# PersiaML/PERSIA

Measured on AMD Instinct MI355X. Metric: samples/sec (whole node), DLRM-style hybrid training, higher is better.
Workload: dtype bf16; 1 GPU; preset=criteo, model=dlrm 26sparse/13dense dim128, global_batch=8192, rows=100000000, capacity_per_rank=100000000, staleness=8, parallelism=dp1+emb-a2a

## Files before the change

persia_amd/core/engine.py:

```python
import contextlib
import functools
import os
import queue
import threading
import time
from dataclasses import dataclass, field
from typing import Dict, List, Optional, Tuple

import numpy as np
import torch

from persia_amd.core import hashing
from persia_amd.core.comm import DistContext
from persia_amd.core.schema import EmbeddingSchema, GlobalConfig, SlotConfig
from persia_amd.core.store import make_store
from persia_amd.embedding import EmbeddingConfig
from persia_amd.embedding.data import PersiaBatch
from persia_amd.embedding.optim import Optimizer
from persia_amd.logger import get_default_logger
from persia_amd.ops import reference as R

_logger = get_default_logger("persia_amd.engine")

_FLIP = -(2 ** 63)
_NO_STREAM = contextlib.nullcontext()


def _roctx_range(name):

    def deco(fn):
        @functools.wraps(fn)
        def wrap(self, *a, **k):
            if not getattr(self, "_roctx", False):
                return fn(self, *a, **k)
            torch.cuda.nvtx.range_push(name)
            try:
                return fn(self, *a, **k)
            finally:
                torch.cuda.nvtx.range_pop()
        return wrap
    return deco


def _update_entry(fn):

    @functools.wraps(fn)
    def wrap(self, *a, **k):
        self._update_counter += 1
        sample = (
            self.metrics_enabled
            and self._update_counter % self._metrics_every
            == 1 % self._metrics_every
        )
        if not (sample or self._roctx):
            return fn(self, *a, **k)
        if self._roctx:
            torch.cuda.nvtx.range_push("persia:update")
        t0 = time.perf_counter()
        try:
            return fn(self, *a, **k)
        finally:
            if sample:
                self.metrics.update_gradient_time_cost_sec.set(
                    time.perf_counter() - t0
                )
            if self._roctx:
                torch.cuda.nvtx.range_pop()

    return wrap


def _sqrt_scale(sqrt_mask: torch.Tensor, seg_lens: torch.Tensor) -> torch.Tensor:
    return torch.where(
        sqrt_mask, seg_lens.clamp(min=1.0).rsqrt(), torch.ones_like(seg_lens)
    )


def _owner_of_keys(keys: torch.Tensor, world_size: int) -> torch.Tensor:
    hi = (keys >> 32) & 0xFFFFFFFF
    return (hi * world_size) >> 32


def _dedup(keys_t: torch.Tensor):
    dev = keys_t.device
    nnz = keys_t.numel()
    if nnz == 0:
        z = torch.zeros(0, dtype=torch.int64, device=dev)
        return z, z, z, torch.zeros(1, dtype=torch.int64, device=dev)
    flipped = keys_t ^ _FLIP
    svals, perm = torch.sort(flipped)
    neq = torch.ones(nnz, dtype=torch.bool, device=dev)
    neq[1:] = svals[1:] != svals[:-1]
    inv_sorted = torch.cumsum(neq, 0) - 1
    inverse = torch.empty(nnz, dtype=torch.int64, device=dev)
    inverse[perm] = inv_sorted
    uniq = svals[neq] ^ _FLIP
    ustarts = torch.cat(
        [
            torch.nonzero(neq, as_tuple=False).view(-1),
            torch.tensor([nnz], dtype=torch.int64, device=dev),
        ]
    )
    return uniq, inverse, perm, ustarts


@dataclass
class SlotPayload:

    name: str
    cfg: SlotConfig
    sum_tensor: Optional[torch.Tensor] = None
    raw_distinct: Optional[torch.Tensor] = None
    raw_index: Optional[torch.Tensor] = None
    raw_non_empty_index: Optional[torch.Tensor] = None
    raw_sample_id_num: Optional[torch.Tensor] = None

    @property
    def is_raw(self) -> bool:
        return self.raw_distinct is not None


@dataclass
class _SlotCtx:
    name: str
    cfg: SlotConfig
    pos_slice: Tuple[int, int]
    seg_offsets: torch.Tensor
    sum_seg_base: int = -1
    slot_uniq_global: Optional[torch.Tensor] = None
    slot_inverse: Optional[torch.Tensor] = None


@dataclass
class _GroupCtx:
    dim: int
    uniq_keys: torch.Tensor
    inverse: torch.Tensor
    perm: torch.Tensor
    ustarts: torch.Tensor
    u_count: Optional[torch.Tensor] = None
    slots: List[_SlotCtx] = field(default_factory=list)
    cat_offsets: Optional[torch.Tensor] = None
    seg_id: Optional[torch.Tensor] = None
    seg_lens: Optional[torch.Tensor] = None
    sqrt_mask: Optional[torch.Tensor] = None
    sum_base: Optional[torch.Tensor] = None
    n_sum_slots: int = 0
    send_counts: Optional[List[int]] = None
    recv_counts: Optional[List[int]] = None
    a2a_plan: Optional["_GroupPlan"] = None
    a2a_idx: Optional[torch.Tensor] = None
    a2a_recv_keys: Optional[torch.Tensor] = None
    a2a_owner_dedup: Optional[tuple] = None


class _GroupPlan:

    def __init__(self, dim: int, cfgs: List[SlotConfig], B: int,
                 device: torch.device):
        S = len(cfgs)
        self.dim = dim
        self.names = tuple(c.name for c in cfgs)
        self.B = B
        self.S = S
        prefixes_np = np.array([c.index_prefix for c in cfgs], dtype=np.uint64)
        self.slot_starts = torch.arange(0, (S + 1) * B, B, dtype=torch.int64,
                                        device=device)
        self.prefixes = torch.from_numpy(prefixes_np.view(np.int64)).to(device)
        self.cat_offsets = torch.arange(S * B + 1, dtype=torch.int64, device=device)
        self.seg_id = torch.arange(S * B, dtype=torch.int64, device=device)
        self.empty_scale = torch.empty(0, dtype=torch.float32, device=device)
        self.a2a_world: Optional[int] = None
        self.a2a_cap: Optional[int] = None
        self.a2a_ar: Optional[torch.Tensor] = None
        self.a2a_ones: Optional[torch.Tensor] = None
        self.owner_seg_id: Optional[torch.Tensor] = None


class _SplitSlots(torch.autograd.Function):

    @staticmethod
    def forward(ctx, base: torch.Tensor, n_slots: int, B: int):
        ctx.n_slots, ctx.B, ctx.dim = n_slots, B, base.shape[1]
        ctx.dev, ctx.dtype = base.device, base.dtype
        return tuple(base[i * B : (i + 1) * B] for i in range(n_slots))

    @staticmethod
    def backward(ctx, *grads):
        parts = [
            g
            if g is not None
            else torch.zeros(ctx.B, ctx.dim, dtype=ctx.dtype, device=ctx.dev)
            for g in grads
        ]
        return torch.cat(parts, dim=0), None, None


class PersiaTrainingBatch:

    def __init__(self):
        self._payloads: List[SlotPayload] = []
        self._lazy_sum_groups: List[Tuple["_GroupCtx", List[str], int]] = []
        self._order: Optional[Dict[str, int]] = None
        self._sorted: bool = False
        self.non_id_type_tensors: List[torch.Tensor] = []
        self.label_tensors: List[torch.Tensor] = []
        self.batch_size: int = 0
        self.requires_grad: bool = True
        self.meta: Optional[bytes] = None
        self.batch_id: Optional[int] = None
        self._groups: List[_GroupCtx] = []
        self._engine: Optional["EmbeddingEngine"] = None

    @property
    def payloads(self) -> List[SlotPayload]:
        if self._lazy_sum_groups:
            for group, _names, B in self._lazy_sum_groups:
                sums = group.sum_base
                for i, sc in enumerate(group.slots):
                    self._payloads.append(
                        SlotPayload(name=sc.name, cfg=sc.cfg,
                                    sum_tensor=sums[i * B : (i + 1) * B])
                    )
            self._lazy_sum_groups.clear()
            self._sorted = False
        if not self._sorted:
            if self._order is not None:
                self._payloads.sort(key=lambda p: self._order[p.name])
            self._sorted = True
        return self._payloads

    def enable_training_views(self) -> Dict[str, torch.Tensor]:
        views: Dict[str, torch.Tensor] = {}
        for group in self._groups:
            if group.sum_base is None:
                continue
            group.sum_base.requires_grad_(True)
            sum_names = [sc.name for sc in group.slots if sc.cfg.embedding_summation]
            parts = _SplitSlots.apply(group.sum_base, len(sum_names), self.batch_size)
            views.update(zip(sum_names, parts))
        return views

    def training_embeddings(self) -> List[torch.Tensor]:
        views = self.enable_training_views()
        return [views.get(p.name, p.sum_tensor) for p in self.payloads]

    def record_stream(self, stream: "torch.cuda.Stream") -> None:
        for t in self._device_tensors():
            t.record_stream(stream)

    def _device_tensors(self):
        for t in self.non_id_type_tensors + self.label_tensors:
            if t.is_cuda:
                yield t
        for g in self._groups:
            a2a_owner = g.a2a_owner_dedup or ()
            for t in (g.uniq_keys, g.inverse, g.perm, g.ustarts, g.u_count,
                      g.sum_base, g.cat_offsets, g.seg_id, g.seg_lens,
                      g.sqrt_mask, g.a2a_idx, g.a2a_recv_keys, *a2a_owner):
                if t is not None and t.is_cuda:
                    yield t
            for sc in g.slots:
                for t in (sc.seg_offsets, sc.slot_uniq_global, sc.slot_inverse):
                    if t is not None and t.is_cuda:
                        yield t
        for p in self._payloads:
            for t in (p.raw_distinct, p.raw_index, p.raw_non_empty_index,
                      p.raw_sample_id_num):
                if t is not None and t.is_cuda:
                    yield t


class EmbeddingEngine:
    def __init__(
        self,
        schema: EmbeddingSchema,
        hyper: EmbeddingConfig,
        optimizer: Optional[Optimizer],
        gconf: GlobalConfig,
        device: torch.device,
        dist_ctx: Optional[DistContext] = None,
        wire_dtype: torch.dtype = torch.float16,
    ):
        self.schema = schema
        self.hyper = hyper
        self.optimizer = optimizer
        self.gconf = gconf
        self.device = device
        self.dist = dist_ctx or DistContext.from_default_group()
        self.dist_grad = (
            DistContext.new_sparse_group() if self.dist.distributed else self.dist
        )
        self.wire_dtype = wire_dtype
        self.groups: Dict[int, List[SlotConfig]] = {}
        for name in schema.slot_names():
            cfg = schema.get_slot(name)
            self.groups.setdefault(cfg.dim, []).append(cfg)
        if optimizer is None:
            from persia_amd.embedding.optim import SGD

            optimizer = SGD(lr=0.0)
            self.optimizer = optimizer
        self.stores = {
            dim: make_store(
                dim, gconf.capacity, optimizer, hyper, device, gconf.spill_capacity
            )
            for dim in self.groups
        }
        self.skipped_grad_signs = 0
        self.nan_grad_batches = 0
        self._plans = {}
        self._empty_scale = torch.empty(0, dtype=torch.float32, device=device)
        spacing = schema.feature_spacing
        self._spacing_arg = spacing if spacing < (1 << 63) else -1
        self.model_manager_status = "Idle"
        self.model_manager_progress = 0.0
        self._prod_timing = os.environ.get("PA_PROD_TIMING", "0") == "1"
        self._prod_timing_live = True
        self._pt = {"prep": 0.0, "native": 0.0, "batch": 0.0, "n": 0,
                    "skip": 20}
        self._fused_dist = os.environ.get("PA_FUSED_DIST", "1") == "1"
        self._force_dist = os.environ.get("PA_FORCE_DIST", "0") == "1"
        self._roctx = os.environ.get("PA_ROCTX", "0") == "1"
        self._a2a_overflow = torch.zeros(1, dtype=torch.int64, device=device)
        from persia_amd.core.metrics import EngineMetrics

        self.metrics_enabled = bool(gconf.enable_metrics)
        self.metrics = EngineMetrics(self.metrics_enabled)
        self._metrics_every = max(1, int(os.environ.get("PA_METRICS_EVERY", "64")))
        self._batch_counter = 0
        self._update_counter = 0
        self._pending_metric = None
        self._skipped_last = (0, 0)
        self._evicted_last = 0
        self.monitor = None
        if self.metrics_enabled:
            from persia_amd.core.monitor import DistinctIdMonitor

            self.monitor = DistinctIdMonitor()
        self.incremental = None
        if gconf.enable_incremental_update:
            self.enable_incremental_update(
                gconf.incremental_dir, gconf.incremental_buffer_size
            )

    def enable_incremental_update(self, dst_dir: str,
                                  buffer_size: int = 1_000_000):
        from persia_amd.core.incremental import IncrementalUpdateDumper

        self.incremental = IncrementalUpdateDumper(self, dst_dir, buffer_size)
        return self.incremental

    @functools.cached_property
    def _C(self):
        from persia_amd.ops import native

        return native()

    def _tick(self, key: str, t0: float) -> float:
        now = time.perf_counter()
        if self._prod_timing_live:
            self._pt[key] = self._pt.get(key, 0.0) + (now - t0)
        return now

    @staticmethod
    def _materialize_group(group: "_GroupCtx") -> "_GroupCtx":
        if group.u_count is None:
            return group
        U = int(group.u_count.item())
        group.uniq_keys = group.uniq_keys.narrow(0, 0, U)
        group.ustarts = group.ustarts.narrow(0, 0, U + 1)
        group.u_count = None
        return group


    def _prepare_slot_keys(self, feat) -> Tuple[np.ndarray, np.ndarray]:
        cfg = self.schema.get_slot(feat.name)
        values, offsets = feat.values, feat.offsets
        rounds = cfg.hash_stack_rounds
        if rounds > 0:
            stacked = hashing.hash_stack(
                values, rounds, cfg.hash_stack_config.embedding_size
            )
            B = len(offsets) - 1
            lens = offsets[1:] - offsets[:-1]
            new_vals = np.empty(len(values) * rounds, dtype=np.uint64)
            new_offsets = np.zeros(B + 1, dtype=np.int64)
            np.cumsum(lens * rounds, out=new_offsets[1:])
            for r in range(rounds):
                for b in range(B):
                    s, e = offsets[b], offsets[b + 1]
                    dst = new_offsets[b] + r * (e - s)
                    new_vals[dst : dst + (e - s)] = stacked[r, s:e]
            values, offsets = new_vals, new_offsets
        signs = hashing.apply_prefix(values, cfg.index_prefix, self.schema.feature_spacing)
        keys = hashing.splitmix64(signs)
        keys[keys == np.uint64(0)] = np.uint64(0xD1B54A32D192ED03)
        return keys, offsets


    def _exchange_rows(self, group: _GroupCtx, train: bool) -> torch.Tensor:
        store = self.stores[group.dim]
        if not self.dist.distributed:
            rows = store.lookup(group.uniq_keys, train, u_count=group.u_count)
            return rows
        owner = _owner_of_keys(group.uniq_keys, self.dist.world_size)
        send_counts = torch.bincount(owner, minlength=self.dist.world_size).tolist()
        recv_counts = self.dist.all_to_all_lengths(send_counts, self.device)
        group.send_counts, group.recv_counts = send_counts, recv_counts
        recv_keys = self.dist.all_to_all(group.uniq_keys, send_counts, recv_counts)
        rows_local = store.lookup(recv_keys, train).to(self.wire_dtype)
        rows = self.dist.all_to_all(rows_local, recv_counts, send_counts)
        return rows


    def _a2a_setup(self, plan: "_GroupPlan") -> Tuple[int, int]:
        if plan.a2a_cap is not None:
            return plan.a2a_world, plan.a2a_cap
        world = self.dist.world_size
        nnz = plan.S * plan.B
        if world > 1:
            lo, hi = self.dist.allreduce_int_minmax(nnz)
            if lo != hi:
                raise RuntimeError(
                    f"padded-a2a fast path needs equal per-rank batch shapes "
                    f"(nnz min {lo} != max {hi}); set PA_FUSED_DIST=0"
                )
            per = max(1, nnz // world)
            cap = per + max(512, per // 8)
        else:
            cap = nnz
        plan.a2a_world = world
        plan.a2a_cap = cap
        plan.a2a_ar = torch.arange(nnz, dtype=torch.int64, device=self.device)
        plan.a2a_ones = torch.ones(nnz, dtype=torch.int64, device=self.device)
        plan.owner_seg_id = torch.arange(
            world * cap, dtype=torch.int64, device=self.device
        )
        return world, cap

    def _a2a_route(self, plan: "_GroupPlan", uniq: torch.Tensor,
                   u_count: Optional[torch.Tensor]):
        world, cap = plan.a2a_world, plan.a2a_cap
        if self.device.type == "cuda":
            return self._C.a2a_route(
                uniq,
                u_count if u_count is not None
                else self.stores[plan.dim].no_count,
                world, cap, self._a2a_overflow,
            )
        n = uniq.numel()
        ar = plan.a2a_ar[:n]
        owner = _owner_of_keys(uniq, world)
        if u_count is not None:
            owner = torch.where(ar < u_count, owner,
                                torch.full_like(owner, world))
        counts = torch.zeros(world + 1, dtype=torch.int64, device=uniq.device)
        counts.scatter_add_(0, owner, plan.a2a_ones[:n])
        starts = torch.cumsum(counts, 0) - counts
        pos = ar - starts.gather(0, owner)
        dummy = world * cap
        bad = (owner >= world) | (pos >= cap)
        idx = torch.where(bad, torch.full_like(pos, dummy), owner * cap + pos)
        send = torch.zeros(dummy + 1, dtype=torch.int64, device=uniq.device)
        send.scatter_(0, idx, uniq)
        self._a2a_overflow.add_((counts[:world] > cap).sum())
        return send, idx

    @_roctx_range("persia:a2a_exchange")
    def _a2a_exchange_fwd(self, plan: "_GroupPlan", group: _GroupCtx,
                          train: bool):
        world, cap = self._a2a_setup(plan)
        timing = self._prod_timing
        if timing:
            t = time.perf_counter()
        send_keys, idx = self._a2a_route(plan, group.uniq_keys, group.u_count)
        comm = self.dist
        if world > 1:
            recv_keys = comm.all_to_all_even(send_keys[: world * cap])
        else:
            recv_keys = send_keys[: world * cap].clone()
        if timing:
            t = self._tick("route", t)
        store = self.stores[group.dim]
        rows_local = store.lookup_wire(recv_keys, train, self.wire_dtype)
        if timing:
            self._tick("lkw", t)
        rows_full = torch.empty(
            world * cap + 1, group.dim, dtype=rows_local.dtype,
            device=self.device,
        )
        if world > 1:
            comm.all_to_all_even(rows_local, out=rows_full[: world * cap])
        else:
            rows_full[: world * cap].copy_(rows_local)
        rows_full[world * cap].zero_()
        group.a2a_plan = plan
        group.a2a_idx = idx
        group.a2a_recv_keys = recv_keys
        if train and self.device.type == "cuda":
            group.a2a_owner_dedup = tuple(self._C.dedup_padded(recv_keys))
        return rows_full, idx

    def check_a2a_overflow(self) -> int:
        return int(self._a2a_overflow.sum().item())


    @_roctx_range("persia:process_batch")
    def process_batch(self, batch: PersiaBatch, train: Optional[bool] = None) -> PersiaTrainingBatch:
        if self._prod_timing:
            self._prod_timing_live = self._pt["skip"] <= 0
            if not self._prod_timing_live:
                self._pt["skip"] -= 1
            _tb0 = time.perf_counter()
        self._batch_counter += 1
        sample = (
            self.metrics_enabled
            and self._batch_counter % self._metrics_every == 1 % self._metrics_every
        )
        if sample:
            _ms_t0 = time.perf_counter()
            _ms_ev0 = None
            if self.device.type == "cuda":
                _ms_ev0 = torch.cuda.Event(enable_timing=True)
                _ms_ev0.record()
        train = batch.requires_grad if train is None else train
        if self.gconf.job_type == "infer":
            train = False
        out = PersiaTrainingBatch()
        out.batch_size = batch.batch_size
        out.requires_grad = batch.requires_grad
        out.meta = batch.meta
        out.batch_id = batch.batch_id
        out._engine = self

        for i, x in enumerate(batch.non_id_type_features):
            out.non_id_type_tensors.append(
                self._upload_aux(batch, ("nid", i), x.data)
            )
        for i, x in enumerate(batch.labels):
            out.label_tensors.append(self._upload_aux(batch, ("lab", i), x.data))

        for dim, feats in self._feats_by_dim(batch).items():
            out._groups.append(self._process_group(dim, feats, out, train, batch))
        out._order = {f.name: i for i, f in enumerate(batch.id_type_features)}
        out._sorted = False
        if sample:
            self._record_lookup_metrics(batch, out, _ms_t0, _ms_ev0)
        if self._prod_timing and self._prod_timing_live:
            self._tick("batch", _tb0)
            self._pt["n"] += 1
        return out

    def _record_lookup_metrics(self, batch, out, t0: float, ev0) -> None:
        m = self.metrics
        m.lookup_preprocess_time_cost_sec.set(time.perf_counter() - t0)
        if self.monitor is not None:
            for feat in batch.id_type_features:
                vals = getattr(feat, "values", None)
                if vals is not None and len(vals):
                    self.monitor.observe(feat.name, vals)
            for name, est in self.monitor.estimates().items():
                m.distinct_id_estimate.labels(name).set(est)
        nnz = sum(
            len(getattr(f, "values", ())) for f in batch.id_type_features
        )
        pend = self._pending_metric
        self._pending_metric = None
        if pend is not None:
            ev_a, ev_b, ucnt_pin, skip_pin, p_nnz, done = pend
            if done.query():
                if ev_a is not None and ev_b is not None:
                    try:
                        m.lookup_hashmap_time_cost_sec.set(
                            ev_a.elapsed_time(ev_b) / 1e3
                        )
                    except Exception:
                        pass
                if ucnt_pin is not None and p_nnz:
                    m.batch_unique_indices_rate.set(
                        float(ucnt_pin.item()) / p_nnz
                    )
                if skip_pin is not None:
                    miss, nan = int(skip_pin[0].item()), int(skip_pin[1].item())
                    lm, ln = self._skipped_last
                    if miss > lm:
                        m.gradient_id_miss_count.inc(miss - lm)
                    if nan > ln:
                        m.nan_grad_skipped.inc(nan - ln)
                    self._skipped_last = (miss, nan)
        if self.device.type == "cuda":
            ev1 = torch.cuda.Event(enable_timing=True)
            ev1.record()
            ucnt_pin = None
            for g in out._groups:
                if g.u_count is not None:
                    ucnt_pin = torch.empty(1, dtype=torch.int64, pin_memory=True)
                    ucnt_pin.copy_(g.u_count, non_blocking=True)
                    break
                m.batch_unique_indices_rate.set(
                    g.uniq_keys.numel() / max(1, nnz)
                )
            skip_pin = None
            skipped = next(iter(self.stores.values())).skip_counters()
            if skipped is not None:
                skip_pin = torch.empty(2, dtype=torch.int32, pin_memory=True)
                skip_pin.copy_(skipped, non_blocking=True)
            done = torch.cuda.Event()
            done.record()
            self._pending_metric = (ev0, ev1, ucnt_pin, skip_pin, nnz, done)
        else:
            U = sum(g.uniq_keys.numel() for g in out._groups)
            m.batch_unique_indices_rate.set(U / max(1, nnz))
            m.nan_grad_skipped.inc(0)
        ev_tot = sum(
            getattr(s, "evicted_total", 0) for s in self.stores.values()
        )
        if ev_tot > self._evicted_last:
            m.evicted_count.inc(ev_tot - self._evicted_last)
            self._evicted_last = ev_tot

    def prepare_host_batch(self, batch: PersiaBatch) -> None:
        if self.device.type != "cuda":
            return
        pc = getattr(batch, "_pinned_cache", None)
        if pc is None:
            pc = batch._pinned_cache = {}
        for kind, items in (("nid", batch.non_id_type_features),
                            ("lab", batch.labels)):
            for i, x in enumerate(items):
                if (kind, i) not in pc:
                    pc[(kind, i)] = self._pin_array(x.data)
        for dim, feats in self._feats_by_dim(batch).items():
            if dim not in pc and self._all_single_sum(feats):
                pc[dim] = self._pin_values(feats)

    def _feats_by_dim(self, batch: PersiaBatch) -> Dict[int, List]:
        by_dim: Dict[int, List] = {}
        for feat in batch.id_type_features:
            by_dim.setdefault(self.schema.get_slot(feat.name).dim, []).append(feat)
        return by_dim

    @staticmethod
    def _pin_array(arr: np.ndarray) -> torch.Tensor:
        src = torch.from_numpy(np.ascontiguousarray(arr))
        t = torch.empty_like(src, pin_memory=True)
        t.copy_(src)
        return t

    def _upload_aux(self, batch, cache_key, arr: np.ndarray) -> torch.Tensor:
        if self.device.type != "cuda":
            return torch.from_numpy(np.ascontiguousarray(arr)).to(self.device)
        pc = getattr(batch, "_pinned_cache", None)
        if pc is None:
            pc = batch._pinned_cache = {}
        t = pc.get(cache_key)
        if t is None:
            t = pc[cache_key] = self._pin_array(arr)
        return t.to(self.device, non_blocking=True)

    def _pin_values(self, feats) -> torch.Tensor:
        values_np = np.concatenate([f.values for f in feats])
        pin = torch.empty(len(values_np), dtype=torch.int64, pin_memory=True)
        pin.numpy()[:] = values_np.view(np.int64)
        return pin

    def _upload_group(self, dim: int, feats, batch) -> torch.Tensor:
        pcache = getattr(batch, "_pinned_cache", None)
        if pcache is None:
            pcache = batch._pinned_cache = {}
        pin = pcache.get(dim)
        if pin is None:
            pin = pcache[dim] = self._pin_values(feats)
        return pin.to(self.device, non_blocking=True)

    def _all_single_sum(self, feats) -> bool:
        get_slot = self.schema.get_slot
        for f in feats:
            if not getattr(f, "is_single", False):
                return False
            cfg = get_slot(f.name)
            if not cfg.embedding_summation or cfg.hash_stack_rounds != 0:
                return False
        return True

    def _padded_a2a(self, store) -> bool:
        return (
            (self.dist.distributed or self._force_dist)
            and self._fused_dist
            and store.spill is None
        )

    def _plan(self, dim: int, names: Tuple[str, ...], B: int) -> _GroupPlan:
        plan = self._plans.get((dim, names, B))
        if plan is None:
            cfgs = [self.schema.get_slot(n) for n in names]
            plan = self._plans[(dim, names, B)] = _GroupPlan(
                dim, cfgs, B, self.device
            )
        return plan

    def _process_group_fast(self, dim: int, feats, out: PersiaTrainingBatch,
                            train: bool, batch: PersiaBatch) -> _GroupCtx:
        timing = self._prod_timing
        if timing:
            t0 = time.perf_counter()
        C = self._C
        B = len(feats[0].values)
        plan = self._plan(dim, tuple(f.name for f in feats), B)
        slot_ctxs = [
            _SlotCtx(
                name=f.name, cfg=self.schema.get_slot(f.name),
                pos_slice=(i * B, (i + 1) * B), seg_offsets=None,
                sum_seg_base=i * B,
            )
            for i, f in enumerate(feats)
        ]
        store = self.stores[dim]
        dist = self.dist.distributed
        one_call = not (dist or self._force_dist or store.spill is not None)
        padded = not one_call and self._padded_a2a(store)
        if one_call:
            if timing:
                t0 = self._tick("prep", t0)
            sums, uniq, inverse, perm, ustarts, u_count = store.lookup_local(
                self._upload_group(dim, feats, batch), plan.slot_starts,
                plan.prefixes, self._spacing_arg, plan.cat_offsets,
                plan.empty_scale, train,
            )
        else:
            ps = cur = None
            if store.spill is not None and not dist and train:
                ps, cur = store.probe_stream, torch.cuda.current_stream()
            with torch.cuda.stream(ps) if ps is not None else _NO_STREAM:
                vals_t = self._upload_group(dim, feats, batch)
                keys_t = C.sign_prep(
                    vals_t, plan.slot_starts, plan.prefixes, self._spacing_arg
                )
                if padded or not dist:
                    uniq, inverse, perm, ustarts, u_count = C.dedup_padded(keys_t)
                else:
                    uniq, inverse, perm, ustarts = _dedup(keys_t)
                    u_count = None
                if ps is not None:
                    store.spill_restore(uniq, u_count)
            if ps is not None:
                cur.wait_stream(ps)
                for x in (vals_t, uniq, inverse, perm, ustarts, u_count):
                    x.record_stream(cur)
        group = _GroupCtx(
            dim=dim, uniq_keys=uniq, inverse=inverse, perm=perm,
            ustarts=ustarts, u_count=u_count, slots=slot_ctxs,
            cat_offsets=plan.cat_offsets, seg_id=plan.seg_id,
            n_sum_slots=plan.S,
        )
        if padded:
            if timing:
                t = self._tick("dedup", t0)
            rows_full, idx = self._a2a_exchange_fwd(plan, group, train)
            if timing:
                t = self._tick("exch", t)
            sums = C.segment_sum(
                rows_full, idx.gather(0, inverse), plan.cat_offsets,
                plan.empty_scale,
            )
            if timing:
                self._tick("sum", t)
        elif not one_call:
            rows = self._exchange_rows(group, train)
            sums = C.segment_sum(
                rows.contiguous(), inverse, plan.cat_offsets, plan.empty_scale
            )
        group.sum_base = sums
        out._lazy_sum_groups.append((group, [sc.name for sc in slot_ctxs], B))
        if timing and (one_call or padded):
            self._tick("native", t0)
        return group

    def _process_group(self, dim: int, feats, out: PersiaTrainingBatch, train: bool,
                       batch: PersiaBatch) -> _GroupCtx:
        native = self.device.type == "cuda"
        fast_shape = self._all_single_sum(feats)
        if native and fast_shape:
            return self._process_group_fast(dim, feats, out, train, batch)
        feats = sorted(
            feats, key=lambda f: 0 if self.schema.get_slot(f.name).embedding_summation else 1
        )
        keys_t, slot_ctxs = self._group_keys(feats, gpu_prep=native)
        uniq_keys, inverse, perm, ustarts = _dedup(keys_t)
        group = _GroupCtx(
            dim=dim, uniq_keys=uniq_keys, inverse=inverse, perm=perm,
            ustarts=ustarts, slots=slot_ctxs,
        )
        if not native and fast_shape and self._padded_a2a(self.stores[dim]):
            plan = self._plan(
                dim, tuple(sc.name for sc in slot_ctxs), out.batch_size
            )
            rows_full, idx = self._a2a_exchange_fwd(plan, group, train)
            rows = rows_full[idx]
        else:
            rows = self._exchange_rows(group, train)
        self._sum_payloads(group, rows, out)
        self._raw_payloads(group, rows, out)
        return group

    def _group_keys(self, feats, gpu_prep: bool):
        dev = self.device
        key_arrays = []
        offset_arrays = []
        slot_ctxs: List[_SlotCtx] = []
        in_lens: List[int] = []
        rounds_list: List[int] = []
        sizes_list: List[int] = []
        pos = 0
        for feat in feats:
            cfg = self.schema.get_slot(feat.name)
            r = cfg.hash_stack_rounds
            if gpu_prep:
                keys = feat.values
                offsets = feat.offsets * r if r > 0 else feat.offsets
                out_len = len(keys) * max(r, 1)
            else:
                keys, offsets = self._prepare_slot_keys(feat)
                out_len = len(keys)
            key_arrays.append(keys)
            offset_arrays.append(offsets)
            in_lens.append(len(keys))
            rounds_list.append(r if gpu_prep else 0)
            sizes_list.append(
                cfg.hash_stack_config.embedding_size if r > 0 else 1
            )
            slot_ctxs.append(
                _SlotCtx(name=feat.name, cfg=cfg, pos_slice=(pos, pos + out_len),
                         seg_offsets=None)
            )
            pos += out_len

        all_keys = np.concatenate(key_arrays) if key_arrays else np.empty(0, np.uint64)
        keys_t = torch.from_numpy(all_keys.view(np.int64)).to(dev, non_blocking=False)
        all_offs = np.concatenate(offset_arrays or [np.zeros(1, np.int64)])
        all_offs_t = torch.from_numpy(all_offs).to(dev)
        o0 = 0
        for sc, offs in zip(slot_ctxs, offset_arrays):
            sc.seg_offsets = all_offs_t[o0 : o0 + len(offs)]
            o0 += len(offs)
        if not gpu_prep:
            return keys_t, slot_ctxs
        out_starts = torch.tensor(
            [sc.pos_slice[0] for sc in slot_ctxs] + [pos],
            dtype=torch.int64, device=dev,
        )
        prefixes = torch.from_numpy(
            np.array([sc.cfg.index_prefix for sc in slot_ctxs], dtype=np.uint64)
            .view(np.int64)
        ).to(dev)
        if not any(rounds_list):
            return self._C.sign_prep(
                keys_t, out_starts, prefixes, self._spacing_arg
            ), slot_ctxs
        in_starts = torch.from_numpy(
            np.concatenate([[0], np.cumsum(in_lens)]).astype(np.int64)
        ).to(dev)
        off_starts = torch.from_numpy(
            np.concatenate(
                [[0], np.cumsum([len(o) for o in offset_arrays])]
            ).astype(np.int64)
        ).to(dev)
        keys_t = self._C.sign_prep_stack(
            keys_t, in_starts, out_starts, prefixes,
            torch.tensor(rounds_list, dtype=torch.int32, device=dev),
            torch.tensor(sizes_list, dtype=torch.int64, device=dev),
            off_starts, all_offs_t, self._spacing_arg, pos,
        )
        return keys_t, slot_ctxs

    def _sum_payloads(self, group: _GroupCtx, rows: torch.Tensor,
                      out: PersiaTrainingBatch) -> None:
        sum_slots = [sc for sc in group.slots if sc.cfg.embedding_summation]
        if not sum_slots:
            return
        dev = self.device
        base = 0
        offs_parts, sqrt_parts = [], []
        for sc in sum_slots:
            s, _e = sc.pos_slice
            sc.sum_seg_base = base
            nseg = sc.seg_offsets.numel() - 1
            offs_parts.append(sc.seg_offsets[:-1] + s)
            sqrt_parts.append(
                torch.full((nseg,), bool(sc.cfg.sqrt_scaling), dtype=torch.bool, device=dev)
            )
            base += nseg
        sum_end = sum_slots[-1].pos_slice[1]
        cat_offsets = torch.cat(
            offs_parts + [torch.tensor([sum_end], dtype=torch.int64, device=dev)]
        )
        group.cat_offsets = cat_offsets
        group.sqrt_mask = torch.cat(sqrt_parts)
        seg_counts = cat_offsets[1:] - cat_offsets[:-1]
        group.seg_lens = seg_counts.float()
        seg_id = torch.full(
            (group.inverse.numel(),), -1, dtype=torch.int64, device=dev
        )
        seg_id[:sum_end] = torch.repeat_interleave(
            torch.arange(base, dtype=torch.int64, device=dev), seg_counts
        )
        group.seg_id = seg_id
        fwd_scale = _sqrt_scale(group.sqrt_mask, group.seg_lens)
        if dev.type == "cuda":
            sums = self._C.segment_sum(
                rows.contiguous(), group.inverse, cat_offsets, fwd_scale
            )
        else:
            sums = (
                R.segment_sum_rows(
                    rows, group.inverse[:sum_end], cat_offsets, False, torch.float32
                )
                * fwd_scale.unsqueeze(1)
            ).to(torch.float16)
        group.sum_base = sums
        group.n_sum_slots = len(sum_slots)
        b0 = 0
        for sc in sum_slots:
            nseg = sc.seg_offsets.numel() - 1
            out._payloads.append(
                SlotPayload(name=sc.name, cfg=sc.cfg, sum_tensor=sums[b0 : b0 + nseg])
            )
            b0 += nseg

    def _raw_payloads(self, group: _GroupCtx, rows: torch.Tensor,
                      out: PersiaTrainingBatch) -> None:
        for sc in group.slots:
            if sc.cfg.embedding_summation:
                continue
            s, e = sc.pos_slice
            slot_uniq, slot_inv = torch.unique(
                group.inverse[s:e], sorted=True, return_inverse=True
            )
            sc.slot_uniq_global = slot_uniq
            sc.slot_inverse = slot_inv
            scale = 1.0
            rounds = sc.cfg.hash_stack_rounds
            if sc.cfg.sqrt_scaling and rounds > 1:
                scale = 1.0 / float(np.sqrt(rounds))
            distinct, index, non_empty, num = R.raw_embedding_tensors(
                rows[slot_uniq], slot_inv, sc.seg_offsets, sc.cfg.sample_fixed_size,
                scale, torch.float16,
            )
            out._payloads.append(
                SlotPayload(
                    name=sc.name, cfg=sc.cfg, raw_distinct=distinct, raw_index=index,
                    raw_non_empty_index=non_empty, raw_sample_id_num=num,
                )
            )


    def _seg_scale(self, group: _GroupCtx, loss_scale: float,
                   skip: Optional[torch.Tensor] = None) -> torch.Tensor:
        mask = group.sqrt_mask
        has_sqrt = mask is not None and (skip is not None or bool(mask.any()))
        if skip is None and loss_scale == 1.0 and not has_sqrt:
            return self._empty_scale
        scale = torch.full(
            (group.cat_offsets.numel() - 1,), 1.0 / loss_scale,
            device=self.device,
        )
        if has_sqrt:
            scale = scale * _sqrt_scale(mask, group.seg_lens)
        if skip is not None:
            scale = torch.where(skip, torch.zeros_like(scale), scale)
        return scale

    def _nan_slot(self, sc: _SlotCtx, g: torch.Tensor) -> bool:
        if not bool(torch.isnan(g).any()):
            return False
        self.nan_grad_batches += 1
        _logger.warning(f"nan found in gradient update of {sc.name}, skipping")
        return True

    def _add_raw_grads(self, group: _GroupCtx, grads, loss_scale: float,
                       buf: torch.Tensor) -> bool:
        added = False
        for sc in group.slots:
            if sc.cfg.embedding_summation:
                continue
            g = grads.get(sc.name)
            if g is None or self._nan_slot(sc, g):
                continue
            gf = g.float()
            if loss_scale != 1.0:
                gf = gf / loss_scale
            rounds = sc.cfg.hash_stack_rounds
            if sc.cfg.sqrt_scaling and rounds > 0:
                gf = gf / float(np.sqrt(rounds))
            buf.index_add_(0, sc.slot_uniq_global, gf)
            added = True
        return added

    @_update_entry
    def apply_gradients(
        self,
        training_batch: PersiaTrainingBatch,
        grads: Dict[str, Optional[torch.Tensor]],
        loss_scale: float = 1.0,
    ) -> None:
        self._apply_slot_grads(training_batch, grads, loss_scale)

    def _apply_slot_grads(self, training_batch, grads, loss_scale) -> None:
        native = self.device.type == "cuda"
        B = training_batch.batch_size
        for group in training_batch._groups:
            self._materialize_group(group)
            U = group.uniq_keys.numel()
            buf = torch.zeros(U, group.dim, dtype=torch.float32, device=self.device)
            sum_slots = [
                sc for sc in group.slots
                if sc.cfg.embedding_summation and grads.get(sc.name) is not None
            ]
            any_grad = False
            if native and sum_slots:
                g_parts, flag_parts = [], []
                for sc in group.slots:
                    if not sc.cfg.embedding_summation:
                        continue
                    g = grads.get(sc.name)
                    if g is None:
                        g = torch.zeros(B, group.dim, dtype=torch.float16, device=self.device)
                        flag = torch.ones((), dtype=torch.bool, device=self.device)
                    else:
                        flag = torch.isnan(g).any()
                    g_parts.append(g.to(torch.float16))
                    flag_parts.append(flag.expand(B))
                scale = self._seg_scale(group, loss_scale, skip=torch.cat(flag_parts))
                self._C.grad_scatter(
                    torch.nan_to_num(torch.cat(g_parts, dim=0)).contiguous(),
                    group.perm, group.ustarts, group.seg_id, scale.contiguous(),
                    buf, 1,
                )
                any_grad = True
            elif not native:
                for sc in sum_slots:
                    g = grads[sc.name]
                    if self._nan_slot(sc, g):
                        continue
                    any_grad = True
                    s, e = sc.pos_slice
                    buf += R.segment_grad_scatter(
                        g, group.inverse[s:e], sc.seg_offsets, U,
                        scale_factor=loss_scale, sqrt_scaling=sc.cfg.sqrt_scaling,
                    )
            if self._add_raw_grads(group, grads, loss_scale, buf) or any_grad:
                self._route_and_update(group, buf)

    def _a2a_backward_native(self, group: _GroupCtx, gbase: torch.Tensor,
                             seg_scale: torch.Tensor, store) -> None:
        plan = group.a2a_plan
        world, cap = plan.a2a_world, plan.a2a_cap
        send_g = torch.empty(
            world * cap + 1, group.dim, dtype=torch.float16, device=self.device
        )
        self._C.grad_scatter_idx(
            gbase.contiguous(), group.perm, group.ustarts, group.seg_id,
            seg_scale, group.a2a_idx, send_g,
            group.u_count if group.u_count is not None else store.no_count,
        )
        if world > 1:
            recv_g = self.dist_grad.all_to_all_even(send_g[: world * cap])
        else:
            recv_g = send_g[: world * cap]
        if group.a2a_owner_dedup is None:
            group.a2a_owner_dedup = tuple(
                self._C.dedup_padded(group.a2a_recv_keys)
            )
        ou, _oinv, operm, oustarts, ou_count = group.a2a_owner_dedup
        store.scatter_update(
            ou, recv_g, operm, oustarts, plan.owner_seg_id, ou_count
        )
        if self.incremental is not None:
            self.incremental.record_keys(ou, ou_count)

    def _store_update(self, store, keys: torch.Tensor, grads: torch.Tensor) -> None:
        self.skipped_grad_signs += store.update_gradients(keys, grads)
        if self.incremental is not None:
            self.incremental.record_keys(keys)

    def _owner_merge_update(self, store, keys_recv: torch.Tensor,
                            grads_recv: torch.Tensor) -> None:
        uniq_f, inv = torch.unique(keys_recv ^ _FLIP, sorted=True, return_inverse=True)
        merged = torch.zeros(
            uniq_f.numel(), store.dim, dtype=torch.float32, device=self.device
        )
        merged.index_add_(0, inv, grads_recv.float())
        self._store_update(store, uniq_f ^ _FLIP, merged)

    def _route_and_update_padded(self, group: _GroupCtx, buf: torch.Tensor) -> None:
        plan = group.a2a_plan
        world, cap = plan.a2a_world, plan.a2a_cap
        send_g = torch.zeros(
            world * cap + 1, group.dim, dtype=self.wire_dtype,
            device=self.device,
        )
        send_g.index_copy_(
            0, group.a2a_idx[: buf.shape[0]], buf.to(self.wire_dtype)
        )
        if world > 1:
            recv_g = self.dist_grad.all_to_all_even(send_g[: world * cap])
        else:
            recv_g = send_g[: world * cap]
        rk = group.a2a_recv_keys
        m = rk != 0
        if bool(m.any()):
            self._owner_merge_update(self.stores[group.dim], rk[m], recv_g[m])

    def _route_and_update(self, group: _GroupCtx, buf: torch.Tensor) -> None:
        store = self.stores[group.dim]
        if group.a2a_idx is not None:
            return self._route_and_update_padded(group, buf)
        if not self.dist.distributed:
            return self._store_update(store, group.uniq_keys, buf)
        comm = self.dist_grad
        send_counts, recv_counts = group.send_counts, group.recv_counts
        if send_counts is None:
            owner = _owner_of_keys(group.uniq_keys, comm.world_size)
            send_counts = torch.bincount(owner, minlength=comm.world_size).tolist()
            recv_counts = comm.all_to_all_lengths(send_counts, self.device)
        keys_recv = comm.all_to_all(group.uniq_keys, send_counts, recv_counts)
        grads_recv = comm.all_to_all(
            buf.to(self.wire_dtype), send_counts, recv_counts
        )
        self._owner_merge_update(store, keys_recv, grads_recv)

    @_update_entry
    def apply_gradients_base(
        self,
        training_batch: PersiaTrainingBatch,
        raw_grads: Optional[Dict[str, Optional[torch.Tensor]]] = None,
        loss_scale: float = 1.0,
        sum_base_grads: Optional[List[torch.Tensor]] = None,
    ) -> None:
        groups = training_batch._groups
        if sum_base_grads is None:
            sum_base_grads = [
                g.sum_base.grad if g.sum_base is not None else None
                for g in groups
            ]
        if self.device.type != "cuda":
            grads: Dict[str, Optional[torch.Tensor]] = dict(raw_grads or {})
            B = training_batch.batch_size
            for group, gbase in zip(groups, sum_base_grads):
                b0 = 0
                for sc in group.slots:
                    if sc.cfg.embedding_summation:
                        grads[sc.name] = (
                            gbase[b0 : b0 + B] if gbase is not None else None
                        )
                        b0 += B
            return self._apply_slot_grads(training_batch, grads, loss_scale)

        for group, gbase in zip(groups, sum_base_grads):
            if gbase is None and not raw_grads:
                continue
            store = self.stores[group.dim]
            if gbase is not None:
                seg_scale = self._seg_scale(group, loss_scale)
                if store.fused_native and not raw_grads:
                    if (
                        group.a2a_idx is not None
                        and self.wire_dtype == torch.float16
                    ):
                        self._a2a_backward_native(group, gbase, seg_scale, store)
                        continue
                    if not self.dist.distributed:
                        store.update_local(
                            gbase, group.perm, group.ustarts, group.seg_id,
                            seg_scale, group.uniq_keys, group.u_count,
                        )
                        if self.incremental is not None:
                            self.incremental.record_keys(
                                group.uniq_keys, group.u_count
                            )
                        continue
            self._materialize_group(group)
            U = group.uniq_keys.numel()
            if gbase is not None:
                buf = torch.empty(
                    U, group.dim, dtype=torch.float32, device=self.device
                )
                self._C.grad_scatter(
                    gbase.contiguous(), group.perm, group.ustarts,
                    group.seg_id, seg_scale, buf, 0,
                )
            else:
                buf = torch.zeros(
                    U, group.dim, dtype=torch.float32, device=self.device
                )
            if raw_grads:
                self._add_raw_grads(group, raw_grads, loss_scale, buf)
            self._route_and_update(group, buf)


    def _set_status(self, status: str, progress: float = 0.0):
        self.model_manager_status = status
        self.model_manager_progress = progress

    def dump(self, dst_dir: str, blocking: bool = True) -> None:
        from persia_amd.core.checkpoint import dump_embedding

        def run():
            try:
                dump_embedding(self, dst_dir)
                self._set_status("Idle", 100.0)
            except Exception as e:
                _logger.error(f"embedding dump failed: {e}")
                self._set_status("Failed")
                if blocking:
                    raise

        self._set_status("Dumping", 0.0)
        if blocking:
            run()
        else:
            threading.Thread(target=run, daemon=True, name="persia-ckpt-dump").start()

    def load(self, src_dir: str, blocking: bool = True) -> None:
        from persia_amd.core.checkpoint import load_embedding

        def run():
            try:
                load_embedding(self, src_dir)
                self._set_status("Idle", 100.0)
            except Exception as e:
                _logger.error(f"embedding load failed: {e}")
                self._set_status("Failed")
                if blocking:
                    raise

        self._set_status("Loading", 0.0)
        if blocking:
            run()
        else:
            threading.Thread(target=run, daemon=True, name="persia-ckpt-load").start()

    def wait_for_emb_dumping(self, timeout: float = 600.0) -> None:
        import time as _time

        t0 = _time.time()
        while getattr(self, "model_manager_status", "Idle") == "Dumping":
            if _time.time() - t0 > timeout:
                raise TimeoutError("embedding dump did not finish")
            _time.sleep(0.05)
        if getattr(self, "model_manager_status", "Idle") == "Failed":
            raise RuntimeError("embedding dump failed")

    def wait_for_emb_loading(self, timeout: float = 600.0) -> None:
        import time as _time

        t0 = _time.time()
        while getattr(self, "model_manager_status", "Idle") == "Loading":
            if _time.time() - t0 > timeout:
                raise TimeoutError("embedding load did not finish")
            _time.sleep(0.05)
        if getattr(self, "model_manager_status", "Idle") == "Failed":
            raise RuntimeError("embedding load failed")

    def num_resident_rows(self) -> int:
        return sum(len(s) for s in self.stores.values())


class ForwardPipeline:

    def __init__(self, engine: EmbeddingEngine, staleness: int = 8, out_buffer: int = 8,
                 reorder: bool = False):
        self.engine = engine
        self.staleness = max(1, staleness)
        self.reorder = reorder
        self._heap: list = []
        self._next_id = 0
        self._sem = threading.Semaphore(self.staleness)
        self._in: "queue.Queue" = queue.Queue(maxsize=max(2, out_buffer))
        self._out: "queue.Queue" = queue.Queue(maxsize=max(2, out_buffer))
        self._thread: Optional[threading.Thread] = None
        self._stop = threading.Event()
        self._exc: Optional[BaseException] = None
        self.inflight = 0
        self.prod_s = 0.0
        self.prod_n = 0

    def start(self):
        if self._thread is None:
            self._thread = threading.Thread(target=self._run, daemon=True, name="persia-forward")
            self._thread.start()

    def _run(self):
        stream = None
        if self.engine.device.type == "cuda":
            torch.cuda.set_device(self.engine.device)
            prio = int(os.environ.get("PA_SPARSE_PRIORITY", "0"))
            stream = torch.cuda.Stream(device=self.engine.device, priority=prio)
        import heapq

        pending_eof = False
        while not self._stop.is_set():
            item = None
            if self.reorder and self._heap and self._heap[0][0] == self._next_id:
                item = heapq.heappop(self._heap)[1]
                self._next_id += 1
            else:
                try:
                    got = self._in.get(timeout=0.1)
                except queue.Empty:
                    if pending_eof and not self._heap:
                        self._out.put(None)
                        break
                    continue
                if got is None:
                    if self.reorder and self._heap:
                        pending_eof = True
                        continue
                    self._out.put(None)
                    break
                if self.reorder and got.batch_id is not None:
                    if got.batch_id != self._next_id:
                        heapq.heappush(self._heap, (got.batch_id, got))
                        continue
                    self._next_id += 1
                item = got
            self._sem.acquire()
            self.inflight += 1
            if self.engine.metrics_enabled:
                self.engine.metrics.staleness.set(self.inflight)
            try:
                t0 = time.perf_counter()
                if stream is not None:
                    with torch.cuda.stream(stream):
                        tb = self.engine.process_batch(item)
                    ev = torch.cuda.Event()
                    ev.record(stream)
                    tb._ready_event = ev
                else:
                    tb = self.engine.process_batch(item)
                self.prod_s += time.perf_counter() - t0
                self.prod_n += 1
                self._out.put(tb)
            except BaseException as e:
                self._exc = e
                self._out.put(None)
                break

    def put(self, batch: PersiaBatch):
        self.start()
        self._in.put(batch)
        if self.engine.metrics_enabled:
            self.engine.metrics.num_pending_batches.set(self._in.qsize())

    def finish(self):
        self.start()
        self._in.put(None)

    def get(self, timeout: Optional[float] = None) -> Optional[PersiaTrainingBatch]:
        tb = self._out.get(timeout=timeout)
        if tb is None and self._exc is not None:
            raise self._exc
        if tb is not None and getattr(tb, "_ready_event", None) is not None:
            cur = torch.cuda.current_stream()
            cur.wait_event(tb._ready_event)
            tb.record_stream(cur)
        return tb

    def release_permit(self):
        self.inflight = max(0, self.inflight - 1)
        self._sem.release()

    def stop(self):
        self._stop.set()
        self._sem.release()
        try:
            self._in.put_nowait(None)
        except queue.Full:
            pass
        if self._thread is not None:
            self._thread.join(timeout=5.0)
            self._thread = None
```

persia_amd/core/store.py:

```python
from typing import Iterator, Optional, Tuple

import numpy as np
import torch

from persia_amd.core import hashing
from persia_amd.embedding import EmbeddingConfig
from persia_amd.embedding.optim import Adagrad, Adam, Optimizer, SGD

BUCKET_SIZE = 8
PROBE_BUCKETS = 4
EMPTY_KEY = np.uint64(0)
_ZERO_REMAP = np.uint64(0xD1B54A32D192ED03)


def _floor_pow2(x: int) -> int:
    p = 1
    while (p << 1) <= x:
        p <<= 1
    return p


def _u01_from_u64(u: np.ndarray) -> np.ndarray:
    return (u >> np.uint64(40)).astype(np.float64) * (1.0 / (1 << 24))


def row_init(sign: int, dim: int, lo: float, hi: float) -> np.ndarray:
    seed = hashing.init_seed_for(np.array([sign], dtype=np.uint64))[0]
    cols = np.arange(1, dim + 1, dtype=np.uint64)
    u = hashing.splitmix64(np.uint64(seed) ^ cols)
    return (lo + (hi - lo) * _u01_from_u64(u)).astype(np.float32)


class HostTier:

    def __init__(self, capacity: int, row_width: int):
        from collections import OrderedDict

        self.capacity = capacity
        self.row_width = row_width
        self._map: "OrderedDict[int, np.ndarray]" = OrderedDict()

    def __len__(self) -> int:
        return len(self._map)

    def insert(self, keys: np.ndarray, rows: np.ndarray) -> None:
        for i, k in enumerate(keys):
            k = int(k)
            if k in self._map:
                self._map.move_to_end(k)
            self._map[k] = rows[i].copy()
        while len(self._map) > self.capacity:
            self._map.popitem(last=False)

    def fetch(self, keys: np.ndarray):
        rows = np.zeros((len(keys), self.row_width), dtype=np.float32)
        found = np.zeros(len(keys), dtype=bool)
        for i, k in enumerate(keys):
            row = self._map.pop(int(k), None)
            if row is not None:
                rows[i] = row
                found[i] = True
        return rows, found

    def __contains__(self, key) -> bool:
        return int(key) in self._map

    def export(self):
        n = len(self._map)
        keys = np.fromiter(self._map.keys(), dtype=np.uint64, count=n)
        rows = (
            np.stack(list(self._map.values()))
            if n
            else np.zeros((0, self.row_width), dtype=np.float32)
        )
        return keys, rows.astype(np.float32)


class NativeHostTier:

    def __init__(self, capacity: int, row_width: int):
        from persia_amd.ops import native

        self.capacity = capacity
        self.row_width = row_width
        self._impl = native().HostTier(capacity, row_width)

    def __len__(self) -> int:
        return int(self._impl.size())

    def insert(self, keys: np.ndarray, rows: np.ndarray) -> None:
        self._impl.insert(
            torch.from_numpy(np.ascontiguousarray(keys).view(np.int64)),
            torch.from_numpy(np.ascontiguousarray(rows, dtype=np.float32)),
        )

    def fetch(self, keys: np.ndarray):
        rows, found = self._impl.fetch(
            torch.from_numpy(np.ascontiguousarray(keys).view(np.int64))
        )
        return rows.numpy(), found.numpy()

    def __contains__(self, key) -> bool:
        return bool(self._impl.contains(int(np.int64(np.uint64(key)))))

    def export(self):
        keys, rows = self._impl.export_all()
        return keys.numpy().view(np.uint64), rows.numpy()



def _adapt_row_width(inner: np.ndarray, row_width: int,
                     state_init: float = 0.0) -> np.ndarray:
    cur = inner.shape[1]
    if cur == row_width:
        return inner
    if cur > row_width:
        return np.ascontiguousarray(inner[:, :row_width])
    out = np.full((inner.shape[0], row_width), state_init, dtype=np.float32)
    out[:, :cur] = inner
    return out


class EmbeddingStoreBase:

    fused_native = False

    def __init__(
        self,
        dim: int,
        capacity: int,
        optimizer: Optimizer,
        hyper: EmbeddingConfig,
        device: torch.device,
        spill_capacity: int = 0,
    ):
        self.dim = dim
        self.optimizer = optimizer
        self.hyper = hyper
        self.device = device
        self.opt_space = optimizer.require_space(dim)
        self.row_width = dim + self.opt_space
        self.n_buckets = _floor_pow2(max(1, capacity // BUCKET_SIZE))
        self.n_slots = self.n_buckets * BUCKET_SIZE
        self.tick = 1
        self._tick_lock = __import__("threading").Lock()
        self.spill = HostTier(spill_capacity, self.row_width) if spill_capacity > 0 else None
        if isinstance(optimizer, Adam):
            self.beta1_power = optimizer.betas[0]
            self.beta2_power = optimizer.betas[1]

    def __len__(self) -> int:
        raise NotImplementedError

    def lookup(self, keys: torch.Tensor, train: bool,
               u_count: Optional[torch.Tensor] = None) -> torch.Tensor:
        raise NotImplementedError

    def update_gradients(self, keys: torch.Tensor, grads: torch.Tensor) -> int:
        raise NotImplementedError

    def lookup_wire(self, keys: torch.Tensor, train: bool,
                    wire_dtype: torch.dtype) -> torch.Tensor:
        raise NotImplementedError

    def export_rows(self) -> Tuple[np.ndarray, np.ndarray]:
        raise NotImplementedError

    def import_rows(self, signs: np.ndarray, inner: np.ndarray) -> None:
        raise NotImplementedError

    def export_chunks(
        self, chunk_rows: int
    ) -> Iterator[Tuple[np.ndarray, np.ndarray]]:
        chunk_rows = max(1, int(chunk_rows))
        signs, inner = self.export_rows()
        for lo in range(0, len(signs), chunk_rows):
            yield signs[lo:lo + chunk_rows], inner[lo:lo + chunk_rows]

    def import_chunk(self, signs: np.ndarray, inner: np.ndarray) -> None:
        self.import_rows(np.asarray(signs), np.asarray(inner))

    def finish_import(self) -> int:
        return 0

    def clear(self) -> None:
        raise NotImplementedError

    def next_tick(self) -> int:
        with self._tick_lock:
            t = self.tick
            self.tick += 1
        return t

    def export_keys(self, signs: np.ndarray) -> Tuple[np.ndarray, np.ndarray]:
        raise NotImplementedError

    def skip_counters(self) -> Optional[torch.Tensor]:
        return None

    def _spill_export(self):
        if self.spill is None or len(self.spill) == 0:
            return None
        keys, rows = self.spill.export()
        return hashing.splitmix64_inv(keys), rows

    def _adam_step_powers(self):
        o = self.optimizer
        if isinstance(o, Adam):
            b1p, b2p = self.beta1_power, self.beta2_power
            self.beta1_power *= o.betas[0]
            self.beta2_power *= o.betas[1]
            return b1p, b2p
        return None


class CpuEmbeddingStore(EmbeddingStoreBase):

    def __init__(self, dim, capacity, optimizer, hyper, device=torch.device("cpu"),
                 spill_capacity: int = 0):
        super().__init__(dim, capacity, optimizer, hyper, device, spill_capacity)
        self.keys = np.zeros(self.n_slots, dtype=np.uint64)
        self.ticks = np.zeros(self.n_slots, dtype=np.uint32)
        self.arena = torch.zeros(self.n_slots, self.row_width, dtype=torch.float32)
        self._count = 0

    def __len__(self) -> int:
        return self._count

    def _probe(self, k: np.uint64) -> int:
        mask = np.uint64(self.n_buckets - 1)
        b0 = int(k & mask)
        for p in range(PROBE_BUCKETS):
            base = ((b0 + p) % self.n_buckets) * BUCKET_SIZE
            for s in range(BUCKET_SIZE):
                if self.keys[base + s] == k:
                    return base + s
        return -1

    def _probe_or_claim(self, k: np.uint64, tick: int) -> Tuple[int, bool]:
        mask = np.uint64(self.n_buckets - 1)
        b0 = int(k & mask)
        empty = -1
        victim, victim_tick = -1, None
        for p in range(PROBE_BUCKETS):
            base = ((b0 + p) % self.n_buckets) * BUCKET_SIZE
            for s in range(BUCKET_SIZE):
                i = base + s
                ki = self.keys[i]
                if ki == k:
                    return i, False
                if ki == EMPTY_KEY:
                    if empty < 0:
                        empty = i
                elif self.ticks[i] != tick and (
                    victim_tick is None or self.ticks[i] < victim_tick
                ):
                    victim, victim_tick = i, self.ticks[i]
        if empty >= 0:
            self.keys[empty] = k
            self.ticks[empty] = tick
            self._count += 1
            return empty, True
        if victim < 0:
            return -1, False
        if self.spill is not None:
            self.spill.insert(
                np.array([self.keys[victim]], dtype=np.uint64),
                self.arena[victim].numpy().reshape(1, -1),
            )
        self.keys[victim] = k
        self.ticks[victim] = tick
        return victim, True

    def _init_row(self, slot: int, k: np.uint64) -> None:
        sign = int(hashing.splitmix64_inv(np.array([k], dtype=np.uint64))[0])
        lo, hi = self.hyper.emb_initialization
        emb = row_init(sign, self.dim, lo, hi)
        row = torch.zeros(self.row_width, dtype=torch.float32)
        row[: self.dim] = torch.from_numpy(emb)
        if self.opt_space:
            row[self.dim :] = self.optimizer.state_init(self.dim)
        self.arena[slot] = row

    def _admitted(self, k: np.uint64, tick: int) -> bool:
        if self.hyper.admit_probability >= 1.0:
            return True
        u = hashing.splitmix64(np.array([k ^ np.uint64(tick)], dtype=np.uint64))
        return float(_u01_from_u64(u)[0]) < self.hyper.admit_probability

    def lookup(self, keys: torch.Tensor, train: bool,
               u_count: Optional[torch.Tensor] = None) -> torch.Tensor:
        assert u_count is None, "padded lookup is a HIP-path feature"
        tick = self.next_tick()
        k_np = keys.cpu().numpy().view(np.uint64).copy()
        k_np[k_np == EMPTY_KEY] = _ZERO_REMAP
        out = torch.zeros(len(k_np), self.dim, dtype=torch.float32)
        for i, k in enumerate(k_np):
            if train:
                if self._admitted(k, tick) or self._probe(k) >= 0:
                    slot, is_new = self._probe_or_claim(k, tick)
                    if slot < 0:
                        continue
                    if is_new:
                        restored = False
                        if self.spill is not None:
                            rows, found = self.spill.fetch(np.array([k], dtype=np.uint64))
                            if found[0]:
                                self.arena[slot] = torch.from_numpy(rows[0])
                                restored = True
                        if not restored:
                            self._init_row(slot, k)
                    self.ticks[slot] = tick
                    out[i] = self.arena[slot, : self.dim]
            else:
                slot = self._probe(k)
                if slot >= 0:
                    self.ticks[slot] = tick
                    out[i] = self.arena[slot, : self.dim]
        return out

    def lookup_wire(self, keys: torch.Tensor, train: bool,
                    wire_dtype: torch.dtype) -> torch.Tensor:
        out = torch.zeros(keys.numel(), self.dim, dtype=torch.float32)
        m = keys != 0
        if bool(m.any()):
            out[m] = self.lookup(keys[m], train)
        else:
            self.next_tick()
        return out.to(wire_dtype)

    def update_gradients(self, keys: torch.Tensor, grads: torch.Tensor) -> int:
        powers = self._adam_step_powers()
        k_np = keys.cpu().numpy().view(np.uint64).copy()
        k_np[k_np == EMPTY_KEY] = _ZERO_REMAP
        slots = np.array([self._probe(k) for k in k_np], dtype=np.int64)
        present = slots >= 0
        nan_rows = torch.isnan(grads.float()).any(dim=1).cpu().numpy()
        present = present & ~nan_rows
        skipped = int((slots < 0).sum())
        if present.sum() == 0:
            return skipped
        idx = torch.from_numpy(slots[present])
        g = grads.float().cpu()[torch.from_numpy(np.nonzero(present)[0])]
        rows = self.arena[idx]
        emb = rows[:, : self.dim]
        from persia_amd.ops import reference as R

        o = self.optimizer
        wb = self.hyper.weight_bound
        if isinstance(o, SGD):
            R.sgd_update(emb, g, o.lr, o.weight_decay, wb)
        elif isinstance(o, Adagrad):
            accum = rows[:, self.dim :] if not o.vectorwise_shared else rows[:, self.dim : self.dim + 1]
            R.adagrad_update(
                emb, accum, g, o.lr, o.g_square_momentum, o.eps, wb, o.vectorwise_shared
            )
        elif isinstance(o, Adam):
            m = rows[:, self.dim : 2 * self.dim]
            v = rows[:, 2 * self.dim :]
            b1p, b2p = powers
            R.adam_update(emb, m, v, g, b1p, b2p, o.lr, o.betas[0], o.betas[1], o.eps, wb)
        else:
            raise ValueError(f"unknown optimizer {o.kind}")
        self.arena[idx] = rows
        return skipped

    def export_keys(self, signs: np.ndarray) -> Tuple[np.ndarray, np.ndarray]:
        ks = hashing.splitmix64(signs.astype(np.uint64))
        ks[ks == EMPTY_KEY] = _ZERO_REMAP
        slots = np.array([self._probe(k) for k in ks], dtype=np.int64)
        found = slots >= 0
        inner = self.arena[torch.from_numpy(slots[found])].numpy().copy()
        return signs[found], inner

    def export_rows(self) -> Tuple[np.ndarray, np.ndarray]:
        occ = np.nonzero(self.keys != EMPTY_KEY)[0]
        signs = hashing.splitmix64_inv(self.keys[occ])
        inner = self.arena[torch.from_numpy(occ)].numpy()
        sp = self._spill_export()
        if sp is not None:
            signs = np.concatenate([signs, sp[0]])
            inner = np.concatenate([inner, sp[1]])
        return signs, inner

    def import_rows(self, signs: np.ndarray, inner: np.ndarray) -> None:
        inner = _adapt_row_width(
            inner, self.row_width, float(self.optimizer.state_init(self.dim))
        )
        ks = hashing.splitmix64(signs.astype(np.uint64))
        ks[ks == EMPTY_KEY] = _ZERO_REMAP
        tick = self.next_tick()
        for i, k in enumerate(ks):
            slot, _ = self._probe_or_claim(k, tick)
            if slot < 0:
                continue
            self.arena[slot] = torch.from_numpy(inner[i].astype(np.float32))
            self.ticks[slot] = tick

    def clear(self) -> None:
        self.keys[:] = EMPTY_KEY
        self.ticks[:] = 0
        self.arena.zero_()
        self._count = 0


class HipEmbeddingStore(EmbeddingStoreBase):

    fused_native = True

    def __init__(self, dim, capacity, optimizer, hyper, device, spill_capacity: int = 0):
        super().__init__(dim, capacity, optimizer, hyper, device, spill_capacity)
        from persia_amd.ops import native

        self._C = native()
        assert device.type == "cuda"
        if self.spill is not None:
            self.spill = NativeHostTier(spill_capacity, self.row_width)
        self.keys = torch.zeros(self.n_slots, dtype=torch.int64, device=device)
        self.ticks = torch.zeros(self.n_slots, dtype=torch.int32, device=device)
        self.arena = torch.zeros(
            self.n_slots, self.row_width, dtype=torch.float32, device=device
        )
        self._skipped = torch.zeros(2, dtype=torch.int32, device=device)
        self._opt_code = {"sgd": 0, "adagrad": 1, "adam": 2}[optimizer.kind]
        self._probe_stream: Optional[torch.cuda.Stream] = None
        self._restore_tick: Optional[int] = None
        self._ckpt_stream: Optional[torch.cuda.Stream] = None
        self._imported = torch.zeros(1, dtype=torch.int64, device=device)
        self._import_offered = 0
        self.evicted_total = 0
        self.no_count = torch.empty(0, dtype=torch.int64, device=device)
        self._no_scale = torch.empty(0, dtype=torch.float32, device=device)
        self._no_evict = (
            self.no_count,
            torch.empty(0, dtype=torch.int32, device=device),
            self._no_scale,
        )

    def _evict_buffers(self, n: int):
        if self.spill is None:
            return self._no_evict
        return (
            torch.zeros(n, dtype=torch.int64, device=self.device),
            torch.zeros(1, dtype=torch.int32, device=self.device),
            torch.empty(n, self.row_width, dtype=torch.float32, device=self.device),
        )

    def _drain_evictions(self, ev):
        keys_t, count_t, rows_t = ev
        if keys_t.numel() == 0:
            return
        self._drain_pending()
        cnt_pin = torch.zeros(1, dtype=torch.int32, pin_memory=True)
        cnt_pin.copy_(count_t, non_blocking=True)
        done = torch.cuda.Event()
        done.record()
        self._pending_evict = (keys_t, rows_t, cnt_pin, done)

    def _drain_pending(self):
        pend = getattr(self, "_pending_evict", None)
        if pend is None:
            return
        self._pending_evict = None
        keys_t, rows_t, cnt_pin, done = pend
        done.synchronize()
        cnt = int(cnt_pin.item())
        if cnt == 0:
            return
        self.evicted_total += cnt
        keys_np = keys_t[:cnt].cpu().numpy().view(np.uint64)
        rows_np = rows_t[:cnt].cpu().numpy()
        self.spill.insert(keys_np, rows_np)

    def flush_spill(self):
        if self.spill is not None:
            self._drain_pending()

    def _opt_params(self):
        o = self.optimizer
        if isinstance(o, SGD):
            return [o.lr, o.weight_decay, 0.0, 0.0, 0.0, 0.0]
        if isinstance(o, Adagrad):
            return [
                o.lr,
                o.g_square_momentum,
                o.eps,
                1.0 if o.vectorwise_shared else 0.0,
                0.0,
                0.0,
            ]
        if isinstance(o, Adam):
            return [o.lr, o.betas[0], o.betas[1], o.eps, 0.0, 0.0]
        raise ValueError(o.kind)

    def _lookup_args(self, train: bool, tick: int):
        lo, hi = self.hyper.emb_initialization
        return (
            self.dim, int(train), tick, float(lo), float(hi),
            float(self.hyper.admit_probability),
            float(self.optimizer.state_init(self.dim)), self.opt_space,
        )

    def _update_args(self):
        powers = self._adam_step_powers()
        b1p, b2p = powers if powers else (0.0, 0.0)
        return (
            self.dim, self._opt_code, self._opt_params(), float(b1p),
            float(b2p), float(self.hyper.weight_bound), self._skipped,
        )

    def __len__(self) -> int:
        return int((self.keys != 0).sum().item())

    @property
    def probe_stream(self) -> "torch.cuda.Stream":
        if self._probe_stream is None:
            self._probe_stream = torch.cuda.Stream(device=self.device)
        return self._probe_stream

    def spill_restore(self, keys: torch.Tensor,
                      u_count: Optional[torch.Tensor] = None) -> None:
        tick = self.next_tick()
        self._restore_tick = tick
        if not len(self.spill) or keys.numel() == 0:
            return
        self._drain_pending()
        ev = self._spill_phase1(
            keys, tick, u_count if u_count is not None else self.no_count, 0
        )
        if ev is not None:
            self._drain_evictions(ev)

    def _spill_phase1(self, keys: torch.Tensor, tick: int, uc: torch.Tensor,
                      log_rows: int):
        slots = self._C.store_probe(self.keys, self.ticks, keys, tick, uc)
        miss_keys = keys[slots < 0]
        if not miss_keys.numel():
            return None
        miss_np = miss_keys.cpu().numpy().view(np.uint64)
        rows, found = self.spill.fetch(miss_np)
        if not found.any():
            return None
        ev = self._evict_buffers(log_rows + int(found.sum()))
        found_keys = torch.from_numpy(
            miss_np[found].view(np.int64).copy()
        ).to(self.device)
        rows_t = torch.from_numpy(rows[found]).to(self.device)
        self._C.store_import(
            self.keys, self.ticks, self.arena, found_keys, rows_t, tick, *ev
        )
        return ev

    def lookup(
        self, keys: torch.Tensor, train: bool,
        u_count: Optional[torch.Tensor] = None,
    ) -> torch.Tensor:
        restored = self._restore_tick is not None
        if restored:
            tick = self._restore_tick
            self._restore_tick = None
        else:
            tick = self.next_tick()
        n = keys.numel()
        uc = u_count if u_count is not None else self.no_count
        ev = self._no_evict
        if self.spill is not None and train and n:
            self._drain_pending()
            ev = self._evict_buffers(n)
            if not restored and len(self.spill):
                ev = self._spill_phase1(keys, tick, uc, n) or ev
        out = torch.empty(n, self.dim, dtype=torch.float32, device=self.device)
        self._C.store_lookup(
            self.keys, self.ticks, self.arena, keys, out,
            *self._lookup_args(train, tick), *ev, uc,
        )
        self._drain_evictions(ev)
        return out

    def lookup_wire(self, keys: torch.Tensor, train: bool,
                    wire_dtype: torch.dtype) -> torch.Tensor:
        out = torch.empty(
            keys.numel(), self.dim, dtype=wire_dtype, device=self.device
        )
        self._C.store_lookup(
            self.keys, self.ticks, self.arena, keys, out,
            *self._lookup_args(train, self.next_tick()), *self._no_evict,
            self.no_count,
        )
        return out

    def lookup_local(self, values: torch.Tensor, slot_starts: torch.Tensor,
                     prefixes: torch.Tensor, spacing_arg: int,
                     cat_offsets: torch.Tensor, seg_scale: torch.Tensor,
                     train: bool):
        return self._C.lookup_local(
            values, slot_starts, prefixes, spacing_arg, cat_offsets, seg_scale,
            self.keys, self.ticks, self.arena,
            *self._lookup_args(train, self.next_tick()),
        )

    def update_local(self, gbase, perm, ustarts, seg_id, seg_scale, uniq,
                     u_count: Optional[torch.Tensor]) -> None:
        self._C.update_local(
            gbase.contiguous(), perm, ustarts, seg_id, seg_scale, uniq,
            self.keys, self.ticks, self.arena, *self._update_args(),
            u_count if u_count is not None else self.no_count,
        )

    def scatter_update(self, uniq, grads, perm, ustarts, seg_id,
                       u_count: torch.Tensor) -> None:
        self._C.scatter_update(
            self.keys, self.ticks, self.arena, uniq, grads, perm, ustarts,
            seg_id, self._no_scale, *self._update_args(), u_count,
        )

    def update_gradients(self, keys: torch.Tensor, grads: torch.Tensor) -> int:
        self._C.store_update(
            self.keys, self.ticks, self.arena, keys,
            grads.float().contiguous(), *self._update_args(),
        )
        return 0

    def skip_counters(self) -> torch.Tensor:
        return self._skipped

    def skipped_count(self) -> int:
        return int(self._skipped[0].item())

    def nan_row_count(self) -> int:
        return int(self._skipped[1].item())

    def export_keys(self, signs: np.ndarray) -> Tuple[np.ndarray, np.ndarray]:
        ks = hashing.splitmix64(signs.astype(np.uint64))
        ks[ks == EMPTY_KEY] = _ZERO_REMAP
        keys_t = torch.from_numpy(ks.view(np.int64)).to(self.device)
        slots = self._C.store_probe(
            self.keys, self.ticks, keys_t, self.tick, self.no_count
        )
        found = slots >= 0
        inner = self.arena[slots[found]].cpu().numpy()
        found_np = found.cpu().numpy()
        out_signs, out_inner = signs[found_np], inner
        if self.spill is not None and (~found_np).any():
            self.flush_spill()
            miss, miss_ks = signs[~found_np], ks[~found_np]
            rows, sp_found = self.spill.fetch(miss_ks)
            if sp_found.any():
                self.spill.insert(miss_ks[sp_found], rows[sp_found])
                out_signs = np.concatenate([out_signs, miss[sp_found]])
                out_inner = np.concatenate([out_inner, rows[sp_found]])
        return out_signs, out_inner

    def export_rows(self) -> Tuple[np.ndarray, np.ndarray]:
        self.flush_spill()
        occ = torch.nonzero(self.keys != 0, as_tuple=False).view(-1)
        keys = self.keys[occ].cpu().numpy().view(np.uint64)
        signs = hashing.splitmix64_inv(keys)
        inner = self.arena[occ].cpu().numpy()
        sp = self._spill_export()
        if sp is not None:
            signs = np.concatenate([signs, sp[0]])
            inner = np.concatenate([inner, sp[1]])
        return signs, inner

    def import_rows(self, signs: np.ndarray, inner: np.ndarray) -> None:
        inner = _adapt_row_width(
            inner, self.row_width, float(self.optimizer.state_init(self.dim))
        )
        ks = hashing.splitmix64(signs.astype(np.uint64))
        ks[ks == EMPTY_KEY] = _ZERO_REMAP
        keys_t = torch.from_numpy(ks.view(np.int64)).to(self.device)
        rows_t = torch.from_numpy(np.ascontiguousarray(inner, dtype=np.float32)).to(
            self.device
        )
        tick = self.next_tick()
        ev = self._evict_buffers(keys_t.numel())
        self._C.store_import(
            self.keys, self.ticks, self.arena, keys_t, rows_t, tick, *ev
        )
        self._drain_evictions(ev)

    @property
    def ckpt_stream(self) -> "torch.cuda.Stream":
        if self._ckpt_stream is None:
            self._ckpt_stream = torch.cuda.Stream(device=self.device)
        return self._ckpt_stream

    def export_chunks(
        self, chunk_rows: int
    ) -> Iterator[Tuple[np.ndarray, np.ndarray]]:
        chunk_rows = max(1, int(chunk_rows))
        self.flush_spill()
        cap = min(chunk_rows, self.n_slots)
        n_win = (self.n_slots + cap - 1) // cap
        st = self.ckpt_stream
        ready = torch.cuda.Event()
        ready.record(torch.cuda.current_stream(self.device))
        with torch.cuda.stream(st):
            st.wait_event(ready)
            dev = [
                (
                    torch.empty(cap, dtype=torch.int64, device=self.device),
                    torch.empty(cap, self.row_width, dtype=torch.float32,
                                device=self.device),
                    torch.empty(1, dtype=torch.int32, device=self.device),
                )
                for _ in range(2)
            ]
        pin = [
            (
                torch.empty(cap, dtype=torch.int64, pin_memory=True),
                torch.empty(cap, self.row_width, dtype=torch.float32,
                            pin_memory=True),
                torch.empty(1, dtype=torch.int32, pin_memory=True),
            )
            for _ in range(2)
        ]
        counted = [torch.cuda.Event() for _ in range(2)]
        copied = [torch.cuda.Event() for _ in range(2)]

        def stage(k: int) -> int:
            b = k % 2
            d_signs, d_rows, d_count = dev[b]
            p_signs, p_rows, p_count = pin[b]
            with torch.cuda.stream(st):
                self._C.store_export_window(
                    self.keys, self.arena, k * cap,
                    min(self.n_slots, (k + 1) * cap), d_signs, d_rows, d_count,
                )
                p_count.copy_(d_count, non_blocking=True)
                counted[b].record(st)
                counted[b].synchronize()
                c = int(p_count.item())
                if c:
                    p_signs[:c].copy_(d_signs[:c], non_blocking=True)
                    p_rows[:c].copy_(d_rows[:c], non_blocking=True)
                copied[b].record(st)
            return c

        c = stage(0)
        for k in range(n_win):
            c_next = stage(k + 1) if k + 1 < n_win else 0
            b = k % 2
            copied[b].synchronize()
            if c:
                yield (
                    pin[b][0][:c].numpy().view(np.uint64),
                    pin[b][1][:c].numpy(),
                )
            c = c_next
        sp = self.spill.export() if self.spill is not None and len(self.spill) else None
        if sp is not None:
            sp_keys, sp_rows = sp
            for lo in range(0, len(sp_keys), chunk_rows):
                yield (
                    hashing.splitmix64_inv(sp_keys[lo:lo + chunk_rows]),
                    sp_rows[lo:lo + chunk_rows],
                )

    def import_chunk(self, signs: np.ndarray, inner: np.ndarray) -> None:
        n = len(signs)
        if n == 0:
            return
        assert inner.shape[0] == n and inner.shape[1] > 0
        p_signs = torch.empty(n, dtype=torch.int64, pin_memory=True)
        p_rows = torch.empty(n, inner.shape[1], dtype=torch.float32, pin_memory=True)
        np.copyto(p_signs.numpy().view(np.uint64), signs, casting="same_kind")
        np.copyto(p_rows.numpy(), inner, casting="same_kind")
        signs_t = p_signs.to(self.device, non_blocking=True)
        rows_t = p_rows.to(self.device, non_blocking=True)
        tick = self.next_tick()
        ev = self._evict_buffers(n)
        self._C.store_import_signs(
            self.keys, self.ticks, self.arena, signs_t, rows_t, tick,
            float(self.optimizer.state_init(self.dim)), *ev, self._imported,
        )
        self._import_offered += n
        self._drain_evictions(ev)

    def finish_import(self) -> int:
        if self._import_offered == 0:
            return 0
        dropped = self._import_offered - int(self._imported.item())
        self._import_offered = 0
        self._imported.zero_()
        return dropped

    def clear(self) -> None:
        self.keys.zero_()
        self.ticks.zero_()
        self.arena.zero_()


def make_store(
    dim: int,
    capacity: int,
    optimizer: Optimizer,
    hyper: EmbeddingConfig,
    device: torch.device,
    spill_capacity: int = 0,
) -> EmbeddingStoreBase:
    if device.type == "cuda":
        return HipEmbeddingStore(dim, capacity, optimizer, hyper, device, spill_capacity)
    return CpuEmbeddingStore(dim, capacity, optimizer, hyper, device, spill_capacity)
```

persia_amd/csrc/engine.cpp:

```cpp
#include <torch/extension.h>

void store_lookup(torch::Tensor table_keys, torch::Tensor ticks,
                  torch::Tensor arena, torch::Tensor query, torch::Tensor out,
                  int64_t dim, int64_t train, int64_t tick, double lo,
                  double hi, double admit_prob, double state_init,
                  int64_t opt_space, torch::Tensor evict_keys,
                  torch::Tensor evict_count, torch::Tensor evict_rows,
                  torch::Tensor u_count);
void store_lookup_sums(torch::Tensor table_keys, torch::Tensor ticks,
                       torch::Tensor arena, torch::Tensor query,
                       torch::Tensor perm, torch::Tensor ustarts,
                       torch::Tensor sums, int64_t dim, int64_t train,
                       int64_t tick, double lo, double hi, double admit_prob,
                       double state_init, int64_t opt_space,
                       torch::Tensor u_count);
void store_update(torch::Tensor table_keys, torch::Tensor ticks,
                  torch::Tensor arena, torch::Tensor query,
                  torch::Tensor grads, int64_t dim, int64_t opt,
                  std::vector<double> params, double b1_power,
                  double b2_power, double weight_bound, torch::Tensor skipped);
torch::Tensor segment_sum(torch::Tensor rows, torch::Tensor inverse,
                          torch::Tensor seg_offsets, torch::Tensor seg_scale);
void grad_scatter(torch::Tensor grads, torch::Tensor perm,
                  torch::Tensor ustarts, torch::Tensor seg_id,
                  torch::Tensor seg_scale, torch::Tensor out,
                  int64_t accumulate);
torch::Tensor sign_prep(torch::Tensor values, torch::Tensor slot_starts,
                        torch::Tensor prefixes, int64_t spacing);
void scatter_update(torch::Tensor table_keys, torch::Tensor ticks,
                    torch::Tensor arena, torch::Tensor uniq,
                    torch::Tensor grads, torch::Tensor perm,
                    torch::Tensor ustarts, torch::Tensor seg_id,
                    torch::Tensor seg_scale, int64_t dim, int64_t opt,
                    std::vector<double> params, double b1_power,
                    double b2_power, double weight_bound,
                    torch::Tensor skipped, torch::Tensor u_count);
void dedup_finalize(torch::Tensor svals_flipped, torch::Tensor perm,
                    torch::Tensor neq, torch::Tensor rank, int64_t flip,
                    torch::Tensor inverse, torch::Tensor uniq,
                    torch::Tensor ustarts, torch::Tensor u_count);
std::vector<torch::Tensor> sort_pairs_u64(torch::Tensor keys);
torch::Tensor neq_flags(torch::Tensor sorted);

static constexpr int64_t kFlip = std::numeric_limits<int64_t>::min();

std::vector<torch::Tensor> dedup_keys(torch::Tensor keys) {
  auto dev = keys.device();
  const int64_t nnz = keys.numel();
  auto opts = torch::TensorOptions().dtype(torch::kInt64).device(dev);
  if (nnz == 0) {
    auto z = torch::zeros({0}, opts);
    return {z, z, z, torch::zeros({1}, opts)};
  }
  auto flipped = keys.bitwise_xor(kFlip);
  auto sorted = flipped.sort();
  auto svals = std::get<0>(sorted);
  auto perm = std::get<1>(sorted);
  auto neq = torch::ones({nnz}, opts.dtype(torch::kBool));
  neq.slice(0, 1, nnz) =
      svals.slice(0, 1, nnz).ne(svals.slice(0, 0, nnz - 1));
  auto inv_sorted = neq.cumsum(0) - 1;
  auto inverse = torch::empty({nnz}, opts);
  inverse.index_put_({perm}, inv_sorted);
  auto uniq = svals.masked_select(neq).bitwise_xor(kFlip);
  auto starts = neq.nonzero().view(-1);
  auto ustarts = torch::cat({starts, torch::full({1}, nnz, opts)});
  return {uniq, inverse, perm, ustarts};
}

std::vector<torch::Tensor> dedup_padded(torch::Tensor keys) {
  const int64_t nnz = keys.numel();
  auto opts = torch::TensorOptions().dtype(torch::kInt64).device(keys.device());
  auto sp = sort_pairs_u64(keys);
  auto& svals = sp[0];
  auto& perm = sp[1];
  auto neq = neq_flags(svals);
  auto rank = neq.cumsum(0);
  rank.sub_(1);
  auto inverse = torch::empty({nnz}, opts);
  auto uniq = torch::zeros({nnz}, opts);
  auto ustarts = torch::empty({nnz + 1}, opts);
  auto u_count = torch::empty({1}, opts);
  dedup_finalize(svals, perm, neq, rank, 0, inverse, uniq, ustarts,
                 u_count);
  return {uniq, inverse, perm, ustarts, u_count};
}

std::vector<torch::Tensor> lookup_local(
    torch::Tensor values, torch::Tensor slot_starts, torch::Tensor prefixes,
    int64_t spacing, torch::Tensor cat_offsets, torch::Tensor seg_scale,
    torch::Tensor table_keys, torch::Tensor ticks, torch::Tensor arena,
    int64_t dim, int64_t train, int64_t tick, double lo, double hi,
    double admit_prob, double state_init, int64_t opt_space) {
  auto keys = sign_prep(values, slot_starts, prefixes, spacing);
  auto d = dedup_padded(keys);
  auto& uniq = d[0];
  auto& inverse = d[1];
  auto& perm = d[2];
  auto& ustarts = d[3];
  auto& u_count = d[4];
  const int64_t nnz = keys.numel();
  auto dev = values.device();
  auto opts = torch::TensorOptions().dtype(torch::kInt64).device(dev);
  auto sums = torch::empty(
      {nnz, dim}, torch::TensorOptions().dtype(torch::kFloat16).device(dev));
  store_lookup_sums(table_keys, ticks, arena, uniq, perm, ustarts, sums, dim,
                    train, tick, lo, hi, admit_prob, state_init, opt_space,
                    u_count);
  return {sums, uniq, inverse, perm, ustarts, u_count};
}

void update_local(torch::Tensor grads, torch::Tensor perm,
                  torch::Tensor ustarts, torch::Tensor seg_id,
                  torch::Tensor seg_scale, torch::Tensor uniq_keys,
                  torch::Tensor table_keys, torch::Tensor ticks,
                  torch::Tensor arena, int64_t dim, int64_t opt,
                  std::vector<double> params, double b1_power, double b2_power,
                  double weight_bound, torch::Tensor skipped,
                  torch::Tensor u_count) {
  if (grads.scalar_type() == torch::kFloat16 && dim <= 512) {
    scatter_update(table_keys, ticks, arena, uniq_keys, grads, perm, ustarts,
                   seg_id, seg_scale, dim, opt, params, b1_power, b2_power,
                   weight_bound, skipped, u_count);
    return;
  }
  if (u_count.numel()) {
    const int64_t U = u_count.item<int64_t>();
    uniq_keys = uniq_keys.narrow(0, 0, U);
    ustarts = ustarts.narrow(0, 0, U + 1);
  }
  auto buf = torch::empty(
      {uniq_keys.numel(), dim},
      torch::TensorOptions().dtype(torch::kFloat32).device(grads.device()));
  grad_scatter(grads, perm, ustarts, seg_id, seg_scale, buf, 0);
  store_update(table_keys, ticks, arena, uniq_keys, buf, dim, opt, params,
               b1_power, b2_power, weight_bound, skipped);
}


#include <list>
#include <memory>
#include <unordered_map>
#include <vector>

struct NativeHostTier {
  static constexpr int64_t CHUNK_ROWS = 1 << 16;
  static constexpr int SHARDS = 16;
  int64_t capacity, row_width;
  std::vector<std::unique_ptr<float[]>> chunks;
  std::vector<int64_t> free_slots;
  int64_t next_fresh = 0;
  std::list<std::pair<uint64_t, int64_t>> lru;
  std::unordered_map<uint64_t,
                     std::list<std::pair<uint64_t, int64_t>>::iterator>
      map[SHARDS];

  NativeHostTier(int64_t cap, int64_t rw) : capacity(cap), row_width(rw) {}

  float* rowp(int64_t slot) {
    return chunks[slot / CHUNK_ROWS].get() + (slot % CHUNK_ROWS) * row_width;
  }
  int64_t alloc_slot() {
    if (!free_slots.empty()) {
      const int64_t s = free_slots.back();
      free_slots.pop_back();
      return s;
    }
    if (next_fresh >= (int64_t)chunks.size() * CHUNK_ROWS)
      chunks.emplace_back(new float[CHUNK_ROWS * row_width]);
    return next_fresh++;
  }
  auto& shard(uint64_t key) { return map[key & (SHARDS - 1)]; }

  void erase_entry(std::list<std::pair<uint64_t, int64_t>>::iterator it) {
    free_slots.push_back(it->second);
    shard(it->first).erase(it->first);
    lru.erase(it);
  }

  void insert(torch::Tensor keys, torch::Tensor rows) {
    TORCH_CHECK(!keys.is_cuda() && !rows.is_cuda(), "HostTier: cpu tensors");
    TORCH_CHECK(rows.size(1) == row_width, "HostTier: row width mismatch");
    auto kc = keys.contiguous();
    auto rc = rows.contiguous();
    const int64_t* kp = kc.data_ptr<int64_t>();
    const float* rp = rc.data_ptr<float>();
    const int64_t k = kc.numel();
    for (int64_t i = 0; i < k; ++i) {
      const uint64_t key = (uint64_t)kp[i];
      auto& m = shard(key);
      auto it = m.find(key);
      int64_t slot;
      if (it != m.end()) {
        slot = it->second->second;
        lru.erase(it->second);
        lru.emplace_back(key, slot);
        it->second = std::prev(lru.end());
      } else {
        slot = alloc_slot();
        lru.emplace_back(key, slot);
        m[key] = std::prev(lru.end());
      }
      std::copy(rp + i * row_width, rp + (i + 1) * row_width, rowp(slot));
    }
    while ((int64_t)lru.size() > capacity) erase_entry(lru.begin());
  }

  std::tuple<torch::Tensor, torch::Tensor> fetch(torch::Tensor keys) {
    auto kc = keys.contiguous();
    const int64_t* kp = kc.data_ptr<int64_t>();
    const int64_t k = kc.numel();
    auto rows = torch::zeros({k, row_width}, torch::kFloat32);
    auto found = torch::zeros({k}, torch::kBool);
    float* rp = rows.data_ptr<float>();
    bool* fp = found.data_ptr<bool>();
    for (int64_t i = 0; i < k; ++i) {
      const uint64_t key = (uint64_t)kp[i];
      auto& m = shard(key);
      auto it = m.find(key);
      if (it == m.end()) continue;
      const float* src = rowp(it->second->second);
      std::copy(src, src + row_width, rp + i * row_width);
      fp[i] = true;
      erase_entry(it->second);
    }
    return {rows, found};
  }

  std::tuple<torch::Tensor, torch::Tensor> export_all() {
    const int64_t n = (int64_t)lru.size();
    auto keys = torch::empty({n}, torch::kInt64);
    auto rows = torch::empty({n, row_width}, torch::kFloat32);
    int64_t* kp = keys.data_ptr<int64_t>();
    float* rp = rows.data_ptr<float>();
    int64_t i = 0;
    for (auto& e : lru) {
      kp[i] = (int64_t)e.first;
      const float* src = rowp(e.second);
      std::copy(src, src + row_width, rp + i * row_width);
      ++i;
    }
    return {keys, rows};
  }

  int64_t size() const { return (int64_t)lru.size(); }
  bool contains(int64_t key) {
    return shard((uint64_t)key).count((uint64_t)key) != 0;
  }
  void clear() {
    lru.clear();
    for (auto& m : map) m.clear();
    chunks.clear();
    free_slots.clear();
    next_fresh = 0;
  }
};

void init_engine(pybind11::module_& m) {
  m.def("dedup_keys", &dedup_keys, "sort-based dedup of u64 keys");
  m.def("dedup_padded", &dedup_padded,
        "sync-free dedup: nnz-padded outputs + device unique count");
  pybind11::class_<NativeHostTier>(m, "HostTier")
      .def(pybind11::init<int64_t, int64_t>())
      .def("insert", &NativeHostTier::insert)
      .def("fetch", &NativeHostTier::fetch)
      .def("export_all", &NativeHostTier::export_all)
      .def("size", &NativeHostTier::size)
      .def("contains", &NativeHostTier::contains)
      .def("clear", &NativeHostTier::clear);
  m.def("lookup_local", &lookup_local,
        "fused single-GPU lookup (sign prep + dedup + probe + gather + sum)");
  m.def("update_local", &update_local,
        "fused single-GPU backward (scatter + optimizer update)");
}
```

persia_amd/csrc/kernels.hip:

```cpp

#include <torch/extension.h>
#include <ATen/hip/HIPContext.h>
#include <hip/hip_runtime.h>
#include <hip/hip_bf16.h>
#include <hipcub/hipcub.hpp>

#include "common.h"
#include "optim.h"
#include "probe.h"

using ull = unsigned long long;

namespace {

struct PaLanes {
  int G, sub, c0, st;
};
__device__ __forceinline__ PaLanes pa_lanes(int lane, int dim) {
  PaLanes l;
  l.G = (dim < PA_WAVE && (PA_WAVE % dim) == 0) ? PA_WAVE / dim : 1;
  l.sub = (l.G > 1) ? lane / dim : 0;
  l.c0 = (l.G > 1) ? lane % dim : lane;
  l.st = (l.G > 1) ? dim : PA_WAVE;
  return l;
}

__device__ __forceinline__ void pa_init_row(float* row, ull key,
                                            int dim, int row_width, double lo,
                                            double hi, float state_init,
                                            int c0, int st) {
  const uint64_t seed = pa_init_seed(pa_splitmix64_inv((uint64_t)key));
  for (int c = c0; c < dim; c += st) row[c] = pa_init_val(seed, c, lo, hi);
  for (int c = dim + c0; c < row_width; c += st) row[c] = state_init;
}


__device__ __forceinline__ long long probe_find(const ull* __restrict__ keys,
                                                int64_t n_buckets, ull k) {
  const int64_t mask = n_buckets - 1;
  int64_t b = (int64_t)(k & (ull)mask);
  for (int p = 0; p < PA_PROBE_BUCKETS; ++p) {
    const int64_t base = ((b + p) & mask) * PA_BUCKET_SIZE;
#pragma unroll
    for (int s = 0; s < PA_BUCKET_SIZE; ++s) {
      if (keys[base + s] == k) return base + s;
    }
  }
  return -1;
}

__global__ void probe_claim_kernel(ull* __restrict__ table_keys,
                                   unsigned* __restrict__ ticks,
                                   const ull* __restrict__ query,
                                   int64_t n, int64_t n_buckets, int train,
                                   unsigned tick, float admit_prob,
                                   long long* __restrict__ out_slot,
                                   int* __restrict__ out_new,
                                   ull* __restrict__ evict_keys,
                                   int* __restrict__ evict_count,
                                   long long* __restrict__ out_evict_idx,
                                   const long long* __restrict__ n_dev) {
  if (n_dev) n = *n_dev;
  const int64_t i = (int64_t)blockIdx.x * blockDim.x + threadIdx.x;
  if (i >= n) return;
  const ull k = query[i];
  if (k == PA_EMPTY_KEY) {
    out_slot[i] = -1;
    out_new[i] = 0;
    if (out_evict_idx) out_evict_idx[i] = -1;
    return;
  }
  long long slot;
  int is_new = 0;
  ull victim = 0;
  if (train) {
    bool admitted = true;
    if (admit_prob < 1.0f) {
      const double u = pa_u01(pa_splitmix64(k ^ (ull)tick));
      admitted = u < (double)admit_prob;
    }
    if (admitted) {
      slot = probe_claim(table_keys, ticks, n_buckets, k, tick, &is_new,
                         evict_keys ? &victim : nullptr);
    } else {
      slot = probe_find(table_keys, n_buckets, k);
    }
  } else {
    slot = probe_find(table_keys, n_buckets, k);
  }
  if (slot >= 0) ticks[slot] = tick;
  out_slot[i] = slot;
  out_new[i] = is_new;
  long long eidx = -1;
  if (evict_keys && victim != 0) {
    eidx = (long long)atomicAdd(evict_count, 1);
    evict_keys[eidx] = victim;
  }
  if (out_evict_idx) out_evict_idx[i] = eidx;
}

__device__ __forceinline__ void pa_store_out(float v, float* p) { *p = v; }
__device__ __forceinline__ void pa_store_out(float v, __half* p) {
  *p = __float2half(v);
}
template <typename OutT>
__global__ void init_gather_kernel(float* __restrict__ arena,
                                   const ull* __restrict__ query,
                                   const long long* __restrict__ slots,
                                   const int* __restrict__ is_new,
                                   OutT* __restrict__ out, int64_t n, int dim,
                                   int row_width, double lo, double hi,
                                   float state_init,
                                   const long long* __restrict__ evict_idx,
                                   float* __restrict__ evict_rows,
                                   const long long* __restrict__ n_dev) {
  if (n_dev) n = *n_dev;
  const int wave = threadIdx.x / PA_WAVE;
  const int lane = threadIdx.x % PA_WAVE;
  const int waves_per_block = blockDim.x / PA_WAVE;
  const PaLanes L = pa_lanes(lane, dim);
  const int c0 = L.c0, st = L.st;
  const int64_t n_waveitems = (n + L.G - 1) / L.G;
  for (int64_t w = (int64_t)blockIdx.x * waves_per_block + wave;
       w < n_waveitems; w += (int64_t)gridDim.x * waves_per_block) {
    const int64_t i = w * L.G + L.sub;
    if (i >= n) continue;
    const long long slot = slots[i];
    OutT* dst = out + i * dim;
    if (slot < 0) {
      for (int c = c0; c < dim; c += st) pa_store_out(0.0f, dst + c);
      continue;
    }
    float* row = arena + (int64_t)slot * row_width;
    if (evict_rows && is_new[i] && evict_idx[i] >= 0) {
      float* spill = evict_rows + evict_idx[i] * row_width;
      for (int c = c0; c < row_width; c += st) spill[c] = row[c];
    }
    if (is_new[i])
      pa_init_row(row, query[i], dim, row_width, lo, hi, state_init, c0, st);
    for (int c = c0; c < dim; c += st) pa_store_out(row[c], dst + c);
  }
}

__global__ void init_scatter_kernel(float* __restrict__ arena,
                                    const ull* __restrict__ query,
                                    const long long* __restrict__ slots,
                                    const int* __restrict__ is_new,
                                    const int64_t* __restrict__ perm,
                                    const int64_t* __restrict__ ustarts,
                                    __half* __restrict__ sums, int64_t n,
                                    int dim, int row_width, double lo,
                                    double hi, float state_init,
                                    const long long* __restrict__ n_dev) {
  if (n_dev) n = *n_dev;
  const int wave = threadIdx.x / PA_WAVE;
  const int lane = threadIdx.x % PA_WAVE;
  const int waves_per_block = blockDim.x / PA_WAVE;
  const PaLanes L = pa_lanes(lane, dim);
  const int c0 = L.c0, st = L.st;
  const int64_t n_waveitems = (n + L.G - 1) / L.G;
  for (int64_t w = (int64_t)blockIdx.x * waves_per_block + wave;
       w < n_waveitems; w += (int64_t)gridDim.x * waves_per_block) {
    const int64_t i = w * L.G + L.sub;
    if (i >= n) continue;
    const long long slot = slots[i];
    const int64_t lo_p = ustarts[i], hi_p = ustarts[i + 1];
    if (slot < 0) {
      for (int64_t p = lo_p; p < hi_p; ++p) {
        __half* dst = sums + perm[p] * dim;
        for (int c = c0; c < dim; c += st) dst[c] = __float2half(0.0f);
      }
      continue;
    }
    float* row = arena + (int64_t)slot * row_width;
    if (is_new[i])
      pa_init_row(row, query[i], dim, row_width, lo, hi, state_init, c0, st);
    for (int64_t p = lo_p; p < hi_p; ++p) {
      __half* dst = sums + perm[p] * dim;
      for (int c = c0; c < dim; c += st) dst[c] = __float2half(row[c]);
    }
  }
}

__global__ void init_scatter2_kernel(float* __restrict__ arena,
                                     const ull* __restrict__ query,
                                     const long long* __restrict__ slots,
                                     const int* __restrict__ is_new,
                                     const int64_t* __restrict__ perm,
                                     const int64_t* __restrict__ ustarts,
                                     __half* __restrict__ sums, int64_t n,
                                     int dim, int row_width, double lo,
                                     double hi, float state_init,
                                     const long long* __restrict__ n_dev) {
  if (n_dev) n = *n_dev;
  const int wave = threadIdx.x / PA_WAVE;
  const int lane = threadIdx.x % PA_WAVE;
  const int waves_per_block = blockDim.x / PA_WAVE;
  const int64_t n_waveitems = (n + 1) / 2;
  for (int64_t w = (int64_t)blockIdx.x * waves_per_block + wave;
       w < n_waveitems; w += (int64_t)gridDim.x * waves_per_block) {
    const int64_t iA = w * 2, iB = w * 2 + 1;
    const bool okB0 = iB < n;
    const long long slotA = slots[iA];
    const long long slotB = okB0 ? slots[iB] : -1;
    if (is_new[iA] && slotA >= 0)
      pa_init_row(arena + (int64_t)slotA * row_width, query[iA], dim,
                  row_width, lo, hi, state_init, lane, PA_WAVE);
    if (okB0 && is_new[iB] && slotB >= 0)
      pa_init_row(arena + (int64_t)slotB * row_width, query[iB], dim,
                  row_width, lo, hi, state_init, lane, PA_WAVE);
    const int64_t loA = ustarts[iA], hiA = ustarts[iA + 1];
    const int64_t loB = okB0 ? ustarts[iB] : 0;
    const int64_t hiB = okB0 ? ustarts[iB + 1] : 0;
    const float* rowA = slotA >= 0 ? arena + (int64_t)slotA * row_width : nullptr;
    const float* rowB = slotB >= 0 ? arena + (int64_t)slotB * row_width : nullptr;
    if (hiA - loA == 1 && hiB - loB == 1) {
      __half* dstA = sums + perm[loA] * dim;
      __half* dstB = sums + perm[loB] * dim;
      for (int c = lane; c < dim; c += PA_WAVE) {
        const float vA = rowA ? rowA[c] : 0.0f;
        const float vB = rowB ? rowB[c] : 0.0f;
        dstA[c] = __float2half(vA);
        dstB[c] = __float2half(vB);
      }
    } else {
      for (int64_t p = loA; p < hiA; ++p) {
        __half* dst = sums + perm[p] * dim;
        for (int c = lane; c < dim; c += PA_WAVE)
          dst[c] = __float2half(rowA ? rowA[c] : 0.0f);
      }
      for (int64_t p = loB; p < hiB; ++p) {
        __half* dst = sums + perm[p] * dim;
        for (int c = lane; c < dim; c += PA_WAVE)
          dst[c] = __float2half(rowB ? rowB[c] : 0.0f);
      }
    }
  }
}


__global__ void update_kernel(ull* __restrict__ table_keys,
                              unsigned* __restrict__ ticks,
                              float* __restrict__ arena,
                              const ull* __restrict__ query,
                              const float* __restrict__ grads, int64_t n,
                              int dim, int row_width, int64_t n_buckets,
                              int opt, float p0, float p1, float p2, float p3,
                              float b1_power, float b2_power,
                              float weight_bound,
                              int* __restrict__ skipped) {
  const int wave = threadIdx.x / PA_WAVE;
  const int lane = threadIdx.x % PA_WAVE;
  const int waves_per_block = blockDim.x / PA_WAVE;
  const int64_t mask = n_buckets - 1;
  const PaOptArgs oa =
      pa_opt_args(opt, p0, p1, p2, p3, b1_power, b2_power, weight_bound);
  for (int64_t i = (int64_t)blockIdx.x * waves_per_block + wave; i < n;
       i += (int64_t)gridDim.x * waves_per_block) {
    const ull k = query[i];
    if (k == PA_EMPTY_KEY) continue;
    long long slot = -1;
    const int64_t b = (int64_t)(k & (ull)mask);
    if (lane < PA_PROBE_BUCKETS * PA_BUCKET_SIZE) {
      const int p = lane / PA_BUCKET_SIZE;
      const int s = lane % PA_BUCKET_SIZE;
      const int64_t j = ((b + p) & mask) * PA_BUCKET_SIZE + s;
      if (table_keys[j] == k) slot = j;
    }
    const unsigned long long found = __ballot(slot >= 0);
    if (found == 0) {
      if (lane == 0) atomicAdd(&skipped[0], 1);
      continue;
    }
    const int src = __ffsll((long long)found) - 1;
    slot = __shfl(slot, src);
    float* row = arena + (int64_t)slot * row_width;
    const float* g = grads + i * dim;
    bool has_nan = false;
    for (int c = lane; c < dim; c += PA_WAVE) has_nan |= isnan(g[c]);
    if (__ballot(has_nan) != 0) {
      if (lane == 0) atomicAdd(&skipped[1], 1);
      continue;
    }
    if (opt == 0) {
      for (int c = lane; c < dim; c += PA_WAVE)
        row[c] = pa_sgd(oa, row[c], g[c]);
    } else if (opt == 1) {
      if (pa_adagrad_shared(oa)) {
        const float acc = row[dim];
        float gsq = 0.0f;
        for (int c = lane; c < dim; c += PA_WAVE) {
          row[c] = pa_adagrad_w(oa, row[c], acc, g[c]);
          gsq += g[c] * g[c];
        }
#pragma unroll
        for (int off = PA_WAVE / 2; off > 0; off >>= 1)
          gsq += __shfl_down(gsq, off);
        if (lane == 0) row[dim] = pa_adagrad_shared_acc(oa, acc, gsq, dim);
      } else {
        for (int c = lane; c < dim; c += PA_WAVE) {
          const float acc = row[dim + c];
          row[c] = pa_adagrad_w(oa, row[c], acc, g[c]);
          row[dim + c] = pa_adagrad_acc(oa, acc, g[c]);
        }
      }
    } else {
      for (int c = lane; c < dim; c += PA_WAVE) {
        const float m = pa_adam_m(oa, row[dim + c], g[c]);
        const float v = pa_adam_v(oa, row[2 * dim + c], g[c]);
        row[c] = pa_adam_w(oa, row[c], m, v);
        row[dim + c] = m;
        row[2 * dim + c] = v;
      }
    }
  }
}


__global__ void sign_prep_kernel(const ull* __restrict__ values,
                                 const int64_t* __restrict__ slot_starts,
                                 const ull* __restrict__ prefixes, int n_slots,
                                 ull spacing, ull* __restrict__ out,
                                 int64_t n) {
  const int64_t i = (int64_t)blockIdx.x * blockDim.x + threadIdx.x;
  if (i >= n) return;
  int lo = 0, hi = n_slots;
  while (hi - lo > 1) {
    const int mid = (lo + hi) >> 1;
    if (i >= slot_starts[mid]) lo = mid; else hi = mid;
  }
  const ull prefix = prefixes[lo];
  ull sign = values[i];
  if (prefix != 0) sign = sign % spacing + prefix;
  ull k = pa_splitmix64(sign);
  if (k == PA_EMPTY_KEY) k = 0xD1B54A32D192ED03ull;
  out[i] = k;
}

__global__ void sign_prep_stack_kernel(
    const ull* __restrict__ values, const int64_t* __restrict__ in_starts,
    const int64_t* __restrict__ out_starts, const ull* __restrict__ prefixes,
    const int* __restrict__ rounds, const int64_t* __restrict__ sizes,
    const int64_t* __restrict__ off_starts,
    const int64_t* __restrict__ all_offs,
    int n_slots, ull spacing, ull* __restrict__ out, int64_t n_in) {
  const int64_t i = (int64_t)blockIdx.x * blockDim.x + threadIdx.x;
  if (i >= n_in) return;
  int lo = 0, hi = n_slots;
  while (hi - lo > 1) {
    const int mid = (lo + hi) >> 1;
    if (i >= in_starts[mid]) lo = mid; else hi = mid;
  }
  const int s = lo;
  const ull prefix = prefixes[s];
  const int R = rounds[s];
  if (R == 0) {
    ull sign = values[i];
    if (prefix != 0) sign = sign % spacing + prefix;
    ull k = pa_splitmix64(sign);
    if (k == PA_EMPTY_KEY) k = 0xD1B54A32D192ED03ull;
    out[out_starts[s] + (i - in_starts[s])] = k;
    return;
  }
  const int64_t j = i - in_starts[s];
  const int64_t* E = all_offs + off_starts[s];
  const int64_t nE = off_starts[s + 1] - off_starts[s];
  const int64_t key = j * (int64_t)R;
  int64_t blo = 0, bhi = nE - 1;
  while (bhi - blo > 1) {
    const int64_t mid = (blo + bhi) >> 1;
    if (key >= E[mid]) blo = mid; else bhi = mid;
  }
  const int64_t seg_lo = E[blo] / R, seg_hi = E[blo + 1] / R;
  const int64_t base = out_starts[s] + E[blo];
  const int64_t size = sizes[s];
  ull h = values[i];
  for (int r = 0; r < R; ++r) {
    h = pa_splitmix64(h);
    ull sign = h % (ull)size + (ull)((int64_t)r * size);
    if (prefix != 0) sign = sign % spacing + prefix;
    ull k = pa_splitmix64(sign);
    if (k == PA_EMPTY_KEY) k = 0xD1B54A32D192ED03ull;
    out[base + (int64_t)r * (seg_hi - seg_lo) + (j - seg_lo)] = k;
  }
}

__global__ void a2a_bounds_kernel(const ull* __restrict__ uniq,
                                  const long long* __restrict__ n_dev,
                                  long long n_pad, int world,
                                  long long* __restrict__ starts) {
  const long long n = n_dev ? *n_dev : n_pad;
  const int r = threadIdx.x;
  if (r > world) return;
  if (r == 0) { starts[0] = 0; return; }
  if (r == world) { starts[world] = n; return; }
  const ull hi_min =
      (ull)((((unsigned __int128)r << 32) + (ull)world - 1) / (ull)world);
  const ull thresh = hi_min << 32;
  long long lo = 0, hi = n;
  while (lo < hi) {
    const long long mid = (lo + hi) >> 1;
    if (uniq[mid] < thresh) lo = mid + 1; else hi = mid;
  }
  starts[r] = lo;
}

__global__ void a2a_scatter_kernel(const ull* __restrict__ uniq,
                                   const long long* __restrict__ n_dev,
                                   long long n_pad,
                                   const long long* __restrict__ starts,
                                   int world, long long cap,
                                   ull* __restrict__ send,
                                   int64_t* __restrict__ idx,
                                   long long* __restrict__ overflow) {
  const long long n = n_dev ? *n_dev : n_pad;
  const long long i = (long long)blockIdx.x * blockDim.x + threadIdx.x;
  if (i >= n_pad) return;
  const long long dummy = (long long)world * cap;
  if (i >= n) {
    idx[i] = dummy;
    return;
  }
  const ull k = uniq[i];
  const int o = (int)(((k >> 32) * (ull)world) >> 32);
  const long long pos = i - starts[o];
  long long d = dummy;
  if (pos < cap) {
    d = (long long)o * cap + pos;
    send[d] = k;
  } else {
    atomicAdd((unsigned long long*)overflow, 1ull);
  }
  idx[i] = d;
}

__global__ void iota_i64_kernel(int64_t* __restrict__ out, int64_t n) {
  const int64_t i = (int64_t)blockIdx.x * blockDim.x + threadIdx.x;
  if (i < n) out[i] = i;
}

__global__ void neq_flags_kernel(const ull* __restrict__ sorted,
                                 bool* __restrict__ flags, int64_t n) {
  const int64_t i = (int64_t)blockIdx.x * blockDim.x + threadIdx.x;
  if (i >= n) return;
  flags[i] = (i == 0) || (sorted[i] != sorted[i - 1]);
}

__global__ void dedup_finalize_kernel(
    const ull* __restrict__ svals_flipped, const int64_t* __restrict__ perm,
    const bool* __restrict__ neq, const int64_t* __restrict__ rank,
    int64_t n, ull flip, int64_t* __restrict__ inverse,
    ull* __restrict__ uniq, int64_t* __restrict__ ustarts,
    long long* __restrict__ u_count) {
  const int64_t i = (int64_t)blockIdx.x * blockDim.x + threadIdx.x;
  if (i >= n) return;
  const int64_t r = rank[i];
  inverse[perm[i]] = r;
  if (neq[i]) {
    uniq[r] = svals_flipped[i] ^ flip;
    ustarts[r] = i;
  }
  if (i == n - 1) {
    u_count[0] = r + 1;
    ustarts[r + 1] = n;
  }
}


__global__ void import_kernel(ull* __restrict__ table_keys,
                              unsigned* __restrict__ ticks,
                              float* __restrict__ arena,
                              const ull* __restrict__ query,
                              const float* __restrict__ rows, int64_t n,
                              int row_width, int64_t n_buckets, unsigned tick,
                              ull* __restrict__ evict_keys,
                              int* __restrict__ evict_count,
                              float* __restrict__ evict_rows) {
  const int64_t i = (int64_t)blockIdx.x * blockDim.x + threadIdx.x;
  if (i >= n) return;
  int is_new;
  ull victim = 0;
  const long long slot =
      probe_claim(table_keys, ticks, n_buckets, query[i], tick, &is_new,
                  evict_keys ? &victim : nullptr);
  if (slot < 0) return;
  ticks[slot] = tick;
  float* dst = arena + (int64_t)slot * row_width;
  if (evict_keys && victim != 0) {
    const long long eidx = (long long)atomicAdd(evict_count, 1);
    evict_keys[eidx] = victim;
    float* spill = evict_rows + eidx * row_width;
    for (int c = 0; c < row_width; ++c) spill[c] = dst[c];
  }
  const float* src = rows + i * row_width;
  for (int c = 0; c < row_width; ++c) dst[c] = src[c];
}


template <typename RowT>
__global__ void segment_sum_kernel(const RowT* __restrict__ rows,
                                   const int64_t* __restrict__ inverse,
                                   const int64_t* __restrict__ seg_offsets,
                                   const float* __restrict__ seg_scale,
                                   __half* __restrict__ out, int64_t n_seg,
                                   int dim) {
  const int wave = threadIdx.x / PA_WAVE;
  const int lane = threadIdx.x % PA_WAVE;
  const int waves_per_block = blockDim.x / PA_WAVE;
  const PaLanes L = pa_lanes(lane, dim);
  const int64_t n_waveitems = (n_seg + L.G - 1) / L.G;
  for (int64_t w = (int64_t)blockIdx.x * waves_per_block + wave;
       w < n_waveitems; w += (int64_t)gridDim.x * waves_per_block) {
    const int64_t s = w * L.G + L.sub;
    if (s >= n_seg) continue;
    const int64_t lo = seg_offsets[s], hi = seg_offsets[s + 1];
    const float scale = seg_scale ? seg_scale[s] : 1.0f;
    __half* dst = out + s * dim;
    for (int c = L.c0; c < dim; c += L.st) {
      float acc = 0.0f;
      for (int64_t k = lo; k < hi; ++k) {
        acc += pa_to_float(rows[inverse[k] * dim + c]);
      }
      dst[c] = __float2half(acc * scale);
    }
  }
}


template <typename GradT, bool ACCUMULATE>
__global__ void grad_scatter_kernel(const GradT* __restrict__ grads,
                                    const int64_t* __restrict__ perm,
                                    const int64_t* __restrict__ ustarts,
                                    const int64_t* __restrict__ seg_id,
                                    const float* __restrict__ seg_scale,
                                    float* __restrict__ out, int64_t n_unique,
                                    int dim) {
  const int wave = threadIdx.x / PA_WAVE;
  const int lane = threadIdx.x % PA_WAVE;
  const int waves_per_block = blockDim.x / PA_WAVE;
  for (int64_t u = (int64_t)blockIdx.x * waves_per_block + wave; u < n_unique;
       u += (int64_t)gridDim.x * waves_per_block) {
    const int64_t lo = ustarts[u], hi = ustarts[u + 1];
    float* dst = out + u * dim;
    for (int c = lane; c < dim; c += PA_WAVE) {
      float acc[1] = {0.0f};
      pa_reduce_positions<1>(acc, grads, perm, seg_id, seg_scale, lo, hi, dim, c,
                          PA_WAVE);
      if (ACCUMULATE) dst[c] += acc[0]; else dst[c] = acc[0];
    }
  }
}

template <typename OutT>
__global__ void grad_scatter_idx_kernel(
    const __half* __restrict__ grads, const int64_t* __restrict__ perm,
    const int64_t* __restrict__ ustarts, const int64_t* __restrict__ seg_id,
    const float* __restrict__ seg_scale, const int64_t* __restrict__ out_idx,
    OutT* __restrict__ out, int64_t n_unique, int dim,
    const long long* __restrict__ n_dev) {
  if (n_dev) n_unique = *n_dev;
  const int wave = threadIdx.x / PA_WAVE;
  const int lane = threadIdx.x % PA_WAVE;
  const int waves_per_block = blockDim.x / PA_WAVE;
  const PaLanes L = pa_lanes(lane, dim);
  const int64_t n_waveitems = (n_unique + L.G - 1) / L.G;
  for (int64_t w = (int64_t)blockIdx.x * waves_per_block + wave;
       w < n_waveitems; w += (int64_t)gridDim.x * waves_per_block) {
    const int64_t u = w * L.G + L.sub;
    if (u >= n_unique) continue;
    const int64_t lo = ustarts[u], hi = ustarts[u + 1];
    OutT* dst = out + out_idx[u] * dim;
    for (int c = L.c0; c < dim; c += L.st) {
      float acc[1] = {0.0f};
      pa_reduce_positions<1>(acc, grads, perm, seg_id, seg_scale, lo, hi, dim, c,
                          L.st);
      pa_store_out(acc[0], dst + c);
    }
  }
}


__global__ void scatter_update_kernel(
    ull* __restrict__ table_keys, unsigned* __restrict__ ticks,
    float* __restrict__ arena, const ull* __restrict__ uniq,
    const __half* __restrict__ grads, const int64_t* __restrict__ perm,
    const int64_t* __restrict__ ustarts, const int64_t* __restrict__ seg_id,
    const float* __restrict__ seg_scale, int64_t n, int dim, int row_width,
    int64_t n_buckets, int opt, float p0, float p1, float p2, float p3,
    float b1_power, float b2_power, float weight_bound,
    int* __restrict__ skipped, const long long* __restrict__ n_dev) {
  if (n_dev) n = *n_dev;
  const int wave = threadIdx.x / PA_WAVE;
  const int lane = threadIdx.x % PA_WAVE;
  const int waves_per_block = blockDim.x / PA_WAVE;
  const int64_t mask = n_buckets - 1;
  const PaOptArgs oa =
      pa_opt_args(opt, p0, p1, p2, p3, b1_power, b2_power, weight_bound);
  const PaLanes L = pa_lanes(lane, dim);
  const int G = L.G, sub = L.sub, c0 = L.c0, st = L.st;
  const int sg = L.st;
  const ull sg_mask = (sg >= 64) ? ~0ull : ((1ull << sg) - 1ull);
  const int64_t n_waveitems = (n + G - 1) / G;
  constexpr int WINDOW = PA_PROBE_BUCKETS * PA_BUCKET_SIZE;
  for (int64_t w = (int64_t)blockIdx.x * waves_per_block + wave;
       w < n_waveitems; w += (int64_t)gridDim.x * waves_per_block) {
    const int64_t u = w * G + sub;
    const ull k = (u < n) ? uniq[u] : 0;
    const bool active = (u < n) && (k != PA_EMPTY_KEY);
    long long slot = -1;
    if (active) {
      const int64_t b = (int64_t)(k & (ull)mask);
      for (int it = 0; it * sg + c0 < WINDOW; ++it) {
        const int widx = it * sg + c0;
        const int p = widx / PA_BUCKET_SIZE;
        const int s = widx % PA_BUCKET_SIZE;
        const int64_t j = ((b + p) & mask) * PA_BUCKET_SIZE + s;
        if (table_keys[j] == k) slot = j;
      }
    }
    const unsigned long long found = __ballot(slot >= 0);
    const unsigned long long sub_found = (found >> (sub * sg)) & sg_mask;
    bool ok = active;
    if (ok && sub_found == 0) {
      if (c0 == 0) atomicAdd(&skipped[0], 1);
      ok = false;
    }
    if (ok)
      slot = __shfl(slot, sub * sg + __ffsll((long long)sub_found) - 1);
    float acc[8];
#pragma unroll
    for (int t = 0; t < 8; ++t) acc[t] = 0.0f;
    if (ok)
      pa_reduce_positions<8>(acc, grads, perm, seg_id, seg_scale, ustarts[u],
                          ustarts[u + 1], dim, c0, st);
    bool has_nan = false;
    if (ok)
      for (int t = 0, c = c0; c < dim; c += st, ++t) has_nan |= isnan(acc[t]);
    const unsigned long long nanb = __ballot(has_nan);
    if (ok && ((nanb >> (sub * sg)) & sg_mask) != 0) {
      if (c0 == 0) atomicAdd(&skipped[1], 1);
      ok = false;
    }
    if (!ok) continue;
    float* row = arena + (int64_t)slot * row_width;
    if (opt == 0) {
      for (int t = 0, c = c0; c < dim; c += st, ++t) {
        const float w0 = __builtin_nontemporal_load(&row[c]);
        __builtin_nontemporal_store(pa_sgd(oa, w0, acc[t]), &row[c]);
      }
    } else if (opt == 1) {
      if (pa_adagrad_shared(oa)) {
        const float a0 = row[dim];
        float gsq = 0.0f;
        for (int t = 0, c = c0; c < dim; c += st, ++t) {
          const float w0 = __builtin_nontemporal_load(&row[c]);
          __builtin_nontemporal_store(pa_adagrad_w(oa, w0, a0, acc[t]), &row[c]);
          gsq += acc[t] * acc[t];
        }
        for (int off = sg / 2; off > 0; off >>= 1)
          gsq += __shfl_down(gsq, off, sg);
        if (c0 == 0) row[dim] = pa_adagrad_shared_acc(oa, a0, gsq, dim);
      } else {
        for (int t = 0, c = c0; c < dim; c += st, ++t) {
          const float a0 = __builtin_nontemporal_load(&row[dim + c]);
          const float w0 = __builtin_nontemporal_load(&row[c]);
          __builtin_nontemporal_store(pa_adagrad_w(oa, w0, a0, acc[t]), &row[c]);
          __builtin_nontemporal_store(pa_adagrad_acc(oa, a0, acc[t]), &row[dim + c]);
        }
      }
    } else {
      for (int t = 0, c = c0; c < dim; c += st, ++t) {
        const float m = pa_adam_m(
            oa, __builtin_nontemporal_load(&row[dim + c]), acc[t]);
        const float v = pa_adam_v(
            oa, __builtin_nontemporal_load(&row[2 * dim + c]), acc[t]);
        const float w0 = __builtin_nontemporal_load(&row[c]);
        __builtin_nontemporal_store(pa_adam_w(oa, w0, m, v), &row[c]);
        __builtin_nontemporal_store(m, &row[dim + c]);
        __builtin_nontemporal_store(v, &row[2 * dim + c]);
      }
    }
  }
}

template <int T>
using PaAccVec = float __attribute__((ext_vector_type(T)));

template <int Q>
__global__ void scatter_update_multi_kernel(
    ull* __restrict__ table_keys, unsigned* __restrict__ ticks,
    float* __restrict__ arena, const ull* __restrict__ uniq,
    const __half* __restrict__ grads, const int64_t* __restrict__ perm,
    const int64_t* __restrict__ ustarts, const int64_t* __restrict__ seg_id,
    const float* __restrict__ seg_scale, int64_t n, int dim, int row_width,
    int64_t n_buckets, int opt, float p0, float p1, float p2, float p3,
    float b1_power, float b2_power, float weight_bound,
    int* __restrict__ skipped, const long long* __restrict__ n_dev) {
  static_assert(Q == 2 || Q == 4, "two or four keys per wave");
  constexpr int WINDOW = PA_PROBE_BUCKETS * PA_BUCKET_SIZE;
  constexpr int PL = PA_WAVE / Q;
  constexpr int WS = WINDOW / PL;
  constexpr int T = 8 / Q;
  constexpr ull PL_MASK = (1ull << PL) - 1ull;
  if (n_dev) n = *n_dev;
  const int wave = threadIdx.x / PA_WAVE;
  const int lane = threadIdx.x % PA_WAVE;
  const int waves_per_block = blockDim.x / PA_WAVE;
  const int64_t mask = n_buckets - 1;
  const PaOptArgs oa =
      pa_opt_args(opt, p0, p1, p2, p3, b1_power, b2_power, weight_bound);
  const int kq = lane / PL;
  const int widx = lane % PL;
  const int64_t n_waveitems = (n + Q - 1) / Q;
  for (int64_t w = (int64_t)blockIdx.x * waves_per_block + wave;
       w < n_waveitems; w += (int64_t)gridDim.x * waves_per_block) {
    const int64_t u = w * Q + kq;
    const ull k = (u < n) ? uniq[u] : 0;
    const bool active = (u < n) && (k != PA_EMPTY_KEY);
    long long slot = -1;
    if (active) {
      const int64_t b = (int64_t)(k & (ull)mask);
#pragma unroll
      for (int h = 0; h < WS; ++h) {
        const int wi = widx + h * PL;
        const int p = wi / PA_BUCKET_SIZE;
        const int s = wi % PA_BUCKET_SIZE;
        const int64_t j = ((b + p) & mask) * PA_BUCKET_SIZE + s;
        if (table_keys[j] == k) slot = j;
      }
    }
    const unsigned long long found = __ballot(slot >= 0);
    const unsigned long long nonzero = __ballot(k != PA_EMPTY_KEY);
    bool ok[Q];
    float* rowk[Q];
#pragma unroll
    for (int q = 0; q < Q; ++q) {
      const unsigned fq = (unsigned)((found >> (PL * q)) & PL_MASK);
      ok[q] = (w * Q + q) < n && (nonzero >> (PL * q) & 1ull);
      if (ok[q] && fq == 0) {
        if (lane == 0) atomicAdd(&skipped[0], 1);
        ok[q] = false;
      }
      const long long slotq = ok[q] ? __shfl(slot, PL * q + __ffs(fq) - 1) : -1;
      rowk[q] = ok[q] ? arena + (int64_t)slotq * row_width : nullptr;
    }
    PaAccVec<T> acc[Q];
#pragma unroll
    for (int q = 0; q < Q; ++q) acc[q] = 0.0f;
    int64_t lop[Q], hip[Q];
    bool all_single = true;
#pragma unroll
    for (int q = 0; q < Q; ++q) {
      lop[q] = ok[q] ? ustarts[w * Q + q] : 0;
      hip[q] = ok[q] ? ustarts[w * Q + q + 1] : 0;
      all_single = all_single && ok[q] && hip[q] - lop[q] == 1;
    }
    if (all_single) {
      const __half* gq[Q];
      float scq[Q];
#pragma unroll
      for (int q = 0; q < Q; ++q) {
        const int64_t s = seg_id[perm[lop[q]]];
        scq[q] = (s >= 0) ? (seg_scale ? seg_scale[s] : 1.0f) : 0.0f;
        gq[q] = grads + (s >= 0 ? s : 0) * dim;
      }
      for (int t = 0, c = lane; c < dim; c += PA_WAVE, ++t) {
#pragma unroll
        for (int q = 0; q < Q; ++q) {
          const float g = __half2float(gq[q][c]);
          acc[q][t] = (scq[q] != 0.0f) ? scq[q] * g : 0.0f;
        }
      }
    } else {
#pragma unroll
      for (int q = 0; q < Q; ++q)
        if (ok[q])
          pa_reduce_positions<T>(acc[q], grads, perm, seg_id, seg_scale,
                                 lop[q], hip[q], dim, lane, PA_WAVE);
    }
#pragma unroll
    for (int q = 0; q < Q; ++q) {
      bool has_nan = false;
      for (int t = 0, c = lane; c < dim; c += PA_WAVE, ++t)
        has_nan |= isnan(acc[q][t]);
      if (ok[q] && __ballot(has_nan) != 0) {
        if (lane == 0) atomicAdd(&skipped[1], 1);
        ok[q] = false;
      }
    }
    bool any_ok = false;
#pragma unroll
    for (int q = 0; q < Q; ++q) any_ok = any_ok || ok[q];
    if (!any_ok) continue;
    if (opt == 0) {
      for (int t = 0, c = lane; c < dim; c += PA_WAVE, ++t) {
        float w0[Q];
#pragma unroll
        for (int q = 0; q < Q; ++q)
          w0[q] = ok[q] ? __builtin_nontemporal_load(&rowk[q][c]) : 0.0f;
#pragma unroll
        for (int q = 0; q < Q; ++q) {
          if (!ok[q]) continue;
          __builtin_nontemporal_store(pa_sgd(oa, w0[q], acc[q][t]), &rowk[q][c]);
        }
      }
    } else if (opt == 1) {
      if (pa_adagrad_shared(oa)) {
        float a0[Q], gsq[Q] = {};
#pragma unroll
        for (int q = 0; q < Q; ++q) a0[q] = ok[q] ? rowk[q][dim] : 0.0f;
        for (int t = 0, c = lane; c < dim; c += PA_WAVE, ++t) {
          float w0[Q];
#pragma unroll
          for (int q = 0; q < Q; ++q)
            w0[q] = ok[q] ? __builtin_nontemporal_load(&rowk[q][c]) : 0.0f;
#pragma unroll
          for (int q = 0; q < Q; ++q) {
            if (!ok[q]) continue;
            __builtin_nontemporal_store(
                pa_adagrad_w(oa, w0[q], a0[q], acc[q][t]), &rowk[q][c]);
            gsq[q] += acc[q][t] * acc[q][t];
          }
        }
#pragma unroll
        for (int off = PA_WAVE / 2; off > 0; off >>= 1)
#pragma unroll
          for (int q = 0; q < Q; ++q) gsq[q] += __shfl_down(gsq[q], off);
        if (lane == 0)
#pragma unroll
          for (int q = 0; q < Q; ++q)
            if (ok[q])
              rowk[q][dim] = pa_adagrad_shared_acc(oa, a0[q], gsq[q], dim);
      } else {
        for (int t = 0, c = lane; c < dim; c += PA_WAVE, ++t) {
          float w0[Q], a0[Q];
#pragma unroll
          for (int q = 0; q < Q; ++q) {
            a0[q] = ok[q] ? __builtin_nontemporal_load(&rowk[q][dim + c]) : 0.0f;
            w0[q] = ok[q] ? __builtin_nontemporal_load(&rowk[q][c]) : 0.0f;
          }
#pragma unroll
          for (int q = 0; q < Q; ++q) {
            if (!ok[q]) continue;
            __builtin_nontemporal_store(
                pa_adagrad_w(oa, w0[q], a0[q], acc[q][t]), &rowk[q][c]);
            __builtin_nontemporal_store(pa_adagrad_acc(oa, a0[q], acc[q][t]),
                                        &rowk[q][dim + c]);
          }
        }
      }
    } else {
      for (int t = 0, c = lane; c < dim; c += PA_WAVE, ++t) {
#pragma unroll
        for (int q = 0; q < Q; ++q) {
          if (!ok[q]) continue;
          const float m = pa_adam_m(
              oa, __builtin_nontemporal_load(&rowk[q][dim + c]), acc[q][t]);
          const float v = pa_adam_v(
              oa, __builtin_nontemporal_load(&rowk[q][2 * dim + c]), acc[q][t]);
          const float w0 = __builtin_nontemporal_load(&rowk[q][c]);
          __builtin_nontemporal_store(pa_adam_w(oa, w0, m, v), &rowk[q][c]);
          __builtin_nontemporal_store(m, &rowk[q][dim + c]);
          __builtin_nontemporal_store(v, &rowk[q][2 * dim + c]);
        }
      }
    }
  }
}

inline int n_blocks_for(int64_t work_items, int per_block) {
  int64_t b = (work_items + per_block - 1) / per_block;
  if (b > 16384) b = 16384;
  if (b < 1) b = 1;
  return (int)b;
}

}


static hipStream_t cur_stream() {
  return at::hip::getCurrentHIPStream().stream();
}

static const long long* count_or_null(const torch::Tensor& u_count) {
  return u_count.numel() ? (const long long*)u_count.data_ptr<int64_t>()
                         : nullptr;
}
static const float* scale_or_null(const torch::Tensor& seg_scale) {
  return seg_scale.numel() ? seg_scale.data_ptr<float>() : nullptr;
}

std::vector<torch::Tensor> sort_pairs_u64(torch::Tensor keys) {
  const int64_t n = keys.numel();
  auto opts = torch::TensorOptions().dtype(torch::kInt64).device(keys.device());
  auto iota = torch::empty({n}, opts);
  auto sorted = torch::empty_like(keys);
  auto perm = torch::empty({n}, opts);
  if (n == 0) return {sorted, perm};
  hipStream_t st = cur_stream();
  hipLaunchKernelGGL(iota_i64_kernel, dim3(n_blocks_for(n, 256)), dim3(256),
                     0, st, iota.data_ptr<int64_t>(), n);
  size_t temp_bytes = 0;
  hipcub::DeviceRadixSort::SortPairs(
      nullptr, temp_bytes, (const ull*)keys.data_ptr<int64_t>(),
      (ull*)sorted.data_ptr<int64_t>(),
      (const long long*)iota.data_ptr<int64_t>(),
      (long long*)perm.data_ptr<int64_t>(), n, 0, 64, st);
  auto temp = torch::empty(
      {(int64_t)temp_bytes},
      torch::TensorOptions().dtype(torch::kUInt8).device(keys.device()));
  hipcub::DeviceRadixSort::SortPairs(
      temp.data_ptr(), temp_bytes, (const ull*)keys.data_ptr<int64_t>(),
      (ull*)sorted.data_ptr<int64_t>(),
      (const long long*)iota.data_ptr<int64_t>(),
      (long long*)perm.data_ptr<int64_t>(), n, 0, 64, st);
  return {sorted, perm};
}

torch::Tensor neq_flags(torch::Tensor sorted) {
  const int64_t n = sorted.numel();
  auto flags = torch::empty(
      {n}, torch::TensorOptions().dtype(torch::kBool).device(sorted.device()));
  if (n == 0) return flags;
  hipLaunchKernelGGL(neq_flags_kernel, dim3(n_blocks_for(n, 256)), dim3(256),
                     0, cur_stream(), (const ull*)sorted.data_ptr<int64_t>(),
                     flags.data_ptr<bool>(), n);
  return flags;
}


void store_lookup(torch::Tensor table_keys, torch::Tensor ticks,
                  torch::Tensor arena, torch::Tensor query, torch::Tensor out,
                  int64_t dim, int64_t train, int64_t tick, double lo,
                  double hi, double admit_prob, double state_init,
                  int64_t opt_space, torch::Tensor evict_keys,
                  torch::Tensor evict_count, torch::Tensor evict_rows,
                  torch::Tensor u_count) {
  const int64_t n = query.numel();
  if (n == 0) return;
  const int64_t n_buckets = table_keys.numel() / PA_BUCKET_SIZE;
  const int row_width = (int)(dim + opt_space);
  const bool spill = evict_keys.numel() > 0;
  const long long* n_dev = count_or_null(u_count);
  auto opts = torch::TensorOptions().dtype(torch::kInt64).device(query.device());
  auto slots = torch::empty({n}, opts);
  auto is_new = torch::empty({n}, opts.dtype(torch::kInt32));
  torch::Tensor evict_idx;
  if (spill) evict_idx = torch::empty({n}, opts);
  hipStream_t st = cur_stream();
  hipLaunchKernelGGL(probe_claim_kernel, dim3(n_blocks_for(n, 256)), dim3(256),
                     0, st, (ull*)table_keys.data_ptr<int64_t>(),
                     (unsigned*)ticks.data_ptr<int32_t>(),
                     (const ull*)query.data_ptr<int64_t>(), n, n_buckets,
                     (int)train, (unsigned)tick, (float)admit_prob,
                     (long long*)slots.data_ptr<int64_t>(),
                     is_new.data_ptr<int32_t>(),
                     spill ? (ull*)evict_keys.data_ptr<int64_t>() : nullptr,
                     spill ? evict_count.data_ptr<int32_t>() : nullptr,
                     spill ? (long long*)evict_idx.data_ptr<int64_t>() : nullptr,
                     n_dev);
  if (out.scalar_type() == torch::kFloat16) {
    hipLaunchKernelGGL(init_gather_kernel<__half>, dim3(n_blocks_for(n, 4)),
                       dim3(256), 0, st, arena.data_ptr<float>(),
                       (const ull*)query.data_ptr<int64_t>(),
                       (const long long*)slots.data_ptr<int64_t>(),
                       is_new.data_ptr<int32_t>(),
                       (__half*)out.data_ptr<at::Half>(), n, (int)dim,
                       row_width, lo, hi, (float)state_init,
                       spill ? (const long long*)evict_idx.data_ptr<int64_t>() : nullptr,
                       spill ? evict_rows.data_ptr<float>() : nullptr, n_dev);
  } else {
    hipLaunchKernelGGL(init_gather_kernel<float>, dim3(n_blocks_for(n, 4)),
                       dim3(256), 0, st, arena.data_ptr<float>(),
                       (const ull*)query.data_ptr<int64_t>(),
                       (const long long*)slots.data_ptr<int64_t>(),
                       is_new.data_ptr<int32_t>(), out.data_ptr<float>(), n,
                       (int)dim, row_width, lo, hi, (float)state_init,
                       spill ? (const long long*)evict_idx.data_ptr<int64_t>() : nullptr,
                       spill ? evict_rows.data_ptr<float>() : nullptr, n_dev);
  }
}

void store_lookup_sums(torch::Tensor table_keys, torch::Tensor ticks,
                       torch::Tensor arena, torch::Tensor query,
                       torch::Tensor perm, torch::Tensor ustarts,
                       torch::Tensor sums, int64_t dim, int64_t train,
                       int64_t tick, double lo, double hi, double admit_prob,
                       double state_init, int64_t opt_space,
                       torch::Tensor u_count) {
  const int64_t n = query.numel();
  if (n == 0) return;
  const int64_t n_buckets = table_keys.numel() / PA_BUCKET_SIZE;
  const int row_width = (int)(dim + opt_space);
  const long long* n_dev = count_or_null(u_count);
  auto opts = torch::TensorOptions().dtype(torch::kInt64).device(query.device());
  auto slots = torch::empty({n}, opts);
  auto is_new = torch::empty({n}, opts.dtype(torch::kInt32));
  hipStream_t st = cur_stream();
  hipLaunchKernelGGL(probe_claim_kernel, dim3(n_blocks_for(n, 256)), dim3(256),
                     0, st, (ull*)table_keys.data_ptr<int64_t>(),
                     (unsigned*)ticks.data_ptr<int32_t>(),
                     (const ull*)query.data_ptr<int64_t>(), n, n_buckets,
                     (int)train, (unsigned)tick, (float)admit_prob,
                     (long long*)slots.data_ptr<int64_t>(),
                     is_new.data_ptr<int32_t>(), nullptr, nullptr, nullptr,
                     n_dev);
  const bool dual = !(dim < PA_WAVE && (PA_WAVE % dim) == 0);
  if (dual) {
    hipLaunchKernelGGL(init_scatter2_kernel,
                       dim3(n_blocks_for((n + 1) / 2, 4)), dim3(256), 0, st,
                       arena.data_ptr<float>(),
                       (const ull*)query.data_ptr<int64_t>(),
                       (const long long*)slots.data_ptr<int64_t>(),
                       is_new.data_ptr<int32_t>(), perm.data_ptr<int64_t>(),
                       ustarts.data_ptr<int64_t>(),
                       (__half*)sums.data_ptr<at::Half>(), n, (int)dim,
                       row_width, lo, hi, (float)state_init, n_dev);
  } else {
    hipLaunchKernelGGL(init_scatter_kernel, dim3(n_blocks_for(n, 4)),
                       dim3(256), 0, st, arena.data_ptr<float>(),
                       (const ull*)query.data_ptr<int64_t>(),
                       (const long long*)slots.data_ptr<int64_t>(),
                       is_new.data_ptr<int32_t>(), perm.data_ptr<int64_t>(),
                       ustarts.data_ptr<int64_t>(),
                       (__half*)sums.data_ptr<at::Half>(), n, (int)dim,
                       row_width, lo, hi, (float)state_init, n_dev);
  }
}

torch::Tensor store_probe(torch::Tensor table_keys, torch::Tensor ticks,
                          torch::Tensor query, int64_t tick,
                          torch::Tensor u_count) {
  const int64_t n = query.numel();
  auto opts = torch::TensorOptions().dtype(torch::kInt64).device(query.device());
  auto slots = u_count.numel() ? torch::zeros({n}, opts) : torch::empty({n}, opts);
  if (n == 0) return slots;
  auto is_new = torch::empty({n}, opts.dtype(torch::kInt32));
  const int64_t n_buckets = table_keys.numel() / PA_BUCKET_SIZE;
  hipLaunchKernelGGL(probe_claim_kernel, dim3(n_blocks_for(n, 256)), dim3(256),
                     0, cur_stream(), (ull*)table_keys.data_ptr<int64_t>(),
                     (unsigned*)ticks.data_ptr<int32_t>(),
                     (const ull*)query.data_ptr<int64_t>(), n, n_buckets,
                     0, (unsigned)tick, 1.0f,
                     (long long*)slots.data_ptr<int64_t>(),
                     is_new.data_ptr<int32_t>(), nullptr, nullptr, nullptr,
                     count_or_null(u_count));
  return slots;
}

void store_update(torch::Tensor table_keys, torch::Tensor ticks,
                  torch::Tensor arena, torch::Tensor query,
                  torch::Tensor grads, int64_t dim, int64_t opt,
                  std::vector<double> params, double b1_power,
                  double b2_power, double weight_bound,
                  torch::Tensor skipped ) {
  const int64_t n = query.numel();
  if (n == 0) return;
  const int64_t n_buckets = table_keys.numel() / PA_BUCKET_SIZE;
  const int row_width = (int)arena.size(1);
  hipStream_t st = cur_stream();
  hipLaunchKernelGGL(update_kernel, dim3(n_blocks_for(n, 4)), dim3(256), 0, st,
                     (ull*)table_keys.data_ptr<int64_t>(),
                     (unsigned*)ticks.data_ptr<int32_t>(),
                     arena.data_ptr<float>(),
                     (const ull*)query.data_ptr<int64_t>(),
                     grads.data_ptr<float>(), n, (int)dim, row_width,
                     n_buckets, (int)opt, (float)params[0], (float)params[1],
                     (float)params[2], (float)params[3], (float)b1_power,
                     (float)b2_power, (float)weight_bound,
                     skipped.data_ptr<int32_t>());
}

void store_import(torch::Tensor table_keys, torch::Tensor ticks,
                  torch::Tensor arena, torch::Tensor query, torch::Tensor rows,
                  int64_t tick, torch::Tensor evict_keys,
                  torch::Tensor evict_count, torch::Tensor evict_rows) {
  const int64_t n = query.numel();
  if (n == 0) return;
  const int64_t n_buckets = table_keys.numel() / PA_BUCKET_SIZE;
  const bool spill = evict_keys.numel() > 0;
  hipLaunchKernelGGL(import_kernel, dim3(n_blocks_for(n, 256)), dim3(256), 0,
                     cur_stream(), (ull*)table_keys.data_ptr<int64_t>(),
                     (unsigned*)ticks.data_ptr<int32_t>(),
                     arena.data_ptr<float>(),
                     (const ull*)query.data_ptr<int64_t>(),
                     rows.data_ptr<float>(), n, (int)rows.size(1), n_buckets,
                     (unsigned)tick,
                     spill ? (ull*)evict_keys.data_ptr<int64_t>() : nullptr,
                     spill ? evict_count.data_ptr<int32_t>() : nullptr,
                     spill ? evict_rows.data_ptr<float>() : nullptr);
}

torch::Tensor segment_sum(torch::Tensor rows, torch::Tensor inverse,
                          torch::Tensor seg_offsets, torch::Tensor seg_scale) {
  const int64_t n_seg = seg_offsets.numel() - 1;
  const int64_t dim = rows.size(1);
  auto out = torch::empty(
      {n_seg, dim},
      torch::TensorOptions().dtype(torch::kFloat16).device(rows.device()));
  if (n_seg == 0) return out;
  const float* scale_ptr = scale_or_null(seg_scale);
  hipStream_t st = cur_stream();
  const dim3 grid(n_blocks_for(n_seg, 4)), block(256);
  if (rows.scalar_type() == torch::kFloat32) {
    hipLaunchKernelGGL(segment_sum_kernel<float>, grid, block, 0, st,
                       rows.data_ptr<float>(), inverse.data_ptr<int64_t>(),
                       seg_offsets.data_ptr<int64_t>(), scale_ptr,
                       (__half*)out.data_ptr<at::Half>(), n_seg, (int)dim);
  } else if (rows.scalar_type() == torch::kFloat16) {
    hipLaunchKernelGGL(segment_sum_kernel<__half>, grid, block, 0, st,
                       (const __half*)rows.data_ptr<at::Half>(),
                       inverse.data_ptr<int64_t>(),
                       seg_offsets.data_ptr<int64_t>(), scale_ptr,
                       (__half*)out.data_ptr<at::Half>(), n_seg, (int)dim);
  } else {
    TORCH_CHECK(false, "segment_sum: rows must be f32 or f16");
  }
  return out;
}

void grad_scatter(torch::Tensor grads, torch::Tensor perm,
                  torch::Tensor ustarts, torch::Tensor seg_id,
                  torch::Tensor seg_scale, torch::Tensor out,
                  int64_t accumulate) {
  const int64_t n_unique = ustarts.numel() - 1;
  const int64_t dim = out.size(1);
  if (n_unique == 0) return;
  hipStream_t st = cur_stream();
  const dim3 grid(n_blocks_for(n_unique, 4)), block(256);
  const float* scale_ptr = scale_or_null(seg_scale);
#define PA_GS(T, ACC)                                                         \
  hipLaunchKernelGGL((grad_scatter_kernel<T, ACC>), grid, block, 0, st,       \
                     (const T*)grads.data_ptr(), perm.data_ptr<int64_t>(),    \
                     ustarts.data_ptr<int64_t>(), seg_id.data_ptr<int64_t>(), \
                     scale_ptr, out.data_ptr<float>(),                        \
                     n_unique, (int)dim)
  if (grads.scalar_type() == torch::kFloat16) {
    if (accumulate) PA_GS(__half, true); else PA_GS(__half, false);
  } else if (grads.scalar_type() == torch::kFloat32) {
    if (accumulate) PA_GS(float, true); else PA_GS(float, false);
  } else if (grads.scalar_type() == torch::kBFloat16) {
    if (accumulate) PA_GS(__hip_bfloat16, true); else PA_GS(__hip_bfloat16, false);
  } else {
    TORCH_CHECK(false, "grad_scatter: grads must be f16/bf16/f32");
  }
#undef PA_GS
}

void grad_scatter_idx(torch::Tensor grads, torch::Tensor perm,
                      torch::Tensor ustarts, torch::Tensor seg_id,
                      torch::Tensor seg_scale, torch::Tensor out_idx,
                      torch::Tensor out, torch::Tensor u_count) {
  const int64_t n_unique = out_idx.numel();
  const int64_t dim = out.size(1);
  if (n_unique == 0) return;
  TORCH_CHECK(grads.scalar_type() == torch::kFloat16,
              "grad_scatter_idx: f16 grads");
  hipStream_t st = cur_stream();
  const dim3 grid(n_blocks_for(n_unique, 4)), block(256);
  const float* scale_ptr = scale_or_null(seg_scale);
  const long long* n_dev = count_or_null(u_count);
  if (out.scalar_type() == torch::kFloat16) {
    hipLaunchKernelGGL(grad_scatter_idx_kernel<__half>, grid, block, 0, st,
                       (const __half*)grads.data_ptr<at::Half>(),
                       perm.data_ptr<int64_t>(), ustarts.data_ptr<int64_t>(),
                       seg_id.data_ptr<int64_t>(), scale_ptr,
                       out_idx.data_ptr<int64_t>(),
                       (__half*)out.data_ptr<at::Half>(), n_unique, (int)dim,
                       n_dev);
  } else if (out.scalar_type() == torch::kFloat32) {
    hipLaunchKernelGGL(grad_scatter_idx_kernel<float>, grid, block, 0, st,
                       (const __half*)grads.data_ptr<at::Half>(),
                       perm.data_ptr<int64_t>(), ustarts.data_ptr<int64_t>(),
                       seg_id.data_ptr<int64_t>(), scale_ptr,
                       out_idx.data_ptr<int64_t>(),
                       out.data_ptr<float>(), n_unique, (int)dim, n_dev);
  } else {
    TORCH_CHECK(false, "grad_scatter_idx: out must be f16/f32");
  }
}

void scatter_update(torch::Tensor table_keys, torch::Tensor ticks,
                    torch::Tensor arena, torch::Tensor uniq,
                    torch::Tensor grads, torch::Tensor perm,
                    torch::Tensor ustarts, torch::Tensor seg_id,
                    torch::Tensor seg_scale, int64_t dim, int64_t opt,
                    std::vector<double> params, double b1_power,
                    double b2_power, double weight_bound,
                    torch::Tensor skipped, torch::Tensor u_count) {
  const int64_t n = uniq.numel();
  if (n == 0) return;
  TORCH_CHECK(grads.scalar_type() == torch::kFloat16, "scatter_update: f16 grads");
  TORCH_CHECK(dim <= 8 * PA_WAVE, "scatter_update: dim too large");
  const int64_t n_buckets = table_keys.numel() / PA_BUCKET_SIZE;
  const int row_width = (int)arena.size(1);
  auto launch = [&](auto kernel, int keys_per_wave) {
    const int64_t waves = (n + keys_per_wave - 1) / keys_per_wave;
    hipLaunchKernelGGL(kernel, dim3(n_blocks_for(waves, 4)), dim3(256), 0,
                       cur_stream(), (ull*)table_keys.data_ptr<int64_t>(),
                       (unsigned*)ticks.data_ptr<int32_t>(),
                       arena.data_ptr<float>(),
                       (const ull*)uniq.data_ptr<int64_t>(),
                       (const __half*)grads.data_ptr<at::Half>(),
                       perm.data_ptr<int64_t>(), ustarts.data_ptr<int64_t>(),
                       seg_id.data_ptr<int64_t>(), scale_or_null(seg_scale), n,
                       (int)dim, row_width, n_buckets, (int)opt,
                       (float)params[0], (float)params[1], (float)params[2],
                       (float)params[3], (float)b1_power, (float)b2_power,
                       (float)weight_bound, skipped.data_ptr<int32_t>(),
                       count_or_null(u_count));
  };
  const bool packed_small = (dim < PA_WAVE && (PA_WAVE % dim) == 0);
  if (!packed_small && dim <= 128)
    launch(scatter_update_multi_kernel<4>, 4);
  else if (!packed_small && dim <= 256)
    launch(scatter_update_multi_kernel<2>, 2);
  else
    launch(scatter_update_kernel, 1);
}

std::vector<torch::Tensor> a2a_route(torch::Tensor uniq, torch::Tensor u_count,
                                     int64_t world, int64_t cap,
                                     torch::Tensor overflow) {
  const int64_t n_pad = uniq.numel();
  auto opts = torch::TensorOptions().dtype(torch::kInt64).device(uniq.device());
  auto send = torch::zeros({world * cap + 1}, opts);
  auto idx = torch::empty({n_pad}, opts);
  auto starts = torch::empty({world + 1}, opts);
  hipStream_t st = cur_stream();
  const long long* n_dev = count_or_null(u_count);
  hipLaunchKernelGGL(a2a_bounds_kernel, dim3(1), dim3(world + 1), 0, st,
                     (const ull*)uniq.data_ptr<int64_t>(), n_dev, n_pad,
                     (int)world, (long long*)starts.data_ptr<int64_t>());
  if (n_pad)
    hipLaunchKernelGGL(a2a_scatter_kernel, dim3(n_blocks_for(n_pad, 256)),
                       dim3(256), 0, st, (const ull*)uniq.data_ptr<int64_t>(),
                       n_dev, n_pad,
                       (const long long*)starts.data_ptr<int64_t>(), (int)world,
                       cap, (ull*)send.data_ptr<int64_t>(),
                       idx.data_ptr<int64_t>(),
                       (long long*)overflow.data_ptr<int64_t>());
  return {send, idx};
}

torch::Tensor sign_prep(torch::Tensor values, torch::Tensor slot_starts,
                        torch::Tensor prefixes, int64_t spacing) {
  const int64_t n = values.numel();
  auto out = torch::empty_like(values);
  if (n == 0) return out;
  hipLaunchKernelGGL(sign_prep_kernel, dim3(n_blocks_for(n, 256)), dim3(256),
                     0, cur_stream(), (const ull*)values.data_ptr<int64_t>(),
                     slot_starts.data_ptr<int64_t>(),
                     (const ull*)prefixes.data_ptr<int64_t>(),
                     (int)(slot_starts.numel() - 1), (ull)spacing,
                     (ull*)out.data_ptr<int64_t>(), n);
  return out;
}

void dedup_finalize(torch::Tensor svals_flipped, torch::Tensor perm,
                    torch::Tensor neq, torch::Tensor rank, int64_t flip,
                    torch::Tensor inverse, torch::Tensor uniq,
                    torch::Tensor ustarts, torch::Tensor u_count) {
  const int64_t n = svals_flipped.numel();
  if (n == 0) return;
  hipLaunchKernelGGL(dedup_finalize_kernel, dim3(n_blocks_for(n, 256)),
                     dim3(256), 0, cur_stream(),
                     (const ull*)svals_flipped.data_ptr<int64_t>(),
                     perm.data_ptr<int64_t>(), neq.data_ptr<bool>(),
                     rank.data_ptr<int64_t>(), n, (ull)flip,
                     inverse.data_ptr<int64_t>(),
                     (ull*)uniq.data_ptr<int64_t>(),
                     ustarts.data_ptr<int64_t>(),
                     (long long*)u_count.data_ptr<int64_t>());
}

torch::Tensor sign_prep_stack(torch::Tensor values, torch::Tensor in_starts,
                              torch::Tensor out_starts, torch::Tensor prefixes,
                              torch::Tensor rounds, torch::Tensor sizes,
                              torch::Tensor off_starts, torch::Tensor all_offs,
                              int64_t spacing, int64_t n_out) {
  const int64_t n_in = values.numel();
  auto out = torch::empty({n_out}, values.options());
  if (n_in == 0) return out;
  hipLaunchKernelGGL(sign_prep_stack_kernel, dim3(n_blocks_for(n_in, 256)),
                     dim3(256), 0, cur_stream(),
                     (const ull*)values.data_ptr<int64_t>(),
                     in_starts.data_ptr<int64_t>(),
                     out_starts.data_ptr<int64_t>(),
                     (const ull*)prefixes.data_ptr<int64_t>(),
                     rounds.data_ptr<int32_t>(), sizes.data_ptr<int64_t>(),
                     off_starts.data_ptr<int64_t>(),
                     all_offs.data_ptr<int64_t>(),
                     (int)(in_starts.numel() - 1), (ull)spacing,
                     (ull*)out.data_ptr<int64_t>(), n_in);
  return out;
}

void init_dense(pybind11::module_& m);
void init_engine(pybind11::module_& m);
void init_interact(pybind11::module_& m);
void init_checkpoint(pybind11::module_& m);

PYBIND11_MODULE(TORCH_EXTENSION_NAME, m) {
  m.doc() = "persia_amd HIP kernels (gfx950)";
  init_dense(m);
  init_engine(m);
  init_interact(m);
  init_checkpoint(m);
  m.def("store_lookup", &store_lookup, "hash-table lookup/insert + gather");
  m.def("store_probe", &store_probe, "probe-only (spill-tier miss detection)");
  m.def("store_lookup_sums", &store_lookup_sums,
        "fast-path lookup: probe + fused init/f16 scatter to sum rows");
  m.def("store_update", &store_update, "fused sparse optimizer update");
  m.def("store_import", &store_import, "bulk insert rows (checkpoint load)");
  m.def("segment_sum", &segment_sum, "fused gather + per-sample summation");
  m.def("grad_scatter", &grad_scatter, "ordered per-sign gradient scatter");
  m.def("grad_scatter_idx", &grad_scatter_idx,
        "ordered per-sign gradient scatter packed into the a2a send layout");
  m.def("sign_prep", &sign_prep, "prefix-fold + splitmix64 key mixing");
  m.def("sign_prep_stack", &sign_prep_stack,
        "hashstack expansion + prefix-fold + splitmix64 key mixing");
  m.def("dedup_finalize", &dedup_finalize,
        "fixed-shape dedup epilogue (padded uniq/ustarts + device count)");
  m.def("sort_pairs_u64", &sort_pairs_u64, "radix sort-pairs, u64 order");
  m.def("a2a_route", &a2a_route,
        "padded-a2a key routing: range-partition bounds + packed scatter");
  m.def("neq_flags", &neq_flags, "sorted-run boundary flags");
  m.def("scatter_update", &scatter_update,
        "fused ordered grad scatter + optimizer update (no [U,dim] buffer)");
}
```

persia_amd/csrc/optim.h:

```cpp
#pragma once

#include <hip/hip_runtime.h>
#include <hip/hip_bf16.h>
#include <hip/hip_fp16.h>
#include <cstdint>

#include "common.h"

__device__ __forceinline__ float pa_to_float(float x) { return x; }
__device__ __forceinline__ float pa_to_float(__half x) { return __half2float(x); }
__device__ __forceinline__ float pa_to_float(__hip_bfloat16 x) {
  return __bfloat162float(x);
}

struct PaOptArgs {
  int opt;
  float p0, p1, p2, p3;
  float weight_bound;
  float om1, om2, c1, c2;
};

__device__ __forceinline__ PaOptArgs pa_opt_args(int opt, float p0, float p1,
                                                 float p2, float p3,
                                                 float b1_power, float b2_power,
                                                 float weight_bound) {
  PaOptArgs a;
  a.opt = opt;
  a.p0 = p0; a.p1 = p1; a.p2 = p2; a.p3 = p3;
  a.weight_bound = weight_bound;
  a.om1 = 1.0f - p1;
  a.om2 = 1.0f - p2;
  a.c1 = 1.0f / (1.0f - b1_power);
  a.c2 = 1.0f / (1.0f - b2_power);
  return a;
}

__device__ __forceinline__ bool pa_adagrad_shared(const PaOptArgs& a) {
  return a.p3 > 0.5f;
}

__device__ __forceinline__ float pa_clamp_weight(const PaOptArgs& a, float w) {
  if (a.weight_bound > 0.0f) w = fminf(fmaxf(w, -a.weight_bound), a.weight_bound);
  return w;
}

__device__ __forceinline__ float pa_sgd(const PaOptArgs& a, float w, float g) {
  return pa_clamp_weight(a, w - a.p0 * (g + a.p1 * w));
}

__device__ __forceinline__ float pa_adagrad_w(const PaOptArgs& a, float w,
                                              float acc, float g) {
  return pa_clamp_weight(a, w - a.p0 * g * rsqrtf(acc + a.p2));
}

__device__ __forceinline__ float pa_adagrad_acc(const PaOptArgs& a, float acc,
                                                float g) {
  return acc * a.p1 + g * g;
}

__device__ __forceinline__ float pa_adagrad_shared_acc(const PaOptArgs& a,
                                                       float acc, float gsq,
                                                       int dim) {
  return acc * a.p1 + gsq / (float)dim;
}

__device__ __forceinline__ float pa_adam_m(const PaOptArgs& a, float m, float g) {
  return a.p1 * m + a.om1 * g;
}
__device__ __forceinline__ float pa_adam_v(const PaOptArgs& a, float v, float g) {
  return a.p2 * v + a.om2 * g * g;
}
__device__ __forceinline__ float pa_adam_w(const PaOptArgs& a, float w, float m,
                                           float v) {
  return pa_clamp_weight(a, w - a.p0 * (m * a.c1) / (a.p3 + sqrtf(v * a.c2)));
}

template <int T, typename AccT, typename GradT>
__device__ __forceinline__ void pa_reduce_positions(
    AccT& acc, const GradT* __restrict__ grads,
    const int64_t* __restrict__ perm, const int64_t* __restrict__ seg_id,
    const float* __restrict__ seg_scale, int64_t lo, int64_t hi, int dim,
    int c0, int st) {
  for (int64_t p = lo; p < hi; ++p) {
    const int64_t s = seg_id[perm[p]];
    if (s < 0) continue;
    const float sc = seg_scale ? seg_scale[s] : 1.0f;
    if (sc == 0.0f) continue;
    const GradT* g = grads + s * dim;
    if constexpr (T == 1) {
      acc[0] += pa_to_float(g[c0]) * sc;
    } else {
      for (int t = 0, c = c0; c < dim; c += st, ++t)
        acc[t] += pa_to_float(g[c]) * sc;
    }
  }
}
```

Measured before the change: 7.908 million samples/s.

## Pass lookup slot and single-source grad hints to fused scatter update

During the training lookup, the probe kernel now records each unique key's table slot and, for keys that occur exactly once, its gradient source segment. These are passed to the fused scatter-update kernel, which checks the cached slot against the stored key and can skip the hash-bucket probe and the perm/seg_id indirection walk. The gradient row is also prefetched before the probe resolves. The row load/store helpers are restructured and the adagrad accumulator uses an FMA. The cost is extra int64 hint buffers, extra writes in the probe kernel, and reliance on slots staying valid between lookup and update, which is guarded by a key equality check.

Measured after the change: 8.067 million samples/s, median of 6. 1.02x the previous value.

```diff
diff --git a/persia_amd/core/engine.py b/persia_amd/core/engine.py
--- a/persia_amd/core/engine.py
+++ b/persia_amd/core/engine.py
@@ -139,6 +139,8 @@
     perm: torch.Tensor
     ustarts: torch.Tensor
     u_count: Optional[torch.Tensor] = None
+    slot_hint: Optional[torch.Tensor] = None
+    src_hint: Optional[torch.Tensor] = None
     slots: List[_SlotCtx] = field(default_factory=list)
     cat_offsets: Optional[torch.Tensor] = None
     seg_id: Optional[torch.Tensor] = None
@@ -256,7 +258,8 @@
         for g in self._groups:
             a2a_owner = g.a2a_owner_dedup or ()
             for t in (g.uniq_keys, g.inverse, g.perm, g.ustarts, g.u_count,
-                      g.sum_base, g.cat_offsets, g.seg_id, g.seg_lens,
+                      g.slot_hint, g.src_hint, g.sum_base, g.cat_offsets,
+                      g.seg_id, g.seg_lens,
                       g.sqrt_mask, g.a2a_idx, g.a2a_recv_keys, *a2a_owner):
                 if t is not None and t.is_cuda:
                     yield t
@@ -311,6 +314,7 @@
         self.nan_grad_batches = 0
         self._plans = {}
         self._empty_scale = torch.empty(0, dtype=torch.float32, device=device)
+        self._no_seg = torch.empty(0, dtype=torch.int64, device=device)
         spacing = schema.feature_spacing
         self._spacing_arg = spacing if spacing < (1 << 63) else -1
         self.model_manager_status = "Idle"
@@ -321,6 +325,7 @@
                     "skip": 20}
         self._fused_dist = os.environ.get("PA_FUSED_DIST", "1") == "1"
         self._force_dist = os.environ.get("PA_FORCE_DIST", "0") == "1"
+        self._update_hints = os.environ.get("PA_UPDATE_HINTS", "1") != "0"
         self._roctx = os.environ.get("PA_ROCTX", "0") == "1"
         self._a2a_overflow = torch.zeros(1, dtype=torch.int64, device=device)
         from persia_amd.core.metrics import EngineMetrics
@@ -723,10 +728,13 @@
         if one_call:
             if timing:
                 t0 = self._tick("prep", t0)
-            sums, uniq, inverse, perm, ustarts, u_count = store.lookup_local(
+            (sums, uniq, inverse, perm, ustarts, u_count, slot_hint,
+             src_hint) = store.lookup_local(
                 self._upload_group(dim, feats, batch), plan.slot_starts,
                 plan.prefixes, self._spacing_arg, plan.cat_offsets,
-                plan.empty_scale, train,
+                plan.empty_scale,
+                plan.seg_id if train and self._update_hints else self._no_seg,
+                train,
             )
         else:
             ps = cur = None
@@ -754,6 +762,9 @@
             cat_offsets=plan.cat_offsets, seg_id=plan.seg_id,
             n_sum_slots=plan.S,
         )
+        if one_call:
+            if slot_hint.numel():
+                group.slot_hint, group.src_hint = slot_hint, src_hint
         if padded:
             if timing:
                 t = self._tick("dedup", t0)
@@ -1174,6 +1185,7 @@
                         store.update_local(
                             gbase, group.perm, group.ustarts, group.seg_id,
                             seg_scale, group.uniq_keys, group.u_count,
+                            group.slot_hint, group.src_hint,
                         )
                         if self.incremental is not None:
                             self.incremental.record_keys(
diff --git a/persia_amd/core/store.py b/persia_amd/core/store.py
--- a/persia_amd/core/store.py
+++ b/persia_amd/core/store.py
@@ -592,19 +592,24 @@
     def lookup_local(self, values: torch.Tensor, slot_starts: torch.Tensor,
                      prefixes: torch.Tensor, spacing_arg: int,
                      cat_offsets: torch.Tensor, seg_scale: torch.Tensor,
-                     train: bool):
+                     seg_id: torch.Tensor, train: bool):
         return self._C.lookup_local(
             values, slot_starts, prefixes, spacing_arg, cat_offsets, seg_scale,
-            self.keys, self.ticks, self.arena,
+            seg_id, self.keys, self.ticks, self.arena,
             *self._lookup_args(train, self.next_tick()),
         )
 
     def update_local(self, gbase, perm, ustarts, seg_id, seg_scale, uniq,
-                     u_count: Optional[torch.Tensor]) -> None:
+                     u_count: Optional[torch.Tensor],
+                     slot_hint: Optional[torch.Tensor] = None,
+                     src_hint: Optional[torch.Tensor] = None) -> None:
+        hinted = slot_hint is not None and src_hint is not None
         self._C.update_local(
             gbase.contiguous(), perm, ustarts, seg_id, seg_scale, uniq,
             self.keys, self.ticks, self.arena, *self._update_args(),
             u_count if u_count is not None else self.no_count,
+            slot_hint if hinted else self.no_count,
+            src_hint if hinted else self.no_count,
         )
 
     def scatter_update(self, uniq, grads, perm, ustarts, seg_id,
diff --git a/persia_amd/csrc/engine.cpp b/persia_amd/csrc/engine.cpp
--- a/persia_amd/csrc/engine.cpp
+++ b/persia_amd/csrc/engine.cpp
@@ -7,13 +7,12 @@
                   int64_t opt_space, torch::Tensor evict_keys,
                   torch::Tensor evict_count, torch::Tensor evict_rows,
                   torch::Tensor u_count);
-void store_lookup_sums(torch::Tensor table_keys, torch::Tensor ticks,
-                       torch::Tensor arena, torch::Tensor query,
-                       torch::Tensor perm, torch::Tensor ustarts,
-                       torch::Tensor sums, int64_t dim, int64_t train,
-                       int64_t tick, double lo, double hi, double admit_prob,
-                       double state_init, int64_t opt_space,
-                       torch::Tensor u_count);
+std::vector<torch::Tensor> store_lookup_sums(
+    torch::Tensor table_keys, torch::Tensor ticks, torch::Tensor arena,
+    torch::Tensor query, torch::Tensor perm, torch::Tensor ustarts,
+    torch::Tensor sums, int64_t dim, int64_t train, int64_t tick, double lo,
+    double hi, double admit_prob, double state_init, int64_t opt_space,
+    torch::Tensor u_count, torch::Tensor seg_id);
 void store_update(torch::Tensor table_keys, torch::Tensor ticks,
                   torch::Tensor arena, torch::Tensor query,
                   torch::Tensor grads, int64_t dim, int64_t opt,
@@ -34,7 +33,8 @@
                     torch::Tensor seg_scale, int64_t dim, int64_t opt,
                     std::vector<double> params, double b1_power,
                     double b2_power, double weight_bound,
-                    torch::Tensor skipped, torch::Tensor u_count);
+                    torch::Tensor skipped, torch::Tensor u_count,
+                    torch::Tensor slot_hint, torch::Tensor src_hint);
 void dedup_finalize(torch::Tensor svals_flipped, torch::Tensor perm,
                     torch::Tensor neq, torch::Tensor rank, int64_t flip,
                     torch::Tensor inverse, torch::Tensor uniq,
@@ -89,9 +89,9 @@
 std::vector<torch::Tensor> lookup_local(
     torch::Tensor values, torch::Tensor slot_starts, torch::Tensor prefixes,
     int64_t spacing, torch::Tensor cat_offsets, torch::Tensor seg_scale,
-    torch::Tensor table_keys, torch::Tensor ticks, torch::Tensor arena,
-    int64_t dim, int64_t train, int64_t tick, double lo, double hi,
-    double admit_prob, double state_init, int64_t opt_space) {
+    torch::Tensor seg_id, torch::Tensor table_keys, torch::Tensor ticks,
+    torch::Tensor arena, int64_t dim, int64_t train, int64_t tick, double lo,
+    double hi, double admit_prob, double state_init, int64_t opt_space) {
   auto keys = sign_prep(values, slot_starts, prefixes, spacing);
   auto d = dedup_padded(keys);
   auto& uniq = d[0];
@@ -104,10 +104,10 @@
   auto opts = torch::TensorOptions().dtype(torch::kInt64).device(dev);
   auto sums = torch::empty(
       {nnz, dim}, torch::TensorOptions().dtype(torch::kFloat16).device(dev));
-  store_lookup_sums(table_keys, ticks, arena, uniq, perm, ustarts, sums, dim,
-                    train, tick, lo, hi, admit_prob, state_init, opt_space,
-                    u_count);
-  return {sums, uniq, inverse, perm, ustarts, u_count};
+  auto hints = store_lookup_sums(table_keys, ticks, arena, uniq, perm, ustarts,
+                                 sums, dim, train, tick, lo, hi, admit_prob,
+                                 state_init, opt_space, u_count, seg_id);
+  return {sums, uniq, inverse, perm, ustarts, u_count, hints[0], hints[1]};
 }
 
 void update_local(torch::Tensor grads, torch::Tensor perm,
@@ -117,11 +117,12 @@
                   torch::Tensor arena, int64_t dim, int64_t opt,
                   std::vector<double> params, double b1_power, double b2_power,
                   double weight_bound, torch::Tensor skipped,
-                  torch::Tensor u_count) {
+                  torch::Tensor u_count, torch::Tensor slot_hint,
+                  torch::Tensor src_hint) {
   if (grads.scalar_type() == torch::kFloat16 && dim <= 512) {
     scatter_update(table_keys, ticks, arena, uniq_keys, grads, perm, ustarts,
                    seg_id, seg_scale, dim, opt, params, b1_power, b2_power,
-                   weight_bound, skipped, u_count);
+                   weight_bound, skipped, u_count, slot_hint, src_hint);
     return;
   }
   if (u_count.numel()) {
diff --git a/persia_amd/csrc/kernels.hip b/persia_amd/csrc/kernels.hip
--- a/persia_amd/csrc/kernels.hip
+++ b/persia_amd/csrc/kernels.hip
@@ -49,6 +49,14 @@
   return -1;
 }
 
+__device__ __forceinline__ long long pa_src_hint(
+    const int64_t* __restrict__ perm, const int64_t* __restrict__ seg_id,
+    int64_t lo_p, int64_t hi_p) {
+  if (hi_p - lo_p != 1) return -1;
+  const int64_t s = seg_id[perm[lo_p]];
+  return s >= 0 ? (long long)s : -1;
+}
+
 __global__ void probe_claim_kernel(ull* __restrict__ table_keys,
                                    unsigned* __restrict__ ticks,
                                    const ull* __restrict__ query,
@@ -59,11 +67,17 @@
                                    ull* __restrict__ evict_keys,
                                    int* __restrict__ evict_count,
                                    long long* __restrict__ out_evict_idx,
-                                   const long long* __restrict__ n_dev) {
+                                   const long long* __restrict__ n_dev,
+                                   const int64_t* __restrict__ ustarts,
+                                   const int64_t* __restrict__ perm,
+                                   const int64_t* __restrict__ seg_id,
+                                   long long* __restrict__ src_hint) {
   if (n_dev) n = *n_dev;
   const int64_t i = (int64_t)blockIdx.x * blockDim.x + threadIdx.x;
   if (i >= n) return;
   const ull k = query[i];
+  if (src_hint)
+    src_hint[i] = pa_src_hint(perm, seg_id, ustarts[i], ustarts[i + 1]);
   if (k == PA_EMPTY_KEY) {
     out_slot[i] = -1;
     out_new[i] = 0;
@@ -580,6 +594,7 @@
 }
 
 
+template <bool HINTS>
 __global__ void scatter_update_kernel(
     ull* __restrict__ table_keys, unsigned* __restrict__ ticks,
     float* __restrict__ arena, const ull* __restrict__ uniq,
@@ -588,7 +603,9 @@
     const float* __restrict__ seg_scale, int64_t n, int dim, int row_width,
     int64_t n_buckets, int opt, float p0, float p1, float p2, float p3,
     float b1_power, float b2_power, float weight_bound,
-    int* __restrict__ skipped, const long long* __restrict__ n_dev) {
+    int* __restrict__ skipped, const long long* __restrict__ n_dev,
+    const long long* __restrict__ slot_hint,
+    const long long* __restrict__ src_hint, int64_t n_slots, int64_t n_src) {
   if (n_dev) n = *n_dev;
   const int wave = threadIdx.x / PA_WAVE;
   const int lane = threadIdx.x % PA_WAVE;
@@ -607,8 +624,26 @@
     const int64_t u = w * G + sub;
     const ull k = (u < n) ? uniq[u] : 0;
     const bool active = (u < n) && (k != PA_EMPTY_KEY);
-    long long slot = -1;
-    if (active) {
+    long long sh = -1, sr = -1;
+    if (HINTS && active) {
+      sh = slot_hint[u];
+      sr = src_hint[u];
+    }
+    if (sh < 0 || sh >= n_slots) sh = -1;
+    if (sr < 0 || sr >= n_src) sr = -1;
+    ull kv = PA_EMPTY_KEY;
+    if (sh >= 0) kv = table_keys[sh];
+    float hsc = 0.0f;
+    __half hg[8];
+    if (sr >= 0) {
+      hsc = seg_scale ? seg_scale[sr] : 1.0f;
+      const __half* g = grads + (int64_t)sr * dim;
+#pragma unroll
+      for (int t = 0; t < 8; ++t)
+        if (c0 + t * st < dim) hg[t] = g[c0 + t * st];
+    }
+    long long slot = (sh >= 0 && kv == k) ? sh : -1;
+    if (active && slot < 0) {
       const int64_t b = (int64_t)(k & (ull)mask);
       for (int it = 0; it * sg + c0 < WINDOW; ++it) {
         const int widx = it * sg + c0;
@@ -630,9 +665,18 @@
     float acc[8];
 #pragma unroll
     for (int t = 0; t < 8; ++t) acc[t] = 0.0f;
-    if (ok)
-      pa_reduce_positions<8>(acc, grads, perm, seg_id, seg_scale, ustarts[u],
-                          ustarts[u + 1], dim, c0, st);
+    if (ok) {
+      if (sr >= 0) {
+        if (hsc != 0.0f) {
+#pragma unroll
+          for (int t = 0; t < 8; ++t)
+            if (c0 + t * st < dim) acc[t] += __half2float(hg[t]) * hsc;
+        }
+      } else {
+        pa_reduce_positions<8>(acc, grads, perm, seg_id, seg_scale, ustarts[u],
+                               ustarts[u + 1], dim, c0, st);
+      }
+    }
     bool has_nan = false;
     if (ok)
       for (int t = 0, c = c0; c < dim; c += st, ++t) has_nan |= isnan(acc[t]);
@@ -665,7 +709,8 @@
           const float a0 = __builtin_nontemporal_load(&row[dim + c]);
           const float w0 = __builtin_nontemporal_load(&row[c]);
           __builtin_nontemporal_store(pa_adagrad_w(oa, w0, a0, acc[t]), &row[c]);
-          __builtin_nontemporal_store(pa_adagrad_acc(oa, a0, acc[t]), &row[dim + c]);
+          __builtin_nontemporal_store(pa_adagrad_acc<true>(oa, a0, acc[t]),
+                                      &row[dim + c]);
         }
       }
     } else {
@@ -686,7 +731,207 @@
 template <int T>
 using PaAccVec = float __attribute__((ext_vector_type(T)));
 
-template <int Q>
+using PaGlobalF = __attribute__((address_space(1))) float;
+
+template <int Q, int T>
+struct PaRowRegs {
+  PaAccVec<T> w0[Q], s1[Q], s2[Q];
+  float a0[Q];
+};
+
+template <int Q, int T>
+__device__ __forceinline__ void pa_load_rows(PaRowRegs<Q, T>& r,
+                                             const PaOptArgs& oa,
+                                             const bool (&ok)[Q],
+                                             float* const (&rows)[Q], int dim,
+                                             int lane) {
+  PaGlobalF* rowk[Q];
+#pragma unroll
+  for (int q = 0; q < Q; ++q) rowk[q] = (PaGlobalF*)rows[q];
+  const bool shared = oa.opt == 1 && pa_adagrad_shared(oa);
+#pragma unroll
+  for (int q = 0; q < Q; ++q)
+    r.a0[q] = (shared && ok[q]) ? rowk[q][dim] : 0.0f;
+#pragma unroll
+  for (int t = 0; t < T; ++t) {
+    const int c = lane + t * PA_WAVE;
+    if (c >= dim) continue;
+#pragma unroll
+    for (int q = 0; q < Q; ++q) {
+      if (!ok[q]) continue;
+      if (oa.opt != 0 && !shared)
+        r.s1[q][t] = __builtin_nontemporal_load(&rowk[q][dim + c]);
+      if (oa.opt == 2)
+        r.s2[q][t] = __builtin_nontemporal_load(&rowk[q][2 * dim + c]);
+      r.w0[q][t] = __builtin_nontemporal_load(&rowk[q][c]);
+    }
+  }
+}
+
+template <int Q, int T>
+__device__ __forceinline__ void pa_step_rows(const PaRowRegs<Q, T>& r,
+                                             const PaOptArgs& oa,
+                                             const bool (&ok)[Q],
+                                             float* const (&rows)[Q],
+                                             const PaAccVec<T> (&acc)[Q],
+                                             int dim, int lane) {
+  PaGlobalF* rowk[Q];
+#pragma unroll
+  for (int q = 0; q < Q; ++q) rowk[q] = (PaGlobalF*)rows[q];
+  if (oa.opt == 0) {
+#pragma unroll
+    for (int t = 0; t < T; ++t) {
+      const int c = lane + t * PA_WAVE;
+      if (c >= dim) continue;
+#pragma unroll
+      for (int q = 0; q < Q; ++q) {
+        if (!ok[q]) continue;
+        __builtin_nontemporal_store(pa_sgd(oa, r.w0[q][t], acc[q][t]),
+                                    &rowk[q][c]);
+      }
+    }
+  } else if (oa.opt == 1) {
+    if (pa_adagrad_shared(oa)) {
+      float gsq[Q] = {};
+#pragma unroll
+      for (int t = 0; t < T; ++t) {
+        const int c = lane + t * PA_WAVE;
+        if (c >= dim) continue;
+#pragma unroll
+        for (int q = 0; q < Q; ++q) {
+          if (!ok[q]) continue;
+          __builtin_nontemporal_store(
+              pa_adagrad_w(oa, r.w0[q][t], r.a0[q], acc[q][t]), &rowk[q][c]);
+          gsq[q] += acc[q][t] * acc[q][t];
+        }
+      }
+#pragma unroll
+      for (int off = PA_WAVE / 2; off > 0; off >>= 1)
+#pragma unroll
+        for (int q = 0; q < Q; ++q) gsq[q] += __shfl_down(gsq[q], off);
+      if (lane == 0)
+#pragma unroll
+        for (int q = 0; q < Q; ++q)
+          if (ok[q])
+            rowk[q][dim] = pa_adagrad_shared_acc(oa, r.a0[q], gsq[q], dim);
+    } else {
+#pragma unroll
+      for (int t = 0; t < T; ++t) {
+        const int c = lane + t * PA_WAVE;
+        if (c >= dim) continue;
+#pragma unroll
+        for (int q = 0; q < Q; ++q) {
+          if (!ok[q]) continue;
+          __builtin_nontemporal_store(
+              pa_adagrad_w(oa, r.w0[q][t], r.s1[q][t], acc[q][t]),
+              &rowk[q][c]);
+          __builtin_nontemporal_store(
+              pa_adagrad_acc(oa, r.s1[q][t], acc[q][t]), &rowk[q][dim + c]);
+        }
+      }
+    }
+  } else {
+#pragma unroll
+    for (int t = 0; t < T; ++t) {
+      const int c = lane + t * PA_WAVE;
+      if (c >= dim) continue;
+#pragma unroll
+      for (int q = 0; q < Q; ++q) {
+        if (!ok[q]) continue;
+        const float m = pa_adam_m(oa, r.s1[q][t], acc[q][t]);
+        const float v = pa_adam_v(oa, r.s2[q][t], acc[q][t]);
+        __builtin_nontemporal_store(pa_adam_w(oa, r.w0[q][t], m, v),
+                                    &rowk[q][c]);
+        __builtin_nontemporal_store(m, &rowk[q][dim + c]);
+        __builtin_nontemporal_store(v, &rowk[q][2 * dim + c]);
+      }
+    }
+  }
+}
+
+template <int Q, int T>
+__device__ __forceinline__ void pa_update_rows(const PaOptArgs& oa,
+                                               const bool (&ok)[Q],
+                                               float* const (&rowk)[Q],
+                                               const PaAccVec<T> (&acc)[Q],
+                                               int dim, int lane) {
+  const int opt = oa.opt;
+  if (opt == 0) {
+    for (int t = 0, c = lane; c < dim; c += PA_WAVE, ++t) {
+      float w0[Q];
+#pragma unroll
+      for (int q = 0; q < Q; ++q)
+        w0[q] = ok[q] ? __builtin_nontemporal_load(&rowk[q][c]) : 0.0f;
+#pragma unroll
+      for (int q = 0; q < Q; ++q) {
+        if (!ok[q]) continue;
+        __builtin_nontemporal_store(pa_sgd(oa, w0[q], acc[q][t]), &rowk[q][c]);
+      }
+    }
+  } else if (opt == 1) {
+    if (pa_adagrad_shared(oa)) {
+      float a0[Q], gsq[Q] = {};
+#pragma unroll
+      for (int q = 0; q < Q; ++q) a0[q] = ok[q] ? rowk[q][dim] : 0.0f;
+      for (int t = 0, c = lane; c < dim; c += PA_WAVE, ++t) {
+        float w0[Q];
+#pragma unroll
+        for (int q = 0; q < Q; ++q)
+          w0[q] = ok[q] ? __builtin_nontemporal_load(&rowk[q][c]) : 0.0f;
+#pragma unroll
+        for (int q = 0; q < Q; ++q) {
+          if (!ok[q]) continue;
+          __builtin_nontemporal_store(
+              pa_adagrad_w(oa, w0[q], a0[q], acc[q][t]), &rowk[q][c]);
+          gsq[q] += acc[q][t] * acc[q][t];
+        }
+      }
+#pragma unroll
+      for (int off = PA_WAVE / 2; off > 0; off >>= 1)
+#pragma unroll
+        for (int q = 0; q < Q; ++q) gsq[q] += __shfl_down(gsq[q], off);
+      if (lane == 0)
+#pragma unroll
+        for (int q = 0; q < Q; ++q)
+          if (ok[q])
+            rowk[q][dim] = pa_adagrad_shared_acc(oa, a0[q], gsq[q], dim);
+    } else {
+      for (int t = 0, c = lane; c < dim; c += PA_WAVE, ++t) {
+        float w0[Q], a0[Q];
+#pragma unroll
+        for (int q = 0; q < Q; ++q) {
+          a0[q] = ok[q] ? __builtin_nontemporal_load(&rowk[q][dim + c]) : 0.0f;
+          w0[q] = ok[q] ? __builtin_nontemporal_load(&rowk[q][c]) : 0.0f;
+        }
+#pragma unroll
+        for (int q = 0; q < Q; ++q) {
+          if (!ok[q]) continue;
+          __builtin_nontemporal_store(
+              pa_adagrad_w(oa, w0[q], a0[q], acc[q][t]), &rowk[q][c]);
+          __builtin_nontemporal_store(pa_adagrad_acc(oa, a0[q], acc[q][t]),
+                                      &rowk[q][dim + c]);
+        }
+      }
+    }
+  } else {
+    for (int t = 0, c = lane; c < dim; c += PA_WAVE, ++t) {
+#pragma unroll
+      for (int q = 0; q < Q; ++q) {
+        if (!ok[q]) continue;
+        const float m = pa_adam_m(
+            oa, __builtin_nontemporal_load(&rowk[q][dim + c]), acc[q][t]);
+        const float v = pa_adam_v(
+            oa, __builtin_nontemporal_load(&rowk[q][2 * dim + c]), acc[q][t]);
+        const float w0 = __builtin_nontemporal_load(&rowk[q][c]);
+        __builtin_nontemporal_store(pa_adam_w(oa, w0, m, v), &rowk[q][c]);
+        __builtin_nontemporal_store(m, &rowk[q][dim + c]);
+        __builtin_nontemporal_store(v, &rowk[q][2 * dim + c]);
+      }
+    }
+  }
+}
+
+template <int Q, bool HINTS>
 __global__ void scatter_update_multi_kernel(
     ull* __restrict__ table_keys, unsigned* __restrict__ ticks,
     float* __restrict__ arena, const ull* __restrict__ uniq,
@@ -695,7 +940,9 @@
     const float* __restrict__ seg_scale, int64_t n, int dim, int row_width,
     int64_t n_buckets, int opt, float p0, float p1, float p2, float p3,
     float b1_power, float b2_power, float weight_bound,
-    int* __restrict__ skipped, const long long* __restrict__ n_dev) {
+    int* __restrict__ skipped, const long long* __restrict__ n_dev,
+    const long long* __restrict__ slot_hint,
+    const long long* __restrict__ src_hint, int64_t n_slots, int64_t n_src) {
   static_assert(Q == 2 || Q == 4, "two or four keys per wave");
   constexpr int WINDOW = PA_PROBE_BUCKETS * PA_BUCKET_SIZE;
   constexpr int PL = PA_WAVE / Q;
@@ -717,66 +964,107 @@
     const int64_t u = w * Q + kq;
     const ull k = (u < n) ? uniq[u] : 0;
     const bool active = (u < n) && (k != PA_EMPTY_KEY);
-    long long slot = -1;
-    if (active) {
-      const int64_t b = (int64_t)(k & (ull)mask);
-#pragma unroll
-      for (int h = 0; h < WS; ++h) {
-        const int wi = widx + h * PL;
-        const int p = wi / PA_BUCKET_SIZE;
-        const int s = wi % PA_BUCKET_SIZE;
-        const int64_t j = ((b + p) & mask) * PA_BUCKET_SIZE + s;
-        if (table_keys[j] == k) slot = j;
-      }
-    }
-    const unsigned long long found = __ballot(slot >= 0);
-    const unsigned long long nonzero = __ballot(k != PA_EMPTY_KEY);
     bool ok[Q];
     float* rowk[Q];
-#pragma unroll
-    for (int q = 0; q < Q; ++q) {
-      const unsigned fq = (unsigned)((found >> (PL * q)) & PL_MASK);
-      ok[q] = (w * Q + q) < n && (nonzero >> (PL * q) & 1ull);
-      if (ok[q] && fq == 0) {
-        if (lane == 0) atomicAdd(&skipped[0], 1);
-        ok[q] = false;
-      }
-      const long long slotq = ok[q] ? __shfl(slot, PL * q + __ffs(fq) - 1) : -1;
-      rowk[q] = ok[q] ? arena + (int64_t)slotq * row_width : nullptr;
-    }
     PaAccVec<T> acc[Q];
 #pragma unroll
     for (int q = 0; q < Q; ++q) acc[q] = 0.0f;
-    int64_t lop[Q], hip[Q];
-    bool all_single = true;
-#pragma unroll
-    for (int q = 0; q < Q; ++q) {
-      lop[q] = ok[q] ? ustarts[w * Q + q] : 0;
-      hip[q] = ok[q] ? ustarts[w * Q + q + 1] : 0;
-      all_single = all_single && ok[q] && hip[q] - lop[q] == 1;
-    }
-    if (all_single) {
-      const __half* gq[Q];
-      float scq[Q];
+    PaRowRegs<Q, T> rows;
+    bool hinted = false;
+    if constexpr (HINTS) {
+      const long long sh = active ? slot_hint[u] : -1;
+      const long long sr = active ? src_hint[u] : -1;
+      const bool usable = sh >= 0 && sh < n_slots && sr >= 0 && sr < n_src;
+      if (__ballot(usable) == ~0ull) {
+        const ull kv = table_keys[sh];
+        float scq[Q];
+        __half graw[Q][T];
+#pragma unroll
+        for (int q = 0; q < Q; ++q) {
+          const long long shq = __shfl(sh, PL * q);
+          const long long srq = __shfl(sr, PL * q);
+          ok[q] = true;
+          rowk[q] = arena + (int64_t)shq * row_width;
+          scq[q] = seg_scale ? seg_scale[srq] : 1.0f;
+          const __half* g = grads + (int64_t)srq * dim;
+#pragma unroll
+          for (int t = 0; t < T; ++t) {
+            const int c = lane + t * PA_WAVE;
+            if (c < dim) graw[q][t] = g[c];
+          }
+        }
+        pa_load_rows<Q, T>(rows, oa, ok, rowk, dim, lane);
+        if (__ballot(kv == k) == ~0ull) {
+          hinted = true;
+#pragma unroll
+          for (int q = 0; q < Q; ++q)
+#pragma unroll
+            for (int t = 0; t < T; ++t)
+              if (lane + t * PA_WAVE < dim)
+                acc[q][t] = (scq[q] != 0.0f)
+                                ? scq[q] * __half2float(graw[q][t])
+                                : 0.0f;
+        }
+      }
+    }
+    if (!hinted) {
+      long long slot = -1;
+      if (active) {
+        const int64_t b = (int64_t)(k & (ull)mask);
+#pragma unroll
+        for (int h = 0; h < WS; ++h) {
+          const int wi = widx + h * PL;
+          const int p = wi / PA_BUCKET_SIZE;
+          const int s = wi % PA_BUCKET_SIZE;
+          const int64_t j = ((b + p) & mask) * PA_BUCKET_SIZE + s;
+          if (table_keys[j] == k) slot = j;
+        }
+      }
+      const unsigned long long found = __ballot(slot >= 0);
+      const unsigned long long nonzero = __ballot(k != PA_EMPTY_KEY);
 #pragma unroll
       for (int q = 0; q < Q; ++q) {
-        const int64_t s = seg_id[perm[lop[q]]];
-        scq[q] = (s >= 0) ? (seg_scale ? seg_scale[s] : 1.0f) : 0.0f;
-        gq[q] = grads + (s >= 0 ? s : 0) * dim;
-      }
-      for (int t = 0, c = lane; c < dim; c += PA_WAVE, ++t) {
+        const unsigned fq = (unsigned)((found >> (PL * q)) & PL_MASK);
+        ok[q] = (w * Q + q) < n && (nonzero >> (PL * q) & 1ull);
+        if (ok[q] && fq == 0) {
+          if (lane == 0) atomicAdd(&skipped[0], 1);
+          ok[q] = false;
+        }
+        const long long slotq =
+            ok[q] ? __shfl(slot, PL * q + __ffs(fq) - 1) : -1;
+        rowk[q] = ok[q] ? arena + (int64_t)slotq * row_width : nullptr;
+      }
+      int64_t lop[Q], hip[Q];
+      bool all_single = true;
+#pragma unroll
+      for (int q = 0; q < Q; ++q) {
+        lop[q] = ok[q] ? ustarts[w * Q + q] : 0;
+        hip[q] = ok[q] ? ustarts[w * Q + q + 1] : 0;
+        all_single = all_single && ok[q] && hip[q] - lop[q] == 1;
+      }
+      if (all_single) {
+        const __half* gq[Q];
+        float scq[Q];
 #pragma unroll
         for (int q = 0; q < Q; ++q) {
-          const float g = __half2float(gq[q][c]);
-          acc[q][t] = (scq[q] != 0.0f) ? scq[q] * g : 0.0f;
+          const int64_t s = seg_id[perm[lop[q]]];
+          scq[q] = (s >= 0) ? (seg_scale ? seg_scale[s] : 1.0f) : 0.0f;
+          gq[q] = grads + (s >= 0 ? s : 0) * dim;
         }
-      }
-    } else {
-#pragma unroll
-      for (int q = 0; q < Q; ++q)
-        if (ok[q])
-          pa_reduce_positions<T>(acc[q], grads, perm, seg_id, seg_scale,
-                                 lop[q], hip[q], dim, lane, PA_WAVE);
+        for (int t = 0, c = lane; c < dim; c += PA_WAVE, ++t) {
+#pragma unroll
+          for (int q = 0; q < Q; ++q) {
+            const float g = __half2float(gq[q][c]);
+            acc[q][t] = (scq[q] != 0.0f) ? scq[q] * g : 0.0f;
+          }
+        }
+      } else {
+#pragma unroll
+        for (int q = 0; q < Q; ++q)
+          if (ok[q])
+            pa_reduce_positions<T>(acc[q], grads, perm, seg_id, seg_scale,
+                                   lop[q], hip[q], dim, lane, PA_WAVE);
+      }
     }
 #pragma unroll
     for (int q = 0; q < Q; ++q) {
@@ -792,78 +1080,11 @@
 #pragma unroll
     for (int q = 0; q < Q; ++q) any_ok = any_ok || ok[q];
     if (!any_ok) continue;
-    if (opt == 0) {
-      for (int t = 0, c = lane; c < dim; c += PA_WAVE, ++t) {
-        float w0[Q];
-#pragma unroll
-        for (int q = 0; q < Q; ++q)
-          w0[q] = ok[q] ? __builtin_nontemporal_load(&rowk[q][c]) : 0.0f;
-#pragma unroll
-        for (int q = 0; q < Q; ++q) {
-          if (!ok[q]) continue;
-          __builtin_nontemporal_store(pa_sgd(oa, w0[q], acc[q][t]), &rowk[q][c]);
-        }
-      }
-    } else if (opt == 1) {
-      if (pa_adagrad_shared(oa)) {
-        float a0[Q], gsq[Q] = {};
-#pragma unroll
-        for (int q = 0; q < Q; ++q) a0[q] = ok[q] ? rowk[q][dim] : 0.0f;
-        for (int t = 0, c = lane; c < dim; c += PA_WAVE, ++t) {
-          float w0[Q];
-#pragma unroll
-          for (int q = 0; q < Q; ++q)
-            w0[q] = ok[q] ? __builtin_nontemporal_load(&rowk[q][c]) : 0.0f;
-#pragma unroll
-          for (int q = 0; q < Q; ++q) {
-            if (!ok[q]) continue;
-            __builtin_nontemporal_store(
-                pa_adagrad_w(oa, w0[q], a0[q], acc[q][t]), &rowk[q][c]);
-            gsq[q] += acc[q][t] * acc[q][t];
-          }
-        }
-#pragma unroll
-        for (int off = PA_WAVE / 2; off > 0; off >>= 1)
-#pragma unroll
-          for (int q = 0; q < Q; ++q) gsq[q] += __shfl_down(gsq[q], off);
-        if (lane == 0)
-#pragma unroll
-          for (int q = 0; q < Q; ++q)
-            if (ok[q])
-              rowk[q][dim] = pa_adagrad_shared_acc(oa, a0[q], gsq[q], dim);
-      } else {
-        for (int t = 0, c = lane; c < dim; c += PA_WAVE, ++t) {
-          float w0[Q], a0[Q];
-#pragma unroll
-          for (int q = 0; q < Q; ++q) {
-            a0[q] = ok[q] ? __builtin_nontemporal_load(&rowk[q][dim + c]) : 0.0f;
-            w0[q] = ok[q] ? __builtin_nontemporal_load(&rowk[q][c]) : 0.0f;
-          }
-#pragma unroll
-          for (int q = 0; q < Q; ++q) {
-            if (!ok[q]) continue;
-            __builtin_nontemporal_store(
-                pa_adagrad_w(oa, w0[q], a0[q], acc[q][t]), &rowk[q][c]);
-            __builtin_nontemporal_store(pa_adagrad_acc(oa, a0[q], acc[q][t]),
-                                        &rowk[q][dim + c]);
-          }
-        }
-      }
+    if constexpr (HINTS) {
+      if (!hinted) pa_load_rows<Q, T>(rows, oa, ok, rowk, dim, lane);
+      pa_step_rows<Q, T>(rows, oa, ok, rowk, acc, dim, lane);
     } else {
-      for (int t = 0, c = lane; c < dim; c += PA_WAVE, ++t) {
-#pragma unroll
-        for (int q = 0; q < Q; ++q) {
-          if (!ok[q]) continue;
-          const float m = pa_adam_m(
-              oa, __builtin_nontemporal_load(&rowk[q][dim + c]), acc[q][t]);
-          const float v = pa_adam_v(
-              oa, __builtin_nontemporal_load(&rowk[q][2 * dim + c]), acc[q][t]);
-          const float w0 = __builtin_nontemporal_load(&rowk[q][c]);
-          __builtin_nontemporal_store(pa_adam_w(oa, w0, m, v), &rowk[q][c]);
-          __builtin_nontemporal_store(m, &rowk[q][dim + c]);
-          __builtin_nontemporal_store(v, &rowk[q][2 * dim + c]);
-        }
-      }
+      pa_update_rows<Q, T>(oa, ok, rowk, acc, dim, lane);
     }
   }
 }
@@ -958,7 +1179,7 @@
                      spill ? (ull*)evict_keys.data_ptr<int64_t>() : nullptr,
                      spill ? evict_count.data_ptr<int32_t>() : nullptr,
                      spill ? (long long*)evict_idx.data_ptr<int64_t>() : nullptr,
-                     n_dev);
+                     n_dev, nullptr, nullptr, nullptr, nullptr);
   if (out.scalar_type() == torch::kFloat16) {
     hipLaunchKernelGGL(init_gather_kernel<__half>, dim3(n_blocks_for(n, 4)),
                        dim3(256), 0, st, arena.data_ptr<float>(),
@@ -981,20 +1202,28 @@
   }
 }
 
-void store_lookup_sums(torch::Tensor table_keys, torch::Tensor ticks,
-                       torch::Tensor arena, torch::Tensor query,
-                       torch::Tensor perm, torch::Tensor ustarts,
-                       torch::Tensor sums, int64_t dim, int64_t train,
-                       int64_t tick, double lo, double hi, double admit_prob,
-                       double state_init, int64_t opt_space,
-                       torch::Tensor u_count) {
+std::vector<torch::Tensor> store_lookup_sums(
+    torch::Tensor table_keys, torch::Tensor ticks, torch::Tensor arena,
+    torch::Tensor query, torch::Tensor perm, torch::Tensor ustarts,
+    torch::Tensor sums, int64_t dim, int64_t train, int64_t tick, double lo,
+    double hi, double admit_prob, double state_init, int64_t opt_space,
+    torch::Tensor u_count, torch::Tensor seg_id) {
   const int64_t n = query.numel();
-  if (n == 0) return;
+  auto opts = torch::TensorOptions().dtype(torch::kInt64).device(query.device());
+  auto slots = torch::empty({n}, opts);
+  const bool hints = seg_id.numel() > 0;
+  auto src_hint = torch::empty({hints ? n : 0}, opts);
+  if (n == 0) return {src_hint, src_hint};
+  TORCH_CHECK(!hints || seg_id.numel() >= perm.numel(),
+              "store_lookup_sums: seg_id shorter than perm");
+  TORCH_CHECK(!hints || ustarts.numel() > n,
+              "store_lookup_sums: ustarts shorter than query + 1");
+  const int64_t* seg_ptr = hints ? seg_id.data_ptr<int64_t>() : nullptr;
+  long long* src_ptr =
+      hints ? (long long*)src_hint.data_ptr<int64_t>() : nullptr;
   const int64_t n_buckets = table_keys.numel() / PA_BUCKET_SIZE;
   const int row_width = (int)(dim + opt_space);
   const long long* n_dev = count_or_null(u_count);
-  auto opts = torch::TensorOptions().dtype(torch::kInt64).device(query.device());
-  auto slots = torch::empty({n}, opts);
   auto is_new = torch::empty({n}, opts.dtype(torch::kInt32));
   hipStream_t st = cur_stream();
   hipLaunchKernelGGL(probe_claim_kernel, dim3(n_blocks_for(n, 256)), dim3(256),
@@ -1004,7 +1233,9 @@
                      (int)train, (unsigned)tick, (float)admit_prob,
                      (long long*)slots.data_ptr<int64_t>(),
                      is_new.data_ptr<int32_t>(), nullptr, nullptr, nullptr,
-                     n_dev);
+                     n_dev, hints ? ustarts.data_ptr<int64_t>() : nullptr,
+                     hints ? perm.data_ptr<int64_t>() : nullptr, seg_ptr,
+                     src_ptr);
   const bool dual = !(dim < PA_WAVE && (PA_WAVE % dim) == 0);
   if (dual) {
     hipLaunchKernelGGL(init_scatter2_kernel,
@@ -1026,6 +1257,8 @@
                        (__half*)sums.data_ptr<at::Half>(), n, (int)dim,
                        row_width, lo, hi, (float)state_init, n_dev);
   }
+  if (!hints) return {src_hint, src_hint};
+  return {slots, src_hint};
 }
 
 torch::Tensor store_probe(torch::Tensor table_keys, torch::Tensor ticks,
@@ -1044,7 +1277,8 @@
                      0, (unsigned)tick, 1.0f,
                      (long long*)slots.data_ptr<int64_t>(),
                      is_new.data_ptr<int32_t>(), nullptr, nullptr, nullptr,
-                     count_or_null(u_count));
+                     count_or_null(u_count), nullptr, nullptr, nullptr,
+                     nullptr);
   return slots;
 }
 
@@ -1187,11 +1421,28 @@
                     torch::Tensor seg_scale, int64_t dim, int64_t opt,
                     std::vector<double> params, double b1_power,
                     double b2_power, double weight_bound,
-                    torch::Tensor skipped, torch::Tensor u_count) {
+                    torch::Tensor skipped, torch::Tensor u_count,
+                    torch::Tensor slot_hint, torch::Tensor src_hint) {
   const int64_t n = uniq.numel();
   if (n == 0) return;
   TORCH_CHECK(grads.scalar_type() == torch::kFloat16, "scatter_update: f16 grads");
   TORCH_CHECK(dim <= 8 * PA_WAVE, "scatter_update: dim too large");
+  const bool hints = slot_hint.numel() > 0;
+  TORCH_CHECK(!hints || (slot_hint.numel() >= n && src_hint.numel() >= n),
+              "scatter_update: hints shorter than uniq");
+  TORCH_CHECK(!hints || (slot_hint.scalar_type() == torch::kInt64 &&
+                         src_hint.scalar_type() == torch::kInt64 &&
+                         slot_hint.device() == uniq.device() &&
+                         src_hint.device() == uniq.device() &&
+                         slot_hint.is_contiguous() && src_hint.is_contiguous()),
+              "scatter_update: hints must be contiguous int64 on uniq's device");
+  TORCH_CHECK(!hints || seg_scale.numel() == 0 ||
+                  seg_scale.numel() >= grads.size(0),
+              "scatter_update: seg_scale shorter than grads");
+  const long long* slot_ptr =
+      hints ? (const long long*)slot_hint.data_ptr<int64_t>() : nullptr;
+  const long long* src_ptr =
+      hints ? (const long long*)src_hint.data_ptr<int64_t>() : nullptr;
   const int64_t n_buckets = table_keys.numel() / PA_BUCKET_SIZE;
   const int row_width = (int)arena.size(1);
   auto launch = [&](auto kernel, int keys_per_wave) {
@@ -1208,15 +1459,20 @@
                        (float)params[0], (float)params[1], (float)params[2],
                        (float)params[3], (float)b1_power, (float)b2_power,
                        (float)weight_bound, skipped.data_ptr<int32_t>(),
-                       count_or_null(u_count));
+                       count_or_null(u_count), slot_ptr, src_ptr,
+                       table_keys.numel(), grads.size(0));
   };
   const bool packed_small = (dim < PA_WAVE && (PA_WAVE % dim) == 0);
-  if (!packed_small && dim <= 128)
-    launch(scatter_update_multi_kernel<4>, 4);
-  else if (!packed_small && dim <= 256)
-    launch(scatter_update_multi_kernel<2>, 2);
-  else
-    launch(scatter_update_kernel, 1);
+  if (!packed_small && dim <= 128) {
+    if (hints) launch(scatter_update_multi_kernel<4, true>, 4);
+    else launch(scatter_update_multi_kernel<4, false>, 4);
+  } else if (!packed_small && dim <= 256) {
+    if (hints) launch(scatter_update_multi_kernel<2, true>, 2);
+    else launch(scatter_update_multi_kernel<2, false>, 2);
+  } else {
+    if (hints) launch(scatter_update_kernel<true>, 1);
+    else launch(scatter_update_kernel<false>, 1);
+  }
 }
 
 std::vector<torch::Tensor> a2a_route(torch::Tensor uniq, torch::Tensor u_count,
@@ -1326,6 +1582,16 @@
   m.def("a2a_route", &a2a_route,
         "padded-a2a key routing: range-partition bounds + packed scatter");
   m.def("neq_flags", &neq_flags, "sorted-run boundary flags");
+  namespace py = pybind11;
   m.def("scatter_update", &scatter_update,
-        "fused ordered grad scatter + optimizer update (no [U,dim] buffer)");
-}
+        "fused ordered grad scatter + optimizer update (no [U,dim] buffer); "
+        "slot_hint/src_hint: optional update hints of store_lookup_sums",
+        py::arg("table_keys"), py::arg("ticks"), py::arg("arena"),
+        py::arg("uniq"), py::arg("grads"), py::arg("perm"),
+        py::arg("ustarts"), py::arg("seg_id"), py::arg("seg_scale"),
+        py::arg("dim"), py::arg("opt"), py::arg("params"),
+        py::arg("b1_power"), py::arg("b2_power"), py::arg("weight_bound"),
+        py::arg("skipped"), py::arg("u_count"),
+        py::arg("slot_hint") = torch::empty({0}, torch::kInt64),
+        py::arg("src_hint") = torch::empty({0}, torch::kInt64));
+}
diff --git a/persia_amd/csrc/optim.h b/persia_amd/csrc/optim.h
--- a/persia_amd/csrc/optim.h
+++ b/persia_amd/csrc/optim.h
@@ -53,9 +53,11 @@
   return pa_clamp_weight(a, w - a.p0 * g * rsqrtf(acc + a.p2));
 }
 
+template <bool FUSE_GG = false>
 __device__ __forceinline__ float pa_adagrad_acc(const PaOptArgs& a, float acc,
                                                 float g) {
-  return acc * a.p1 + g * g;
+  if constexpr (FUSE_GG) return __builtin_fmaf(g, g, acc * a.p1);
+  return __builtin_fmaf(acc, a.p1, g * g);
 }
 
 __device__ __forceinline__ float pa_adagrad_shared_acc(const PaOptArgs& a,
```
